# Kizuna42/office-person-detection-vit

Measured on AMD Instinct MI355X. Metric: frames/sec (Phase-2 DETR detect) at 800x1333 batch 8, higher is better.
Workload: dtype f16

## Files before the change

office_person_detection_vit_amd/_capi.py:

```python

from __future__ import annotations

import ctypes as C
import os
from typing import Optional

_HERE = os.path.dirname(os.path.abspath(__file__))
LIB_PATH = os.path.join(_HERE, "libopd_hip.so")
TEST_LIB_PATH = os.path.join(_HERE, "libopd_hip_test.so")

OPD_PIXELS_U8_BGR_HWC = 0
OPD_PIXELS_F32_NCHW = 1
OPD_MEM_HOST = 0
OPD_MEM_DEVICE = 1
OPD_MEM_HOST_PIXELS_DEVICE_OUT = 2
OPD_FLAG_NO_GRAPH = 1
OPD_FLAG_MULTI_STREAM = 2
OPD_REID_MODEL_CLIP = 0
OPD_REID_MODEL_OSNET = 1
OPD_FLAG_BF16 = 4
OPD_COMM_ID_BYTES = 128
OPD_OK, OPD_EINVAL, OPD_EIO, OPD_ESCHEMA, OPD_EHIP, OPD_ENOMEM, OPD_ESTATE = 0, -1, -2, -3, -4, -5, -6


class OpdConfig(C.Structure):
    _fields_ = [("struct_size", C.c_int32), ("max_batch", C.c_int32), ("max_height", C.c_int32),
                ("max_width", C.c_int32), ("flags", C.c_int32), ("reserved", C.c_int32 * 3)]


class OpdKernelStat(C.Structure):
    _fields_ = [("name", C.c_char * 96), ("launches", C.c_int32), ("ms", C.c_float), ("flops", C.c_double)]


class OpdDet(C.Structure):
    _fields_ = [("x1", C.c_float), ("y1", C.c_float), ("x2", C.c_float), ("y2", C.c_float), ("score", C.c_float),
                ("label", C.c_int32), ("query_index", C.c_int32), ("frame", C.c_int32)]


class OpdModelInfo(C.Structure):
    _fields_ = [("depths", C.c_int32 * 4), ("d_model", C.c_int32), ("heads", C.c_int32), ("ffn_dim", C.c_int32),
                ("encoder_layers", C.c_int32), ("decoder_layers", C.c_int32), ("num_queries", C.c_int32),
                ("num_classes_plus1", C.c_int32), ("max_batch", C.c_int32), ("max_height", C.c_int32),
                ("max_width", C.c_int32), ("device_ordinal", C.c_int32), ("weight_bytes_device", C.c_int64),
                ("workspace_bytes_device", C.c_int64)]


class OpdReidConfig(C.Structure):
    _fields_ = [("struct_size", C.c_int32), ("max_crops", C.c_int32), ("flags", C.c_int32), ("model", C.c_int32), ("reserved", C.c_int32 * 4)]


class OpdReidModelInfo(C.Structure):
    _fields_ = [("feature_dim", C.c_int32), ("tokens", C.c_int32), ("hidden", C.c_int32), ("layers", C.c_int32), ("heads", C.c_int32),
                ("mlp_dim", C.c_int32), ("patch", C.c_int32), ("max_crops", C.c_int32), ("device_ordinal", C.c_int32),
                ("model", C.c_int32), ("weight_bytes_device", C.c_int64), ("workspace_bytes_device", C.c_int64)]


API = {
    "opd_detr_create": (C.c_int, [C.POINTER(OpdConfig), C.c_char_p, C.c_int, C.POINTER(C.c_void_p)]),
    "opd_detr_destroy": (None, [C.c_void_p]),
    "opd_detr_clone": (C.c_int, [C.c_void_p, C.POINTER(C.c_void_p)]),
    "opd_detr_info": (C.c_int, [C.c_void_p, C.POINTER(OpdModelInfo)]),
    "opd_detr_forward": (C.c_int, [C.c_void_p, C.c_void_p, C.c_int, C.c_int, C.c_int, C.c_int, C.c_int, C.c_void_p,
                                   C.c_void_p, C.c_void_p]),
    "opd_detr_forward_ragged": (C.c_int, [C.c_void_p, C.c_void_p, C.c_int, C.c_int, C.c_int, C.c_int, C.c_int, C.c_void_p,
                                          C.c_void_p, C.c_void_p, C.c_void_p]),
    "opd_detr_forward_resized": (C.c_int, [C.c_void_p, C.c_void_p] + [C.c_int] * 6 + [C.c_void_p] * 3),
    "opd_detr_resize_u8": (C.c_int, [C.c_void_p, C.c_void_p] + [C.c_int] * 5 + [C.c_void_p]),
    "opd_detr_detect_resized": (C.c_int, [C.c_void_p, C.c_void_p] + [C.c_int] * 6 + [C.c_float, C.POINTER(OpdDet), C.POINTER(C.c_int32)]),
    "opd_detr_detect_frames": (C.c_int, [C.c_void_p, C.POINTER(C.c_void_p)] + [C.c_int] * 6 + [C.c_float, C.POINTER(OpdDet), C.POINTER(C.c_int32)]),
    "opd_detr_detect_frames_features": (C.c_int, [C.c_void_p, C.POINTER(C.c_void_p)] + [C.c_int] * 5 + [C.c_float, C.c_int, C.POINTER(OpdDet), C.POINTER(C.c_int32),
                                                   C.POINTER(C.c_float)]),
    "opd_detr_postprocess": (C.c_int, [C.c_void_p, C.c_float, C.c_void_p, C.POINTER(OpdDet), C.POINTER(C.c_int32)]),
    "opd_detr_detect": (C.c_int, [C.c_void_p, C.c_void_p, C.c_int, C.c_int, C.c_int, C.c_int, C.c_int, C.c_float,
                                  C.c_void_p, C.POINTER(OpdDet), C.POINTER(C.c_int32)]),
    "opd_detr_detect_ragged": (C.c_int, [C.c_void_p, C.c_void_p, C.c_int, C.c_int, C.c_int, C.c_int, C.c_int, C.c_void_p,
                                         C.c_float, C.c_void_p, C.POINTER(OpdDet), C.POINTER(C.c_int32)]),
    "opd_detr_detect_async": (C.c_int, [C.c_void_p, C.c_void_p, C.c_int, C.c_int, C.c_int, C.c_int, C.c_int, C.c_float, C.c_void_p,
                                        C.POINTER(OpdDet), C.POINTER(C.c_int32), C.POINTER(C.c_int)]),
    "opd_detr_wait": (C.c_int, [C.c_void_p, C.c_int]),
    "opd_person_nms": (C.c_int, [C.POINTER(OpdDet), C.c_int, C.c_int, C.c_float]),
    "opd_person_nms_batch": (C.c_int, [C.POINTER(OpdDet), C.POINTER(C.c_int32), C.c_int, C.c_int, C.c_int, C.c_float]),
    "opd_host_alloc": (C.c_int, [C.c_size_t, C.POINTER(C.c_void_p)]),
    "opd_host_free": (None, [C.c_void_p]),
    "opd_similarity_matrix": (C.c_int, [C.c_int, C.c_void_p, C.c_void_p, C.c_void_p, C.c_int, C.c_void_p, C.c_void_p, C.c_void_p, C.c_int,
                                        C.c_int, C.c_double, C.c_double, C.c_int, C.c_void_p]),
    "opd_detr_roi_features": (C.c_int, [C.c_void_p, C.c_int, C.c_void_p, C.c_int, C.c_int, C.c_int, C.c_void_p]),
    "opd_detr_attention_map": (C.c_int, [C.c_void_p, C.c_int, C.c_int, C.c_void_p, C.c_int, C.c_void_p, C.c_int]),
    "opd_detr_set_profiling": (C.c_int, [C.c_void_p, C.c_int]),
    "opd_detr_stage_times": (C.c_int, [C.c_void_p, C.POINTER(C.c_float)]),
    "opd_detr_kernel_times": (C.c_int, [C.c_void_p, C.POINTER(C.c_float), C.POINTER(C.c_int32), C.POINTER(C.c_double)]),
    "opd_detr_kernel_table": (C.c_int, [C.c_void_p, C.c_void_p, C.c_int, C.POINTER(C.c_int)]),
    "opd_comm_available": (C.c_int, []),
    "opd_comm_unique_id": (C.c_int, [C.c_void_p]),
    "opd_comm_create": (C.c_int, [C.c_void_p, C.c_int, C.c_int, C.c_void_p, C.POINTER(C.c_void_p)]),
    "opd_comm_attach": (C.c_int, [C.c_void_p, C.c_void_p, C.POINTER(C.c_void_p)]),
    "opd_comm_destroy": (None, [C.c_void_p]),
    "opd_comm_info": (C.c_int, [C.c_void_p, C.POINTER(C.c_int), C.POINTER(C.c_int)]),
    "opd_comm_begin": (C.c_int, [C.c_void_p, C.c_int]),
    "opd_comm_detect": (C.c_int, [C.c_void_p, C.c_int, C.c_void_p, C.c_int, C.c_int, C.c_int, C.c_int, C.c_int, C.c_float, C.c_void_p]),
    "opd_comm_buffers": (C.c_int, [C.c_void_p, C.c_int, C.POINTER(C.c_void_p), C.POINTER(C.c_void_p)]),
    "opd_comm_exchange": (C.c_int, [C.c_void_p]),
    "opd_comm_wait": (C.c_int, [C.c_void_p, C.POINTER(OpdDet), C.POINTER(C.c_int32)]),
    "opd_reid_create": (C.c_int, [C.POINTER(OpdReidConfig), C.c_char_p, C.c_int, C.POINTER(C.c_void_p)]),
    "opd_reid_destroy": (None, [C.c_void_p]),
    "opd_reid_info": (C.c_int, [C.c_void_p, C.POINTER(OpdReidModelInfo)]),
    "opd_reid_extract": (C.c_int, [C.c_void_p, C.POINTER(C.c_void_p), C.c_void_p, C.c_int, C.c_int, C.c_void_p, C.c_void_p, C.c_int,
                                   C.c_void_p]),
    "opd_last_error": (C.c_char_p, []),
    "opd_version": (C.c_char_p, []),
}

TEST_API = {
    "opd_test_conv_gemm": (C.c_int, [C.c_void_p] * 6 + [C.c_int] * 15),
    "opd_test_gemm_splitk_ln": (C.c_int, [C.c_void_p] * 8 + [C.c_int] * 3),
    "opd_test_gemm_k256": (C.c_int, [C.c_void_p] * 5 + [C.c_int] * 5),
    "opd_test_gemm_ln": (C.c_int, [C.c_void_p] * 8 + [C.c_int] * 2),
    "opd_test_bench_gemm_ln": (C.c_int, [C.c_int] * 4 + [C.POINTER(C.c_float)]),
    "opd_test_gemm_ln_deep": (C.c_int, [C.c_void_p] * 7 + [C.c_int] + [C.c_void_p] * 3 + [C.c_int] * 3),
    "opd_test_set_heads2": (C.c_int, [C.c_int]),
    "opd_test_enc_ffn": (C.c_int, [C.c_void_p] * 9 + [C.c_int] + [C.c_void_p] * 3 + [C.c_int] * 3 + [C.c_void_p] * 2 + [C.c_int] * 2 + [C.c_void_p] * 5 + [C.c_int]),
    "opd_test_bench_enc_ffn": (C.c_int, [C.c_int] * 6 + [C.POINTER(C.c_float)]),
    "opd_test_bench_conv": (C.c_int, [C.c_int] * 11 + [C.POINTER(C.c_float)]),
    "opd_test_trace_btail": (C.c_int, [C.c_int] * 6 + [C.POINTER(C.c_ulonglong), C.c_int, C.POINTER(C.c_int)]),
    "opd_test_trace_conv": (C.c_int, [C.c_int] * 10 + [C.POINTER(C.c_ulonglong), C.c_int, C.POINTER(C.c_int)]),
    "opd_test_btail": (C.c_int, [C.c_void_p] * 10 + [C.c_int] * 6),
    "opd_test_bench_btail": (C.c_int, [C.c_int] * 8 + [C.POINTER(C.c_float)]),
    "opd_test_btail_repeat": (C.c_int, [C.c_void_p] * 8 + [C.c_int] * 6 + [C.POINTER(C.c_int)]),
    "opd_test_attention": (C.c_int, [C.c_void_p] * 4 + [C.c_int] * 4 + [C.c_float]),
    "opd_test_layernorm": (C.c_int, [C.c_void_p] * 5 + [C.c_int]),
    "opd_test_maxpool": (C.c_int, [C.c_void_p] * 2 + [C.c_int] * 6),
    "opd_test_preprocess_u8": (C.c_int, [C.c_void_p] * 2 + [C.c_int] * 5 + [C.c_void_p]),
    "opd_test_attention_masked": (C.c_int, [C.c_void_p] * 4 + [C.c_int] * 4 + [C.c_float, C.c_void_p, C.c_int]),
    "opd_test_stem2": (C.c_int, [C.c_void_p] * 4 + [C.c_int] * 5),
    "opd_test_stem_pool": (C.c_int, [C.c_void_p] * 4 + [C.c_int] * 7),
    "opd_test_set_fuse_stem_pool": (C.c_int, [C.c_void_p, C.c_int]),
    "opd_test_set_pos_shadow": (C.c_int, [C.c_void_p, C.c_int]),
    "opd_test_stem_pool_u8": (C.c_int, [C.c_void_p] * 6 + [C.c_int] * 3),
    "opd_test_set_fuse_btail": (C.c_int, [C.c_void_p, C.c_int]),
    "opd_test_set_fuse_gemm_ln": (C.c_int, [C.c_void_p, C.c_int]),
    "opd_test_f32_to_f16": (C.c_uint16, [C.c_float]),
    "opd_test_f16_to_f32": (C.c_float, [C.c_uint16]),
    "opd_test_normalise_key": (C.c_int, [C.c_char_p, C.c_char_p, C.c_int]),
    "opd_test_inspect_checkpoint": (C.c_int, [C.c_char_p, C.POINTER(C.c_int32)]),
    "opd_test_resize_coeffs": (C.c_int, [C.c_int, C.c_int, C.c_void_p, C.c_void_p, C.c_int]),
    "opd_test_valid_prefix": (C.c_int, [C.c_int] * 3),
    "opd_test_trunk_plan": (C.c_int, [C.c_void_p] + [C.c_int] * 6 + [C.c_void_p, C.c_int, C.c_void_p]),
    "opd_test_sine_pos_embed": (C.c_int, [C.c_int] * 5 + [C.c_void_p]),
    "opd_test_conv_dual": (C.c_int, [C.c_void_p] * 6 + [C.c_int] * 13),
    "opd_test_btail_sc": (C.c_int, [C.c_void_p] * 11 + [C.c_int] * 3),
    "opd_test_btail_chain": (C.c_int, [C.c_void_p] * 13 + [C.c_int] * 4),
    "opd_test_bench_attention": (C.c_int, [C.c_void_p] * 3 + [C.c_int] * 6 + [C.c_float, C.c_int, C.POINTER(C.c_float)]),
    "opd_test_trace_attention": (C.c_int, [C.c_void_p] * 3 + [C.c_int] * 6 + [C.c_float, C.c_void_p, C.c_int, C.POINTER(C.c_int)]),
    "opd_test_heads": (C.c_int, [C.c_void_p] * 13 + [C.c_int] * 2),
    "opd_test_postprocess": (C.c_int, [C.c_void_p] * 3 + [C.c_int] * 3 + [C.c_float, C.c_void_p, C.c_void_p]),
    "opd_test_roi_features": (C.c_int, [C.c_void_p] * 2 + [C.c_int] * 3 + [C.c_void_p]),
    "opd_test_set_conv_flags": (C.c_int, [C.c_int]),
    "opd_test_set_gemm_ln_kloop": (C.c_int, [C.c_int]),
    "opd_test_set_graph_guard": (C.c_int, [C.c_int]),
    "opd_test_set_alloc_poison": (C.c_int, [C.c_int]),
    "opd_test_check_redzones": (C.c_int, [C.c_void_p]),
    "opd_test_set_taps": (C.c_int, [C.c_void_p, C.c_int]),
    "opd_test_read_taps": (C.c_int, [C.c_void_p, C.c_void_p, C.c_int, C.c_char_p, C.c_int]),
    "opd_test_round_f16_diffused": (C.c_int, [C.c_void_p, C.c_int, C.c_int, C.c_int]),
    "opd_test_dec_qkv": (C.c_int, [C.c_void_p, C.c_void_p, C.c_int] + [C.c_void_p] * 5 + [C.c_int] * 2 + [C.c_void_p] * 4),
    "opd_test_dec_self": (C.c_int, [C.c_void_p] * 10 + [C.c_int, C.c_int, C.c_float, C.c_void_p]),
    "opd_test_attention_split": (C.c_int, [C.c_void_p] * 3 + [C.c_int] * 4 + [C.c_float, C.c_int, C.c_void_p, C.c_int, C.c_void_p, C.c_void_p]),
    "opd_test_dec_cross_out": (C.c_int, [C.c_void_p, C.c_void_p, C.c_int, C.c_void_p, C.c_int] + [C.c_void_p] * 4 + [C.c_int, C.c_void_p]),
    "opd_test_dec_ffn": (C.c_int, [C.c_void_p] * 4 + [C.c_int, C.c_int, C.c_void_p]),
    "opd_test_bench_dec": (C.c_int, [C.c_int] * 6 + [C.POINTER(C.c_float)]),
    "opd_test_heads_fused": (C.c_int, [C.c_void_p, C.c_void_p, C.c_int] + [C.c_void_p] * 13 + [C.c_int, C.c_int, C.c_void_p, C.c_void_p]),
    "opd_test_set_fused_dec": (C.c_int, [C.c_void_p, C.c_int]),
    "opd_test_set_elem_bf16": (C.c_int, [C.c_int]),
    "opd_test_trace_dec_self": (C.c_int, [C.c_int, C.c_int, C.c_void_p]),
    "opd_test_reid_geometry": (C.c_int, [C.c_void_p, C.c_int, C.c_int, C.c_int, C.c_void_p]),
    "opd_test_reid_coeffs": (C.c_int, [C.c_int] * 4 + [C.c_void_p, C.c_void_p, C.c_int]),
    "opd_test_reid_lut": (C.c_int, [C.c_void_p]),
    "opd_test_reid_pixels_host": (C.c_int, [C.c_void_p, C.c_int, C.c_int, C.c_void_p] + [C.c_int] * 3 + [C.c_void_p]),
    "opd_test_reid_pixels": (C.c_int, [C.c_void_p, C.POINTER(C.c_void_p), C.c_void_p, C.c_int, C.c_int, C.c_void_p, C.c_void_p, C.c_int,
                                       C.c_void_p]),
    "opd_test_reid_attention": (C.c_int, [C.c_void_p, C.c_void_p] + [C.c_int] * 3),
    "opd_test_reid_layernorm": (C.c_int, [C.c_void_p] * 5 + [C.c_int] * 3),
    "opd_test_reid_gemm": (C.c_int, [C.c_int, C.c_void_p, C.c_void_p, C.c_void_p, C.c_int, C.c_void_p] + [C.c_int] * 3),
    "opd_test_reid_l2norm": (C.c_int, [C.c_void_p] + [C.c_int] * 2),
    "opd_test_osnet_lut": (C.c_int, [C.c_void_p]),
    "opd_test_osnet_geometry": (C.c_int, [C.c_void_p, C.c_int, C.c_int, C.c_int, C.c_void_p]),
    "opd_test_osnet_pixels_host": (C.c_int, [C.c_void_p, C.c_int, C.c_int, C.c_void_p, C.c_int, C.c_void_p]),
    "opd_test_osnet_stem": (C.c_int, [C.c_void_p] * 4 + [C.c_int] * 2),
    "opd_test_osnet_gemm": (C.c_int, [C.c_int, C.c_void_p, C.c_int, C.c_int, C.c_void_p, C.c_int, C.c_int, C.c_void_p, C.c_void_p, C.c_void_p,
                                      C.c_int, C.c_void_p] + [C.c_int] * 6),
    "opd_test_osnet_dwconv": (C.c_int, [C.c_void_p] * 4 + [C.c_int] * 7),
    "opd_test_osnet_gate": (C.c_int, [C.c_void_p] * 7 + [C.c_int] * 4),
    "opd_test_osnet_avgpool2": (C.c_int, [C.c_void_p] * 2 + [C.c_int] * 4),
    "opd_test_osnet_head": (C.c_int, [C.c_void_p] * 4 + [C.c_int] * 3),
    "opd_test_reid_kernel_table": (C.c_int, [C.c_void_p, C.POINTER(C.c_void_p), C.c_void_p, C.c_int, C.c_void_p, C.c_void_p, C.c_int, C.c_int,
                                             C.POINTER(OpdKernelStat), C.c_int, C.POINTER(C.c_int)]),
}

_lib: Optional[C.CDLL] = None
_lib_has_hooks = False


def load_library(test_hooks: bool = False) -> C.CDLL:
    global _lib, _lib_has_hooks
    test_hooks = test_hooks or os.environ.get("OPD_TEST_HOOKS") == "1"
    if _lib is not None:
        if test_hooks and not _lib_has_hooks:
            raise RuntimeError("the product library is already loaded in this process; load the test build first "
                               "(_capi.load_library(test_hooks=True) or OPD_TEST_HOOKS=1)")
        return _lib
    path = TEST_LIB_PATH if test_hooks else LIB_PATH
    if not os.path.exists(path):
        raise RuntimeError(
            f"HIP extension not built: {path} is missing (run `python -c 'import __graft_entry__ as g; g.build()'`). "
            "This package has no CPU fallback.")
    lib = C.CDLL(path)
    for table in (API, TEST_API) if test_hooks else (API,):
        for name, (res, args) in table.items():
            fn = getattr(lib, name)
            fn.restype = res
            fn.argtypes = args
    _lib, _lib_has_hooks = lib, test_hooks
    return lib


def last_error() -> str:
    return load_library().opd_last_error().decode("utf-8", "replace")


def check(rc: int, what: str) -> None:
    if rc != 0:
        raise RuntimeError(f"{what} failed (code {rc}): {last_error()}")
```

office_person_detection_vit_amd/csrc/kernels_btail.hip:

```cpp
#include <hip/hip_runtime.h>
#include "opd_kernels.h"
#include "opd_elem.h"

typedef elem_t half8 __attribute__((ext_vector_type(8)));
typedef float float4v __attribute__((ext_vector_type(4)));
typedef unsigned int uint2v __attribute__((ext_vector_type(2)));
typedef unsigned int uint4v __attribute__((ext_vector_type(4)));

namespace {

constexpr int ROW_BYTES = 128;
constexpr int NW = 4;

__device__ __forceinline__ int swz(int row, int chunk) { return row * ROW_BYTES + ((chunk ^ (row & 7)) << 4); }

__device__ __forceinline__ int xcd_logical_block(int bid, int nblocks) {
    const int q = nblocks >> 3, r = nblocks & 7;
    const int x = bid & 7, k = bid >> 3;
    return (x < r ? x * (q + 1) : r * (q + 1) + (x - r) * q) + k;
}

__device__ __forceinline__ int own_row(const int rho) { return (rho & ~31) | (((rho >> 2) & 3) << 3) | (((rho >> 4) & 1) << 2) | (rho & 3); }
__device__ __forceinline__ int own_ch(const int nt, const int g) { return (nt >> 1) * 32 + g * 8 + (nt & 1) * 4; }

__device__ __forceinline__ int fdiv(const int m, const FastDiv& f) {
    return f.one ? m : (int)(__umulhi((unsigned)m, f.mul) >> f.shift);
}

__device__ __forceinline__ int xcd_logical_block_rev(int bid, int nblocks) {
    const int q = nblocks >> 3, r = nblocks & 7;
    const int x = bid & 7, k = bid >> 3;
    return (x < r ? x * (q + 1) + q - k : r * (q + 1) + (x - r) * q + q - 1 - k);
}

__device__ __forceinline__ unsigned pack2h(float a, float b) {
    typedef elem_t half2v __attribute__((ext_vector_type(2)));
    half2v h;
    h[0] = (elem_t)a;
    h[1] = (elem_t)b;
    unsigned u;
    __builtin_memcpy(&u, &h, 4);
    return u;
}
__device__ __forceinline__ void unpack2h(unsigned u, float& a, float& b) {
    typedef elem_t half2v __attribute__((ext_vector_type(2)));
    half2v h;
    __builtin_memcpy(&h, &u, 4);
    a = (float)h[0];
    b = (float)h[1];
}
__device__ __forceinline__ half8 as_half8(unsigned a, unsigned b, unsigned c, unsigned d) {
    uint4v u = {a, b, c, d};
    half8 h;
    __builtin_memcpy(&h, &u, 16);
    return h;
}

template <int N_OUTSTANDING>
__device__ __forceinline__ void wait_vmcnt() {
    static_assert(N_OUTSTANDING >= 0 && N_OUTSTANDING <= 63, "vmcnt range");
    asm volatile("s_waitcnt vmcnt(%0)" ::"n"(N_OUTSTANDING) : "memory");
}
__device__ __forceinline__ void compiler_fence() { asm volatile("" ::: "memory"); }

template <int C1, int C3, bool RDMA, bool SC = false, bool TRACE = false, int RC = 0>
__global__ __launch_bounds__(64 * NW, 8 / NW) void btail_kernel(BtailParams p) {
#if defined(__HIP_DEVICE_COMPILE__)
    unsigned long long tstamp[16] = {};
    auto stamp = [&](const int i) {
        if constexpr (TRACE) asm volatile("s_memtime %0\n\ts_waitcnt lgkmcnt(0)" : "=s"(tstamp[i])::"memory");
    };
    if constexpr (TRACE) asm volatile("s_memrealtime %0\n\ts_waitcnt lgkmcnt(0)" : "=s"(tstamp[0])::"memory");
    stamp(1);
    static_assert(!RDMA || C1 == 64, "residual staging buffers are budgeted for C1 == 64 (80 KiB of LDS per workgroup)");
    static_assert(!RDMA || RC == 0, "a rebuilt residual is not staged");
    static_assert(!SC || (C1 == 64 && !RDMA), "fused shortcut: 64-channel tails only; it replaces the residual");
    extern __shared__ __attribute__((aligned(16))) unsigned char smem[];
    constexpr int C2 = 4 * C1;
    constexpr int NT1 = C1 / 16;
    constexpr int KK1 = C1 / 32;
    constexpr int BM = 32 * NW;
    constexpr int A_BYTES = BM * ROW_BYTES;
    constexpr int RC_BYTES = RC ? 2 * 64 * ROW_BYTES : 0;
    constexpr int W1_PIECES = C1 / (8 * NW);
    constexpr int NCH = C2 / 64;
    constexpr int W2C_BYTES = 64 * C1 * 2;
    constexpr int W2_PIECES = W2C_BYTES / (1024 * NW);
    constexpr int W3_PIECES = C3 / (8 * NW);
    constexpr int SC_PIECES = 8 / NW;
    static_assert(W1_PIECES >= 1 && W2_PIECES >= 1 && (C3 == 0 || W3_PIECES >= 1), "every wave stages at least one piece of every operand");
    constexpr int NT3 = C3 / 16;
    constexpr int WSC_BYTES = SC ? 64 * ROW_BYTES : 0;
    constexpr int CHUNK_BYTES = W2C_BYTES + C3 * ROW_BYTES + WSC_BYTES + RC_BYTES;
    constexpr int STAGE_BYTES = (A_BYTES + C1 * ROW_BYTES) > CHUNK_BYTES ? (A_BYTES + C1 * ROW_BYTES) : CHUNK_BYTES;
    static_assert(RC == 0 || (RC == 1 && C1 == 64 && !RDMA && !SC), "residual rebuild: second block of stage 1");

    const int tid = threadIdx.x;
    const int lane = tid & 63;
    const int wave = __builtin_amdgcn_readfirstlane(tid >> 6);
    const int g = lane >> 4, li = lane & 15;
    const int m_base = (p.rev ? xcd_logical_block_rev(blockIdx.x, gridDim.x) : xcd_logical_block(blockIdx.x, gridDim.x)) * BM;
    const int wm0 = m_base + wave * 32;

    const int lrow = lane >> 3;
    const int lchunk = (lane & 7) ^ lrow;
    const unsigned backoff = (unsigned)(p.W + 1) * (unsigned)C1 * 2u;
    const __amdgpu_buffer_rsrc_t rsrc_a = __builtin_amdgcn_make_buffer_rsrc(
        const_cast<char*>(reinterpret_cast<const char*>(p.x1)) - backoff, 0, (unsigned)((size_t)p.B * p.H * p.W * C1 * 2) + backoff, 0x00020000);
    const __amdgpu_buffer_rsrc_t rsrc_w1 = __builtin_amdgcn_make_buffer_rsrc(const_cast<f16_t*>(p.w1), 0, (unsigned)(C1 * 9 * C1 * 2), 0x00020000);
    const __amdgpu_buffer_rsrc_t rsrc_w2 = __builtin_amdgcn_make_buffer_rsrc(const_cast<f16_t*>(p.w2p), 0, (unsigned)(C2 * C1 * 2), 0x00020000);
    const __amdgpu_buffer_rsrc_t rsrc_w3 = __builtin_amdgcn_make_buffer_rsrc(const_cast<f16_t*>(C3 ? p.w3p : p.w2p), 0, (unsigned)((C3 ? C3 : 1) * C2 * 2), 0x00020000);
    const __amdgpu_buffer_rsrc_t rsrc_sc = __builtin_amdgcn_make_buffer_rsrc(const_cast<f16_t*>(SC ? p.wsc : RC ? p.rc_wsc : p.w2p), 0, (unsigned)(C2 * 64 * 2), 0x00020000);
    const __amdgpu_buffer_rsrc_t rsrc_rw = __builtin_amdgcn_make_buffer_rsrc(const_cast<f16_t*>(RC ? p.rc_w2 : p.w2p), 0, (unsigned)(C2 * 64 * 2), 0x00020000);
    unsigned rowoff[4], rowmask[4], woff1[W1_PIECES], woff2[W2_PIECES], woff3[W3_PIECES ? W3_PIECES : 1], woffsc[2];
#pragma unroll
    for (int i = 0; i < 2; ++i)
        woffsc[i] = (unsigned)(own_row(((wave * SC_PIECES + i) & 7) * 8 + lrow) * 64) * 2u + (unsigned)lchunk * 16u;
    {
        const int ohw = p.OH * p.OW;
#pragma unroll
        for (int i = 0; i < 4; ++i) {
            const int m = m_base + (wave * 4 + i) * 8 + lrow;
            const bool okm = m < p.M;
            const int mm = okm ? m : 0;
            const int b = fdiv(mm, p.fd_ohw);
            const int r = mm - b * ohw;
            const int oh = fdiv(r, p.fd_ow);
            const int ow = r - oh * p.OW;
            rowoff[i] = (unsigned)(((b * p.H + oh * p.stride) * p.W + ow * p.stride) * C1) * 2u + (unsigned)lchunk * 16u;
            unsigned kwmask = 0, mask = 0;
#pragma unroll
            for (int kw = 0; kw < 3; ++kw)
                if ((unsigned)(ow * p.stride - 1 + kw) < (unsigned)p.W) kwmask |= 1u << kw;
#pragma unroll
            for (int kh = 0; kh < 3; ++kh)
                if ((unsigned)(oh * p.stride - 1 + kh) < (unsigned)p.H) mask |= kwmask << (kh * 3);
            rowmask[i] = okm ? mask : 0u;
        }
#pragma unroll
        for (int i = 0; i < W1_PIECES; ++i)
            woff1[i] = (unsigned)(own_row((wave * W1_PIECES + i) * 8 + lrow) * (9 * C1)) * 2u + (unsigned)lchunk * 16u;
#pragma unroll
        for (int i = 0; i < W2_PIECES; ++i) {
            const int q = wave * W2_PIECES + i;
            woff2[i] = (unsigned)(own_row((q & 7) * 8 + lrow) * C1 + (q >> 3) * 64) * 2u + (unsigned)lchunk * 16u;
        }
#pragma unroll
        for (int i = 0; i < W3_PIECES; ++i)
            woff3[i] = (unsigned)(own_row((wave * W3_PIECES + i) * 8 + lrow) * C2) * 2u + (unsigned)lchunk * 16u;
    }

    constexpr int kpc = C1 / 64;
    constexpr int nk = 9 * kpc;
    int tap_kh = 0, tap_kw = 0, tap_c = 0;
    auto issue_main = [&](int ks, int buf) {
        unsigned char* As = smem + buf * STAGE_BYTES;
        unsigned char* Ws = As + A_BYTES;
        const int tap = tap_kh * 3 + tap_kw;
        const int soff_a = ((tap_kh * p.W + tap_kw) * C1 + tap_c * 64) * 2;
#pragma unroll
        for (int i = 0; i < 4; ++i) {
            const unsigned vo = ((rowmask[i] >> tap) & 1u) ? rowoff[i] : 0x80000000u;
            __builtin_amdgcn_raw_ptr_buffer_load_lds(rsrc_a, (__attribute__((address_space(3))) void*)(As + (wave * 4 + i) * 1024), 16, vo,
                                                     soff_a, 0, 0);
        }
#pragma unroll
        for (int i = 0; i < W1_PIECES; ++i)
            __builtin_amdgcn_raw_ptr_buffer_load_lds(rsrc_w1, (__attribute__((address_space(3))) void*)(Ws + (wave * W1_PIECES + i) * 1024),
                                                     16, woff1[i], ks * 128, 0, 0);
        if (++tap_c == kpc) {
            tap_c = 0;
            if (++tap_kw == 3) { tap_kw = 0; ++tap_kh; }
        }
    };
    auto issue_chunk = [&](int j, int buf) {
        unsigned char* W2s = smem + buf * STAGE_BYTES;
#pragma unroll
        for (int i = 0; i < W2_PIECES; ++i)
            __builtin_amdgcn_raw_ptr_buffer_load_lds(rsrc_w2, (__attribute__((address_space(3))) void*)(W2s + (wave * W2_PIECES + i) * 1024),
                                                     16, woff2[i], j * (64 * C1 * 2), 0, 0);
        if constexpr (C3 > 0) {
            unsigned char* W3s = W2s + W2C_BYTES;
#pragma unroll
            for (int i = 0; i < W3_PIECES; ++i)
                __builtin_amdgcn_raw_ptr_buffer_load_lds(rsrc_w3, (__attribute__((address_space(3))) void*)(W3s + (wave * W3_PIECES + i) * 1024),
                                                         16, woff3[i], j * 128, 0, 0);
        }
        if constexpr (SC) {
            unsigned char* Wscs = W2s + W2C_BYTES + C3 * ROW_BYTES;
#pragma unroll
            for (int i = 0; i < SC_PIECES; ++i)
                __builtin_amdgcn_raw_ptr_buffer_load_lds(rsrc_sc, (__attribute__((address_space(3))) void*)(Wscs + (wave * SC_PIECES + i) * 1024), 16,
                                                         woffsc[i], j * (64 * 64 * 2), 0, 0);
        }
        if constexpr (RC) {
            unsigned char* Wr = W2s + W2C_BYTES + C3 * ROW_BYTES;
#pragma unroll
            for (int i = 0; i < SC_PIECES; ++i) {
                __builtin_amdgcn_raw_ptr_buffer_load_lds(rsrc_rw, (__attribute__((address_space(3))) void*)(Wr + (wave * SC_PIECES + i) * 1024), 16,
                                                         woffsc[i], j * (64 * 64 * 2), 0, 0);
                __builtin_amdgcn_raw_ptr_buffer_load_lds(rsrc_sc, (__attribute__((address_space(3))) void*)(Wr + 8192 + (wave * SC_PIECES + i) * 1024), 16,
                                                         woffsc[i], j * (64 * 64 * 2), 0, 0);
            }
        }
    };
    const bool pr_ok[2] = {wm0 + li < p.M, wm0 + 16 + li < p.M};
    bool y_ok[2] = {pr_ok[0] && p.y != nullptr, pr_ok[1] && p.y != nullptr};
    if (p.y_stride2) {
#pragma unroll
        for (int mt = 0; mt < 2; ++mt) {
            const int m = wm0 + mt * 16 + li;
            const int r = m - fdiv(m, p.fd_ohw) * (p.OH * p.OW);
            const int oh = fdiv(r, p.fd_ow), ow = r - oh * p.OW;
            y_ok[mt] = y_ok[mt] && !((oh | ow) & 1);
        }
    }
    const size_t pr_row[2] = {(size_t)(wm0 + li) * C2 + g * 8, (size_t)(wm0 + 16 + li) * C2 + g * 8};
    constexpr int RES_BUF = NW * 4096;
    unsigned char* const res_lds = smem + 2 * STAGE_BYTES + wave * 4096;
    const __amdgpu_buffer_rsrc_t rsrc_r = __builtin_amdgcn_make_buffer_rsrc(
        const_cast<f16_t*>(p.res ? p.res : p.x1), 0, p.res ? (unsigned)((size_t)p.M * C2 * 2) : 0u, 0x00020000);
    const unsigned res_voff = (unsigned)((wm0 + lrow) * C2) * 2u + (unsigned)lchunk * 16u;
    auto issue_res = [&](int j) {
#pragma unroll
        for (int i = 0; i < 4; ++i)
            __builtin_amdgcn_raw_ptr_buffer_load_lds(rsrc_r, (__attribute__((address_space(3))) void*)(res_lds + (j & 1) * RES_BUF + i * 1024), 16,
                                                     res_voff + (unsigned)(i * 8 * C2 * 2), j * 128, 0, 0);
    };
    const bool has_res = RC ? true : (!SC && p.res != nullptr && !(p.dbg & 4));
    const bool res_dma = RDMA && has_res;
    auto load_res = [&](int j, uint4 (&r)[4]) {
        if constexpr (RDMA) {
            if (has_res) issue_res(j);
        } else {
#pragma unroll
            for (int i = 0; i < 4; ++i) {
                r[i] = make_uint4(0u, 0u, 0u, 0u);
                if (has_res && pr_ok[i & 1]) r[i] = *reinterpret_cast<const uint4*>(p.res + pr_row[i & 1] + j * 64 + (i >> 1) * 32);
            }
        }
    };

    const int ks_first = (p.dbg & 1) ? nk - 1 : 0;
    if (ks_first) { tap_kh = 2; tap_kw = 2; tap_c = kpc - 1; }
    half8 xs[2][2], a1p[2][2];
    if constexpr (SC || RC != 0) {
        const f16_t* xsrc = SC ? p.xs : p.rc_xs;
#pragma unroll
        for (int mt = 0; mt < 2; ++mt) {
            const int m = wm0 + mt * 16 + li;
#pragma unroll
            for (int kk = 0; kk < 2; ++kk) {
                half8 v = {}, u = {};
                if (m < p.M) v = *reinterpret_cast<const half8*>(xsrc + (size_t)m * 64 + kk * 32 + g * 8);
                if constexpr (RC != 0)
                    if (m < p.M) u = *reinterpret_cast<const half8*>(p.rc_a1 + (size_t)m * 64 + kk * 32 + g * 8);
                xs[mt][kk] = v;
                a1p[mt][kk] = u;
            }
        }
    }
    stamp(2);
    issue_main(ks_first, ks_first & 1);
    float4v acc1[NT1][2];
#pragma unroll
    for (int nt = 0; nt < NT1; ++nt) {
        const float4v b = *reinterpret_cast<const float4v*>(p.b1 + own_ch(nt, g));
        acc1[nt][0] = b;
        acc1[nt][1] = b;
    }
    OPD_DMA_BARRIER();
    uint4 res[3][4];
    auto compute_main = [&](int buf) {
        const unsigned char* As = smem + buf * STAGE_BYTES;
        const unsigned char* Ws = As + A_BYTES;
#pragma unroll
        for (int kk = 0; kk < 2; ++kk) {
            half8 xf[2], wf[NT1];
#pragma unroll
            for (int mt = 0; mt < 2; ++mt) xf[mt] = *reinterpret_cast<const half8*>(As + swz(wave * 32 + mt * 16 + li, kk * 4 + g));
#pragma unroll
            for (int nt = 0; nt < NT1; ++nt) wf[nt] = *reinterpret_cast<const half8*>(Ws + swz(nt * 16 + li, kk * 4 + g));
#pragma unroll
            for (int nt = 0; nt < NT1; ++nt)
#pragma unroll
                for (int mt = 0; mt < 2; ++mt) acc1[nt][mt] = OPD_MFMA_16x16x32(wf[nt], xf[mt], acc1[nt][mt]);
        }
    };
#pragma unroll 1
    for (int ks = ks_first; ks + 1 < nk; ++ks) {
        issue_main(ks + 1, (ks + 1) & 1);
        compute_main(ks & 1);
        __syncthreads();
    }
    issue_chunk(0, nk & 1);
    compiler_fence();
    if constexpr (RC == 0) {
        load_res(0, res[0]);
        load_res(1, res[1]);
    }
    compiler_fence();
    compute_main((nk - 1) & 1);
    if (res_dma) wait_vmcnt<4>();
    else wait_vmcnt<0>();
    __builtin_amdgcn_s_barrier();
    stamp(3);

    half8 a1[2][KK1];
#pragma unroll
    for (int mt = 0; mt < 2; ++mt)
#pragma unroll
        for (int kk = 0; kk < KK1; ++kk) {
            float4v u = acc1[2 * kk][mt], v = acc1[2 * kk + 1][mt];
#pragma unroll
            for (int r = 0; r < 4; ++r) {
                u[r] = u[r] > 0.f ? u[r] : 0.f;
                v[r] = v[r] > 0.f ? v[r] : 0.f;
            }
            a1[mt][kk] = as_half8(pack2h(u[0], u[1]), pack2h(u[2], u[3]), pack2h(v[0], v[1]), pack2h(v[2], v[3]));
        }

    if (p.a1_out) {
#pragma unroll
        for (int mt = 0; mt < 2; ++mt)
#pragma unroll
            for (int kk = 0; kk < KK1; ++kk)
                if (pr_ok[mt]) *reinterpret_cast<half8*>(p.a1_out + (size_t)(wm0 + mt * 16 + li) * C1 + kk * 32 + g * 8) = a1[mt][kk];
    }

    float4v accz[NT3 ? NT3 : 1][2];
    if constexpr (C3 > 0) {
#pragma unroll
        for (int nt = 0; nt < NT3; ++nt) {
            const float4v b = *reinterpret_cast<const float4v*>(p.b3 + own_ch(nt, g));
            accz[nt][0] = b;
            accz[nt][1] = b;
        }
    }

    if (p.dbg & 8) return;
#pragma unroll
    for (int j = 0; j < NCH; ++j) {
        const int buf = (nk + j) & 1;
        uint4 (&res_cur)[4] = res[j % 3];
        if (j + 1 < NCH) issue_chunk(j + 1, buf ^ 1);
        compiler_fence();
        if constexpr (RDMA) {
            if (has_res) {
#pragma unroll
                for (int i = 0; i < 4; ++i)
                    res_cur[i] = *reinterpret_cast<const uint4*>(res_lds + (j & 1) * RES_BUF + swz((i & 1) * 16 + li, (i >> 1) * 4 + g));
                asm volatile("s_waitcnt lgkmcnt(0)" ::: "memory");
                if (j + 2 < NCH) issue_res(j + 2);
            }
        } else if constexpr (RC == 0) {
            if (j + 2 < NCH) load_res(j + 2, res[(j + 2) % 3]);
        }
        compiler_fence();
        const unsigned char* W2s = smem + buf * STAGE_BYTES;
        if constexpr (RC != 0) {
            const unsigned char* Wr = W2s + W2C_BYTES + C3 * ROW_BYTES;
            float4v accr[4][2];
#pragma unroll
            for (int nt = 0; nt < 4; ++nt) {
                const float4v b = *reinterpret_cast<const float4v*>(p.rc_b + j * 64 + own_ch(nt, g));
                accr[nt][0] = b;
                accr[nt][1] = b;
            }
#pragma unroll
            for (int half = 0; half < 2; ++half)
#pragma unroll
                for (int kk = 0; kk < 2; ++kk) {
                    half8 wf[4];
#pragma unroll
                    for (int nt = 0; nt < 4; ++nt) wf[nt] = *reinterpret_cast<const half8*>(Wr + half * 8192 + swz(nt * 16 + li, kk * 4 + g));
#pragma unroll
                    for (int nt = 0; nt < 4; ++nt)
#pragma unroll
                        for (int mt = 0; mt < 2; ++mt) accr[nt][mt] = OPD_MFMA_16x16x32(wf[nt], half ? xs[mt][kk] : a1p[mt][kk], accr[nt][mt]);
                }
#pragma unroll
            for (int q = 0; q < 2; ++q)
#pragma unroll
                for (int mt = 0; mt < 2; ++mt) {
                    float4v v0 = accr[2 * q][mt], v1 = accr[2 * q + 1][mt];
#pragma unroll
                    for (int r = 0; r < 4; ++r) {
                        v0[r] = v0[r] > 0.f ? v0[r] : 0.f;
                        v1[r] = v1[r] > 0.f ? v1[r] : 0.f;
                    }
                    res_cur[2 * q + mt] = make_uint4(pack2h(v0[0], v0[1]), pack2h(v0[2], v0[3]), pack2h(v1[0], v1[1]), pack2h(v1[2], v1[3]));
                }
        }
        float4v acc2[4][2];
#pragma unroll
        for (int nt = 0; nt < 4; ++nt) {
            const float4v b = *reinterpret_cast<const float4v*>(p.b2 + j * 64 + own_ch(nt, g));
            acc2[nt][0] = b;
            acc2[nt][1] = b;
        }
#pragma unroll
        for (int kk = 0; kk < KK1; ++kk) {
            half8 wf[4];
#pragma unroll
            for (int nt = 0; nt < 4; ++nt)
                wf[nt] = *reinterpret_cast<const half8*>(W2s + (kk >> 1) * 8192 + swz(nt * 16 + li, (kk & 1) * 4 + g));
#pragma unroll
            for (int nt = 0; nt < 4; ++nt)
#pragma unroll
                for (int mt = 0; mt < 2; ++mt) acc2[nt][mt] = OPD_MFMA_16x16x32(wf[nt], a1[mt][kk], acc2[nt][mt]);
        }
        if constexpr (SC) {
            const unsigned char* Wscs = W2s + W2C_BYTES + C3 * ROW_BYTES;
#pragma unroll
            for (int kk = 0; kk < 2; ++kk) {
                half8 wf[4];
#pragma unroll
                for (int nt = 0; nt < 4; ++nt) wf[nt] = *reinterpret_cast<const half8*>(Wscs + swz(nt * 16 + li, kk * 4 + g));
#pragma unroll
                for (int nt = 0; nt < 4; ++nt)
#pragma unroll
                    for (int mt = 0; mt < 2; ++mt) acc2[nt][mt] = OPD_MFMA_16x16x32(wf[nt], xs[mt][kk], acc2[nt][mt]);
            }
        }
        half8 yf[2][2];
#pragma unroll
        for (int q = 0; q < 2; ++q)
#pragma unroll
            for (int mt = 0; mt < 2; ++mt) {
                float4v v0 = acc2[2 * q][mt], v1 = acc2[2 * q + 1][mt];
                if (has_res) {
                    const uint4 r = res_cur[2 * q + mt];
                    float a, b;
                    unpack2h(r.x, a, b); v0[0] += a; v0[1] += b;
                    unpack2h(r.y, a, b); v0[2] += a; v0[3] += b;
                    unpack2h(r.z, a, b); v1[0] += a; v1[1] += b;
                    unpack2h(r.w, a, b); v1[2] += a; v1[3] += b;
                }
#pragma unroll
                for (int r = 0; r < 4; ++r) {
                    v0[r] = v0[r] > 0.f ? v0[r] : 0.f;
                    v1[r] = v1[r] > 0.f ? v1[r] : 0.f;
                }
                yf[q][mt] = as_half8(pack2h(v0[0], v0[1]), pack2h(v0[2], v0[3]), pack2h(v1[0], v1[1]), pack2h(v1[2], v1[3]));
            }
        if constexpr (C3 > 0) {
            const unsigned char* W3s = W2s + W2C_BYTES;
#pragma unroll
            for (int kk = 0; kk < 2; ++kk) {
#pragma unroll
                for (int nt = 0; nt < NT3; ++nt) {
                    const half8 wf = *reinterpret_cast<const half8*>(W3s + swz(nt * 16 + li, kk * 4 + g));
#pragma unroll
                    for (int mt = 0; mt < 2; ++mt) accz[nt][mt] = OPD_MFMA_16x16x32(wf, yf[kk][mt], accz[nt][mt]);
                }
            }
        }
        if (j + 1 < NCH) {
            if (res_dma && j + 2 < NCH) wait_vmcnt<4>();
            else wait_vmcnt<0>();
            __builtin_amdgcn_s_barrier();
        }
#pragma unroll
        for (int q = 0; q < 2; ++q)
#pragma unroll
            for (int mt = 0; mt < 2; ++mt)
                if (y_ok[mt] && !(p.dbg & 2)) *reinterpret_cast<half8*>(p.y + pr_row[mt] + j * 64 + q * 32) = yf[q][mt];
        stamp(4 + j);
    }

    if constexpr (C3 > 0) {
#pragma unroll
        for (int q = 0; q < NT3 / 2; ++q)
#pragma unroll
            for (int mt = 0; mt < 2; ++mt) {
                float4v v0 = accz[2 * q][mt], v1 = accz[2 * q + 1][mt];
#pragma unroll
                for (int r = 0; r < 4; ++r) {
                    v0[r] = v0[r] > 0.f ? v0[r] : 0.f;
                    v1[r] = v1[r] > 0.f ? v1[r] : 0.f;
                }
                if (pr_ok[mt] && !(p.dbg & 2))
                    *reinterpret_cast<uint4*>(p.z + (size_t)(wm0 + mt * 16 + li) * C3 + q * 32 + g * 8) =
                        make_uint4(pack2h(v0[0], v0[1]), pack2h(v0[2], v0[3]), pack2h(v1[0], v1[1]), pack2h(v1[2], v1[3]));
            }
    }
    if constexpr (TRACE) {
        stamp(4 + NCH);
        asm volatile("s_waitcnt vmcnt(0)" ::: "memory");
        stamp(5 + NCH);
        asm volatile("s_memrealtime %0\n\ts_waitcnt lgkmcnt(0)" : "=s"(tstamp[15])::"memory");
        if (threadIdx.x == 0 && p.trace) {
#pragma unroll
            for (int i = 0; i < 16; ++i) p.trace[(size_t)blockIdx.x * 16 + i] = tstamp[i];
        }
    }
#endif
}

template <int C1, int C3, bool RDMA, bool SC = false, bool TRACE = false, int RC = 0>
hipError_t launch_btail_t(const BtailParams& p, hipStream_t stream) {
    constexpr int BM = 32 * NW;
    constexpr int MAIN = (BM + C1) * ROW_BYTES, CHUNK = 64 * C1 * 2 + C3 * ROW_BYTES + (SC ? 64 * ROW_BYTES : 0) + (RC ? 2 * 64 * ROW_BYTES : 0);
    constexpr int LDS = 2 * (MAIN > CHUNK ? MAIN : CHUNK) + (RDMA ? 2 * NW * 4096 : 0);
    static_assert(LDS <= 160 * 1024, "LDS per workgroup");
    OPD_SET_MAX_LDS_ONCE((btail_kernel<C1, C3, RDMA, SC, TRACE, RC>), LDS);
    OPD_LAUNCH((btail_kernel<C1, C3, RDMA, SC, TRACE, RC>), dim3((p.M + BM - 1) / BM), dim3(64 * NW), LDS, stream, p);
    static const char* const kname = opd_kernel_name("btail_kernel<%d, %d, %s, %s, %s, %d>", C1, C3, OPD_BOOLSTR(RDMA), OPD_BOOLSTR(SC), OPD_BOOLSTR(TRACE), RC);
    opd_last_kernel_name = kname;
    return hipGetLastError();
}

}

#ifndef OPD_ELEM_BF16
bool opd_btail_supported(int C1, int C3) {
    return (C1 == 64 && (C3 == 0 || C3 == 64 || C3 == 128)) || (C1 == 128 && (C3 == 0 || C3 == 128)) || opd_btail256_supported(C1, C3);
}
#endif

hipError_t OPD_SYM(opd_launch_btail)(const BtailParams& p_in, hipStream_t stream) {
    if (!opd_btail_supported(p_in.C1, p_in.C3) || p_in.OH <= 0 || p_in.OW <= 0) return hipErrorInvalidValue;
    BtailParams p = p_in;
    p.fd_ohw = opd_make_fastdiv((unsigned)p.OH * (unsigned)p.OW);
    p.fd_ow = opd_make_fastdiv((unsigned)p.OW);
    if ((size_t)p.B * p.H * p.W * p.C1 * 2 + (size_t)(p.W + 1) * p.C1 * 2 >= 0x7fffff00ull) return hipErrorInvalidValue;
    if ((size_t)p.M * p.C1 * 8 >= 0x7fffff00ull) return hipErrorInvalidValue;
    if (p.C1 == 256) return OPD_SYM(opd_launch_btail256)(p, stream);
    if (p.y_stride2 && (p.stride != 1 || p.C3 == 0)) return hipErrorInvalidValue;
    if (!p.y && !p.a1_out) return hipErrorInvalidValue;
    if (p.rc) {
        if (p.rc != 1 || p.C1 != 64 || p.C3 != 64 || p.stride != 1 || p.res || p.xs || !p.rc_a1 || !p.rc_xs || !p.rc_w2 || !p.rc_wsc || !p.rc_b ||
            p.trace || (size_t)p.M * 64 * 2 >= 0x7fffff00ull)
            return hipErrorInvalidValue;
        return launch_btail_t<64, 64, false, false, false, 1>(p, stream);
    }
    if (p.xs) {
        if (p.C1 != 64 || p.C3 != 64 || p.stride != 1 || !p.wsc || p.res || (size_t)p.M * 64 * 2 >= 0x7fffff00ull) return hipErrorInvalidValue;
        return launch_btail_t<64, 64, false, true>(p, stream);
    }
    if (p.trace) {
        if (p.C1 == 64 && p.C3 == 64 && (p.dbg & 16)) return launch_btail_t<64, 64, false, false, true>(p, stream);
        if (p.C1 == 64 && p.C3 == 64) return launch_btail_t<64, 64, true, false, true>(p, stream);
        if (p.C1 == 128 && p.C3 == 128) return launch_btail_t<128, 128, false, false, true>(p, stream);
        return hipErrorInvalidValue;
    }
    if (p.C1 == 64) {
        const bool rdma = !(p.dbg & 16);
        if (p.C3 == 0) return rdma ? launch_btail_t<64, 0, true>(p, stream) : launch_btail_t<64, 0, false>(p, stream);
        if (p.C3 == 64) return rdma ? launch_btail_t<64, 64, true>(p, stream) : launch_btail_t<64, 64, false>(p, stream);
        return rdma ? launch_btail_t<64, 128, true>(p, stream) : launch_btail_t<64, 128, false>(p, stream);
    }
    if (p.C3 == 0) return launch_btail_t<128, 0, false>(p, stream);
    return launch_btail_t<128, 128, false>(p, stream);
}

#ifndef OPD_ELEM_BF16
void opd_permute_k32(const f16_t* w, f16_t* out, int rows, int K) {
    for (int n = 0; n < rows; ++n)
        for (int b = 0; b < K; b += 32)
            for (int g = 0; g < 4; ++g)
                for (int e = 0; e < 4; ++e) {
                    out[(size_t)n * K + b + 8 * g + e] = w[(size_t)n * K + b + 4 * g + e];
                    out[(size_t)n * K + b + 8 * g + 4 + e] = w[(size_t)n * K + b + 16 + 4 * g + e];
                }
}
#endif
```

office_person_detection_vit_amd/csrc/opd_kernels.h:

```cpp
#pragma once
#include <hip/hip_runtime.h>
#include <stdint.h>
#include <vector>

typedef uint16_t f16_t;
enum { OPD_DT_F16 = 0, OPD_DT_BF16 = 1 };

#include <mutex>
#define OPD_SET_MAX_LDS_ONCE(kernel, bytes)                                                                                  \
    do {                                                                                                                     \
        static std::once_flag once_[16];                                                                                     \
        static hipError_t err_[16];                                                                                          \
        int dev_ = 0;                                                                                                        \
        if (hipGetDevice(&dev_) != hipSuccess || dev_ < 0 || dev_ >= 16) return hipErrorInvalidDevice;    \
        std::call_once(once_[dev_], [&] { err_[dev_] = hipFuncSetAttribute(reinterpret_cast<const void*>(kernel), hipFuncAttributeMaxDynamicSharedMemorySize, (bytes)); }); \
        if (err_[dev_] != hipSuccess) return err_[dev_];                                                                     \
    } while (0)

extern thread_local const char* opd_last_kernel_name;
extern thread_local int opd_dbg_skip_launch;
const char* opd_kernel_name(const char* fmt, ...);
#define OPD_LAUNCH(kernel, ...)                       \
    do {                                              \
        opd_last_kernel_name = #kernel;               \
        if (!opd_dbg_skip_launch) hipLaunchKernelGGL(kernel, __VA_ARGS__); \
    } while (0)
#define OPD_BOOLSTR(b) ((b) ? "true" : "false")

#if defined(__HIP_DEVICE_COMPILE__)
#define OPD_DMA_BARRIER()                                        \
    do {                                                         \
        asm volatile("s_waitcnt vmcnt(0)" ::: "memory");         \
        __syncthreads();                                         \
    } while (0)
#else
#define OPD_DMA_BARRIER() __syncthreads()
#endif

struct FastDiv { unsigned mul, shift, one; };
inline FastDiv opd_make_fastdiv(unsigned d) {
    FastDiv f{0u, 0u, 1u};
    if (d <= 1u) return f;
    int s = 0;
    while ((1ull << s) < d) ++s;
    f.mul = (unsigned)(((1ull << (31 + s)) + d - 1) / d);
    f.shift = (unsigned)(s - 1);
    f.one = 0u;
    return f;
}

struct ConvGemmParams {
    const f16_t* x;
    const f16_t* w;
    const float* bias;
    const float* const* bias_ptrs;
    const f16_t* res16;
    const float* res32;
    void* out;
    f16_t* out16_aux;
    const void* zero16;
    int B, H, W, Cin, OH, OW, N, KH, KW, stride, pad;
    int M, K;
    int relu, bias_period, out_f32;
    int bias_pmod, bias_pcols;
    int stem;
    int dbg;
    int split_k;
    const f16_t* x2;
    int H2, W2, Cin2, stride2, K1;
    FastDiv fd_ohw, fd_ow, fd_period;
    const f16_t* x_alt;
    int alt_mod, alt_cols;
    unsigned tap_rep;
    FastDiv fd_tilesn, fd_ntiles;
    unsigned long long* trace;
    int force_mt;
    int wprefetch;
    int flat_staging;
    int dtype;
};
hipError_t opd_launch_conv_gemm(const ConvGemmParams& p, hipStream_t stream);
bool opd_conv_w8_supported(const ConvGemmParams& p);
hipError_t opd_launch_conv_w8(const ConvGemmParams& p, hipStream_t stream);
hipError_t opd_launch_stem_pool_u8(const uint8_t* frames, const int32_t* valid_hw, const f16_t* w, const float* bias, f16_t* out, int B, int H,
                                   int W, int OH, int OW, int PH, int PW, hipStream_t stream, int dtype = 0);
hipError_t opd_launch_stem_pool(const f16_t* x4p, const f16_t* w, const float* bias, f16_t* out, int B, int Hp, int Wp, int OH,
                                int OW, int PH, int PW, hipStream_t stream, int dtype = 0);
struct BtailParams {
    const f16_t* x1;
    const f16_t* w1;
    const float* b1;
    const f16_t* w2p;
    const float* b2;
    const f16_t* res;
    const f16_t* xs;
    const f16_t* wsc;
    f16_t* y;
    const f16_t* w3p;
    const float* b3;
    f16_t* z;
    int B, H, W, OH, OW, stride, M, C1, C3;
    int dbg;
    FastDiv fd_ohw, fd_ow;
    unsigned long long* trace;
    int rev;
    int dtype;
    f16_t* a1_out;
    const f16_t* rc_a1;
    const f16_t* rc_xs;
    const f16_t* rc_w2;
    const f16_t* rc_wsc;
    const float* rc_b;
    int rc;
    int y_stride2;
};
bool opd_btail_supported(int C1, int C3);
hipError_t opd_launch_btail(const BtailParams& p, hipStream_t stream);
void opd_permute_k32(const f16_t* w, f16_t* out, int rows, int K);
bool opd_btail256_supported(int C1, int C3);
hipError_t opd_launch_btail256(const BtailParams& p, hipStream_t stream);

struct GemmLnParams {
    const f16_t* x;
    const f16_t* w;
    const float* bias;
    const float* res32;
    const float* gamma;
    const float* beta;
    float* y32;
    f16_t* y16;
    int M, K;
    int kloop;
    int deep_k;
    const float* pos;
    const float* const* pos_ptrs;
    int pos_period;
    f16_t* yp16;
    int dtype;
};
hipError_t opd_launch_gemm_ln(const GemmLnParams& p, hipStream_t stream);
struct EncFfnParams {
    const f16_t* x;
    const unsigned char* wpack;
    const float* b2;
    const float* res32;
    const float* gamma;
    const float* beta;
    float* y32;
    f16_t* y16;
    f16_t* yp16;
    const float* pos;
    const float* const* pos_ptrs;
    int pos_period;
    int M, F;
    int dtype;
    int dbg;
    int wprefetch;
    const f16_t* attn;
    const float* bo;
    const float* gamma1;
    const float* beta1;
    int pack_front;
    int pack_tail;
    int tail, tail_pos;
    f16_t* tail_out;
    int tail_ld;
    int tail_col[16];
};
hipError_t opd_launch_enc_ffn(const EncFfnParams& p, hipStream_t stream);
size_t opd_encffn_pack_bytes(int F, int tail, int front);
void opd_encffn_pack(const uint16_t* w1, const float* b1, const uint16_t* w2, int F, const uint16_t* wt, const float* bt, int tail, const uint16_t* wo,
                     unsigned char* out);
struct GemmK256Params {
    const f16_t* x;
    const f16_t* w;
    const float* bias;
    f16_t* out16;
    float* out32;
    int M, N, ldx, ldw, slices, bias_period, relu;
    int dtype;
};
hipError_t opd_launch_gemm_k256(const GemmK256Params& p, hipStream_t stream);

hipError_t opd_launch_preprocess_u8(const uint8_t* frames, f16_t* out, int B, int H, int W, int Hp, int Wp, const int32_t* valid_hw,
                                    hipStream_t stream, int dtype = 0);
hipError_t opd_launch_preprocess_f32(const float* pv, f16_t* out, int B, int H, int W, int Hp, int Wp, const int32_t* valid_hw,
                                     hipStream_t stream, int dtype = 0);
void opd_resize_coeffs(int in_size, int out_size, std::vector<int32_t>* bounds, std::vector<int32_t>* coeffs, int* ksize_out);
hipError_t opd_launch_resize_u8(const uint8_t* in, uint8_t* out, int B, int h, int w, int oh, int ow, const int32_t* bounds_h,
                                const int32_t* coeff_h, int ksize_h, const int32_t* bounds_v, const int32_t* coeff_v, int ksize_v,
                                hipStream_t stream);
hipError_t opd_launch_maxpool(const f16_t* x, f16_t* out, int B, int H, int W, int C, int OH, int OW, hipStream_t stream, int dtype = 0);
hipError_t opd_launch_layernorm(const float* x, const float* gamma, const float* beta, float* y, f16_t* y16,
                                int rows, hipStream_t stream, int dtype = 0);
hipError_t opd_launch_reduce_ln(const float* partials, int nsplit, size_t slab_stride, const float* residual,
                                const float* gamma, const float* beta, float* y, f16_t* y16, int rows, hipStream_t stream, int dtype = 0);
hipError_t opd_launch_reduce_ln_pos(const float* partials, int nsplit, size_t slab_stride, const float* residual, const float* gamma,
                                    const float* beta, float* y, f16_t* y16, int rows, const float* pos, const float* const* pos_ptrs,
                                    int period, f16_t* yp16, hipStream_t stream, int dtype = 0);
hipError_t opd_launch_broadcast_rows(const float* c, float* y, f16_t* y16, int rows, hipStream_t stream, int dtype = 0);
hipError_t opd_launch_cast_f16(const float* x, f16_t* y, size_t n, hipStream_t stream, int dtype = 0);
hipError_t opd_launch_reduce_act16(const float* partials, int nsplit, size_t slab_stride, f16_t* out, size_t n, int relu, hipStream_t stream, int dtype = 0);
#define OPD_TAP_BLOCKS 64
hipError_t opd_launch_checksum(const void* buf, size_t bytes, unsigned long long* slots, hipStream_t stream);
hipError_t opd_launch_gemm_f32(const float* A, const float* Wt, const float* bias, float* C, int M, int N, int K,
                               int ldc, hipStream_t stream);
struct HeadParams {
    const float* hs;
    const float* partials;
    int nsplit;
    const float *ffn_b2, *ln3_gamma, *ln3_beta;
    const float *ln_gamma, *ln_beta;
    const float *wc, *bc, *w1, *b1, *w2, *b2, *w3, *b3;
    const f16_t *wc_f, *w1_f, *w2_f;
    float* logits;
    float* boxes;
    int rows, ncls;
};
hipError_t opd_launch_heads(const HeadParams& p, hipStream_t stream);
hipError_t opd_launch_heads2(const HeadParams& p, hipStream_t stream);
struct PostParams {
    const float* logits;
    const float* boxes;
    const int32_t* orig_hw;
    void* records;
    int32_t* counts;
    int B, Q, ncls;
    float threshold;
};
hipError_t opd_launch_postprocess(const PostParams& p, hipStream_t stream);
hipError_t opd_launch_roi_features(const float* enc, const int32_t* rois , float* out,
                                   int n, int h, int w, hipStream_t stream);
hipError_t opd_launch_roi_features_records(const float* enc, const void* records, const int32_t* counts, const int32_t* orig_hw, int label,
                                           float* out, int B, int Q, int h, int w, hipStream_t stream);

hipError_t opd_launch_attention_map(const f16_t* q, int ldq, const f16_t* k, int ldk, const int32_t* sel, int nsel, int heads, int Lk, float scale,
                                    const int32_t* key_valid2, int key_row, void* stat, float* out, hipStream_t stream, int dtype = 0);

hipError_t opd_launch_similarity_matrix(const float* f1, const float* b1, const uint8_t* has1, int n1, const float* f2, const float* b2,
                                        const uint8_t* has2, int n2, int D, double aw, double mw, int as_distance, float* out,
                                        hipStream_t stream);

void opd_split_f16_frag(const float* w, int N, int K, f16_t* out);
struct DecQkvParams {
    const float* h_in;
    const float* partials;
    int nsplit;
    const float* b2;
    const float *ln_g, *ln_b;
    float* h_out;
    const f16_t* w;
    const float* bias;
    f16_t* q16;
    f16_t* k16;
    f16_t* vT;
    int M, Q;
};
hipError_t opd_launch_dec_qkv(const DecQkvParams& p, hipStream_t stream);
struct DecSelfParams {
    const f16_t *q16, *k16, *vT;
    float* h;
    const f16_t* wo;
    const float *bo, *ln_g, *ln_b;
    const f16_t* wq;
    const float* rbq;
    f16_t* qc16;
    int qc_bf16;
// ... 72 lines not shown
```

office_person_detection_vit_amd/csrc/opd_model.cpp:

```cpp
#include <new>
#include <stdexcept>

#include "opd_model.h"

using namespace opd;


namespace opd {

std::atomic<int> g_alloc_poison{-1};

static int upload_f32(opd_detr* m, float** dst, const std::vector<float>& v) {
    RCCHK(dalloc(m, dst, v.size(), true));
    HIPCHK(hipMemcpy(*dst, v.data(), v.size() * 4, hipMemcpyHostToDevice));
    return OPD_OK;
}
static int upload_f16(opd_detr* m, f16_t** dst, const std::vector<float>& v) {
    std::vector<f16_t> h(v.size());
    if (m->dtype == OPD_DT_BF16) for (size_t i = 0; i < v.size(); ++i) h[i] = f32_to_bf16(v[i]);
    else for (size_t i = 0; i < v.size(); ++i) h[i] = f32_to_f16(v[i]);
    RCCHK(dalloc(m, dst, h.size(), true));
    HIPCHK(hipMemcpy(*dst, h.data(), h.size() * 2, hipMemcpyHostToDevice));
    return OPD_OK;
}
// ... 492 lines not shown
    HIPCHK(opd_launch_checksum(p, bytes, m->d_taps + (size_t)m->tap_next * OPD_TAP_BLOCKS, m->stream));
    if ((int)m->tap_names.size() <= m->tap_next) m->tap_names.resize(m->tap_next + 1);
    m->tap_names[m->tap_next++] = name;
    return OPD_OK;
}

static int conv_splits(const opd_detr* m, const Conv& c, int stage) {
    if (!m->sw.small_splitk || stage < 0 || stage > 3 || c.stem || c.K % 64 != 0 || c.Cout % 64 != 0) return 1;
    const long long px = (long long)m->cfg.max_batch * (long long)m->stage_px[stage];
    const long long tiles = ((px + 127) / 128) * (c.Cout / 64);
    const int nk = c.K / 64;
    if (tiles > 160 || nk < 24) return 1;
    int best = 1;
    for (int s : {2, 3, 4, 6, 8})
        if (nk % s == 0 && nk / s >= 6 && tiles * s <= 640) best = s;
    return best;
}

static int run_conv(opd_detr* m, const Conv& c, const f16_t* x, int B, int H, int W, int OH, int OW, void* out, bool relu,
                    const f16_t* res16, int stage = -1) {
    ConvGemmParams p{}; p.dtype = m->dtype;
    p.x = x; p.w = c.w; p.bias = c.bias; p.res16 = res16; p.res32 = nullptr; p.out = out; p.out16_aux = nullptr; p.zero16 = m->zero_bias;
    p.B = B; p.H = H; p.W = W; p.Cin = c.Cin; p.OH = OH; p.OW = OW; p.N = c.Cout; p.KH = c.KH; p.KW = c.KW;
    p.stride = c.stride; p.pad = c.pad; p.M = B * OH * OW; p.K = c.K; p.relu = relu ? 1 : 0; p.bias_period = 0;
    p.out_f32 = 0; p.stem = c.stem ? 1 : 0; p.dbg = m->sw.dbg_gemm; p.wprefetch = m->sw.wprefetch & 1;
    if (const int splits = res16 ? 1 : conv_splits(m, c, stage); splits > 1 && (size_t)splits * p.M * c.Cout <= m->slab_floats) {
        p.out = m->d_slab; p.out_f32 = 1; p.relu = 0; p.split_k = splits;
        RCCHK(timed_begin(m, CLS_CONV, 2.0 * p.M * (double)c.Cout * c.KH * c.KW * c.Cin));
        HIPCHK(opd_launch_conv_gemm(p, m->stream));
        RCCHK(timed_end(m));
        RCCHK(timed_begin(m, CLS_OTHER, 0.0));
        HIPCHK(opd_launch_reduce_act16(m->d_slab, splits, (size_t)p.M * c.Cout, reinterpret_cast<f16_t*>(out), (size_t)p.M * c.Cout, relu ? 1 : 0, m->stream, m->dtype));
        RCCHK(timed_end(m));
        RCCHK(tap(m, c.KH == 3 ? "conv3x3" : "conv1x1", out, (size_t)p.M * c.Cout * 2));
        return OPD_OK;
    }
    RCCHK(timed_begin(m, CLS_CONV, 2.0 * p.M * (double)c.Cout * c.KH * c.KW * c.Cin));
    bool w8 = false;
    if (m->sw.w8 && c.Cout % 256 == 0 && c.Cout >= 512) {
        const long long tiles = (((long long)OH * OW * m->cfg.max_batch + 127) / 128) * (c.Cout / 256);
        const bool few = tiles <= 3LL * m->num_cus;
        const int kind = c.KH == 3 ? (m->sw.w8 & 1) : (c.K >= 1024 ? (m->sw.w8 & 2) : (c.K == 512 ? (m->sw.w8 & 4) : 0));
        w8 = few && kind && opd_conv_w8_supported(p);
    }
    HIPCHK(w8 ? opd_launch_conv_w8(p, m->stream) : opd_launch_conv_gemm(p, m->stream));
    RCCHK(timed_end(m));
    RCCHK(tap(m, c.KH == 3 ? "conv3x3" : "conv1x1", out, (size_t)p.M * c.Cout * 2));
    return OPD_OK;
}

static int run_gemm(opd_detr* m, const f16_t* x, const f16_t* w, const float* bias, int bias_period, int M, int N, int K,
                    void* out, bool out_f32, bool relu, const float* res32, const float* const* bias_ptrs = nullptr, int bias_pmod = 0,
                    int bias_pcols = 0, const f16_t* x_alt = nullptr, int alt_mod = 0, int alt_cols = 0) {
    ConvGemmParams p{}; p.dtype = m->dtype;
    p.bias_ptrs = bias_ptrs; p.bias_pmod = bias_pmod; p.bias_pcols = bias_pcols;
    p.x_alt = x_alt; p.alt_mod = alt_mod; p.alt_cols = alt_cols;
    p.x = x; p.w = w; p.bias = bias; p.res16 = nullptr; p.res32 = res32; p.out = out; p.out16_aux = nullptr; p.zero16 = m->zero_bias;
    p.B = M; p.H = 1; p.W = 1; p.Cin = K; p.OH = 1; p.OW = 1; p.N = N; p.KH = 1; p.KW = 1; p.stride = 1; p.pad = 0;
    p.M = M; p.K = K; p.relu = relu ? 1 : 0; p.bias_period = bias_period; p.out_f32 = out_f32 ? 1 : 0; p.stem = 0; p.dbg = m->sw.dbg_gemm; p.wprefetch = m->sw.wprefetch & 1;
    RCCHK(timed_begin(m, CLS_GEMM, 2.0 * M * (double)N * K));
    HIPCHK(opd_launch_conv_gemm(p, m->stream));
    RCCHK(timed_end(m));
    RCCHK(tap(m, "gemm", out, (size_t)M * N * (out_f32 ? 4 : 2)));
    return OPD_OK;
}

struct PosShadow { const float* pos; const float* const* pos_ptrs; int period; f16_t* yp16; };
static int run_gemm_splitk_ln(opd_detr* m, const f16_t* x, const f16_t* w, const float* bias, int M, int N, int K, int splits,
                              const float* res32, const LNp* ln, float* y32, f16_t* y16, int cls, const PosShadow* ps = nullptr) {
    ConvGemmParams p{}; p.dtype = m->dtype;
    p.x = x; p.w = w; p.bias = bias; p.out = m->d_slab; p.zero16 = m->zero_bias;
    p.B = M; p.H = 1; p.W = 1; p.Cin = K; p.OH = 1; p.OW = 1; p.N = N; p.KH = 1; p.KW = 1; p.stride = 1; p.pad = 0;
    p.M = M; p.K = K; p.out_f32 = 1; p.split_k = splits;
    RCCHK(timed_begin(m, cls, 2.0 * M * (double)N * K));
    HIPCHK(opd_launch_conv_gemm(p, m->stream));
    RCCHK(timed_end(m));
    RCCHK(tap(m, "splitk_slabs", m->d_slab, (size_t)splits * M * N * 4));
    RCCHK(timed_begin(m, CLS_OTHER, 0.0));
    HIPCHK(opd_launch_reduce_ln_pos(m->d_slab, splits, (size_t)M * N, res32, ln ? ln->g : nullptr, ln ? ln->b : nullptr, y32, y16, M,
                                    ps ? ps->pos : nullptr, ps ? ps->pos_ptrs : nullptr, ps ? ps->period : 0, ps ? ps->yp16 : nullptr, m->stream, m->dtype));
    RCCHK(timed_end(m));
    RCCHK(tap(m, "reduce_ln", y32, (size_t)M * N * 4));
    return OPD_OK;
}

static int run_gemm_ln(opd_detr* m, const f16_t* x, const f16_t* w, const float* bias, int M, int K, const float* res32,
                       const LNp& ln, float* y32, f16_t* y16) {
    GemmLnParams p{}; p.dtype = m->dtype;
    p.x = x; p.w = w; p.bias = bias; p.res32 = res32; p.gamma = ln.g; p.beta = ln.b; p.y32 = y32; p.y16 = y16; p.M = M; p.K = K;
    RCCHK(timed_begin(m, CLS_GEMM, 2.0 * M * 256.0 * K));
    HIPCHK(opd_launch_gemm_ln(p, m->stream));
    RCCHK(timed_end(m));
    RCCHK(tap(m, "gemm_ln", y32, (size_t)M * 256 * 4));
    return OPD_OK;
}

static int run_small_gemm(opd_detr* m, const f16_t* x, const f16_t* w, const float* bias, int bias_period, int M, int N, int K,
                          f16_t* out16, bool relu) {
    GemmK256Params p{}; p.dtype = m->dtype;
    p.x = x; p.w = w; p.bias = bias; p.out16 = out16; p.M = M; p.N = N; p.ldx = K; p.ldw = K; p.slices = 1;
    p.bias_period = bias_period; p.relu = relu ? 1 : 0;
    RCCHK(timed_begin(m, CLS_GEMM, 2.0 * M * (double)N * K));
    HIPCHK(opd_launch_gemm_k256(p, m->stream));
    RCCHK(timed_end(m));
    RCCHK(tap(m, "gemm_k256", out16, (size_t)M * N * 2));
    return OPD_OK;
}
static int run_small_gemm_ln(opd_detr* m, const f16_t* x, const f16_t* w, const float* bias, int M, int K, const float* res32,
                             const LNp& ln, float* y32, f16_t* y16) {
    GemmK256Params p{}; p.dtype = m->dtype;
    p.x = x; p.w = w; p.bias = bias; p.out32 = m->d_slab; p.M = M; p.N = 256; p.ldx = K; p.ldw = K; p.slices = K / 256;
    RCCHK(timed_begin(m, CLS_GEMM, 2.0 * M * 256.0 * K));
    HIPCHK(opd_launch_gemm_k256(p, m->stream));
    RCCHK(timed_end(m));
    RCCHK(timed_begin(m, CLS_OTHER, 0.0));
    HIPCHK(opd_launch_reduce_ln(m->d_slab, p.slices, (size_t)M * 256, res32, ln.g, ln.b, y32, y16, M, m->stream, m->dtype));
    RCCHK(timed_end(m));
    RCCHK(tap(m, "small_gemm_ln", y32, (size_t)M * 256 * 4));
    return OPD_OK;
}

static int run_attn(opd_detr* m, const f16_t* q, int ldq, const f16_t* k, int ldk, const f16_t* v, int ldv, f16_t* o, int ldo,
                    int B, int Lq, int Lk, const int32_t* key_valid = nullptr, int key_row = 0) {
    AttnParams p{}; p.dtype = m->dtype;
    p.key_valid = key_valid; p.key_row = key_row;
    p.q = q; p.k = k; p.v = v; p.o = o; p.B = B; p.heads = m->arch.heads; p.Lq = Lq; p.Lk = Lk;
    p.ldq = ldq; p.ldk = ldk; p.ldv = ldv; p.ldo = ldo;
    p.scale = 1.0f / sqrtf((float)(m->arch.d_model / m->arch.heads));
    RCCHK(timed_begin(m, CLS_ATTN, 4.0 * B * (double)m->arch.heads * Lq * Lk * 32));
    HIPCHK(opd_launch_attention(p, m->stream));
    RCCHK(timed_end(m));
    if (ldo == m->arch.d_model) RCCHK(tap(m, "attention", o, (size_t)B * Lq * ldo * 2));
    return OPD_OK;
}

TrunkPlan plan_trunk(const Arch& a, const std::vector<Block>& blocks, const opd_config& cfg, const Switches& sw, int B, int H2, int W2, int num_cus,
                     bool taps, int profiling, bool has_stream2) {
    TrunkPlan plan;
    plan.steps.resize(blocks.size());
    plan.split = B;
    const bool multi = (cfg.flags & OPD_FLAG_MULTI_STREAM) != 0;
    int ch = H2, cw = W2, oh3 = 0, ow3 = 0;
    for (int s = 0, bi = 0; s < 4; ++s) {
        for (int l = 0; l < a.depths[s]; ++l, ++bi) {
            const Block& b = blocks[bi];
            const Block* nbk = bi + 1 < (int)blocks.size() ? &blocks[bi + 1] : nullptr;
            const int oh = (b.c1.stride == 2) ? down2(ch) : ch, ow = (b.c1.stride == 2) ? down2(cw) : cw;
            const int C1 = b.c1.Cin;
            const bool sc_in_tail = b.has_sc && sw.fuse_shortcut && sw.fuse_btail && block_has_bias2sc(b) && b.sc.KH == 1 && b.sc.stride == 1 &&
                                    b.sc.Cin == 64 && b.c1.Cin == 64 && b.c1.stride == 1 && b.c2.Cout == 256 && nbk && conv_has_kperm(nbk->c0) &&
                                    nbk->c0.Cin == 256 && nbk->c0.Cout == 64;
            bool tail = sw.fuse_btail && b.c1.KH == 3 && b.c1.Cout == C1 && b.c2.Cin == C1 && b.c2.Cout == 4 * C1 && conv_has_kperm(b.c2) &&
                        opd_btail_supported(C1, 0);
            if (sw.dual_over_tail && tail && b.has_sc && !sc_in_tail && block_has_w2sc(b)) tail = false;
            if (C1 == 256 && tail) {
                const long long tiles = ((long long)cfg.max_batch * oh * ow + 127) / 128;
                const bool pays = tiles * 10 >= (long long)num_cus * 6;
                if (sw.tail3 == 0 || (sw.tail3 == 1 && !pays && !multi)) tail = false;
            }
            const bool sc_in_expand = b.has_sc && sw.fuse_shortcut && block_has_w2sc(b) && !sc_in_tail && !tail;
            tail = tail && (size_t)B * ch * cw * C1 * 2 < 0x7ff00000ull;
            TrunkStep& t = plan.steps[bi];
            t.path = tail ? PATH_TAIL : sc_in_expand ? PATH_DUAL : PATH_CONVS;
            t.sc = !b.has_sc ? SC_NONE : (sc_in_tail && tail) ? SC_TAIL : sc_in_expand ? SC_EXPAND : SC_LAUNCH;
            t.res = (t.sc == SC_TAIL || t.sc == SC_EXPAND) ? RES_NONE : t.sc == SC_LAUNCH ? RES_SHORTCUT : RES_TRUNK;
            t.store = STORE_Y;
            t.C3 = 0;
            if (tail && nbk && conv_has_kperm(nbk->c0) && nbk->c0.Cin == 4 * C1 && opd_btail_supported(C1, nbk->c0.Cout)) t.C3 = nbk->c0.Cout;
            if (tail && sw.y_stride2 && t.C3 && b.c1.stride == 1 && l + 1 == a.depths[s] && nbk && nbk->has_sc && nbk->sc.stride == 2 && nbk->sc.KH == 1 &&
                nbk->c1.stride == 2 && !taps)
                t.store = STORE_Y_STRIDE2;
            if (l > 0 && sw.tail_rc && !taps) {
                TrunkStep& prev = plan.steps[bi - 1];
                if (prev.path == PATH_TAIL && prev.sc == SC_TAIL && prev.C3 == 64 && prev.store == STORE_Y && tail && C1 == 64 && t.C3 == 64 &&
                    t.res == RES_TRUNK) {
                    prev.store = STORE_A1;
                    t.res = RES_REBUILD;
                }
            }
            if (s == 2 && l == 0) { oh3 = oh; ow3 = ow; }
            ch = oh; cw = ow;
        }
    }
    const int s3 = a.depths[0] + a.depths[1], s4 = s3 + a.depths[2];
    bool fused3 = a.depths[2] > 2 && profiling != 1 && !taps && has_stream2 && sw.tail3_split && !multi && B >= 2;
    for (int bi = s3 + 1; bi < s4 && fused3; ++bi) fused3 = plan.steps[bi].path == PATH_TAIL;
    if (fused3) {
        auto tiles_of = [&](int frames) { return ((long long)frames * oh3 * ow3 + 127) / 128; };
        const long long total = tiles_of(B), cus = num_cus, last = total % cus;
        if (total > cus && last > 0 && last < cus / 2) {
            const long long whole = (total / cus) * cus;
            int bA = B - 1;
            while (bA > 1 && tiles_of(bA) > whole) --bA;
            if (tiles_of(bA) <= whole) plan.split = bA;
        }
    }
    int n = 0;
    auto rev = [&](const TrunkStep& t) { return t.path == PATH_TAIL && sw.tail_rev ? (n++ & 1) : 0; };
    for (int bi = 0; bi < s4; ++bi) plan.steps[bi].rev = rev(plan.steps[bi]);
    for (int bi = s3 + 1; bi < s4 && plan.split < B; ++bi) plan.steps[bi].rev_b = rev(plan.steps[bi]);
    for (int bi = s4; bi < (int)blocks.size(); ++bi) plan.steps[bi].rev = rev(plan.steps[bi]);
    return plan;
}

#define MARK(i)                                                   \
    do {                                                          \
        if (m->profiling) HIPCHK(hipEventRecord(m->ev[i], m->stream)); \
        opd_dbg_skip_launch = (m->sw.dbg_skip >> (i)) & 1;           \
    } while (0)

static bool is_ragged(const int32_t* valid_hw, int B, int H, int W) {
    if (!valid_hw) return false;
    for (int b = 0; b < B; ++b)
        if (valid_hw[2 * b] != H || valid_hw[2 * b + 1] != W) return true;
    return false;
}

static int enqueue_forward(opd_detr* m, const void* d_pixels, int pixel_format, int B, int H, int W, const int32_t* valid_hw = nullptr) {
    const Arch& a = m->arch;
    Dims d;
    compute_dims(B, H, W, &d);
    const int fh = d.sh[3], fw = d.sw[3];
    const bool ragged = is_ragged(valid_hw, B, H, W);
    Plan* plan = nullptr;
    const float* const* enc_bias_ptrs[16] = {};
    const float* const* kv_bias_ptrs = nullptr;
    const float* const* pos_ptrs = nullptr;
    const int32_t *d_valid = nullptr, *d_keyv = nullptr;
    if (!ragged) {
        RCCHK(get_plan(m, fh, fw, fh, fw, &plan));
    } else {
        if (a.enc_layers > 16) return fail(OPD_EINVAL, "ragged batches: at most 16 encoder layers");
        m->h_valid_hw.assign(valid_hw, valid_hw + 2 * B);
        m->h_key_valid.resize((size_t)2 * B);
        m->h_bias_ptrs.assign((size_t)(a.enc_layers + 2) * B, nullptr);
        for (int b = 0; b < B; ++b) {
            const int vh = valid_hw[2 * b], vw = valid_hw[2 * b + 1];
            if (vh < 1 || vw < 1 || vh > H || vw > W) return fail(OPD_EINVAL, "valid_hw outside the frame canvas");
            const int vfh = valid_prefix(vh, H, fh), vfw = valid_prefix(vw, W, fw);
            if (vfh < 1 || vfw < 1) return fail(OPD_EINVAL, "frame too small: no valid feature-map position");
            m->h_key_valid[2 * b] = vfh; m->h_key_valid[2 * b + 1] = vfw;
            Plan* pb = nullptr;
            RCCHK(get_plan(m, fh, fw, vfh, vfw, &pb));
            if (b == 0) plan = pb;
            for (int i = 0; i < a.enc_layers; ++i) m->h_bias_ptrs[(size_t)i * B + b] = pb->rb_enc[i];
            m->h_bias_ptrs[(size_t)a.enc_layers * B + b] = pb->rb_kv;
            m->h_bias_ptrs[(size_t)(a.enc_layers + 1) * B + b] = pb->d_pos;
        }
        HIPCHK(hipMemcpyAsync(m->d_valid_hw, m->h_valid_hw.data(), (size_t)2 * B * 4, hipMemcpyHostToDevice, m->stream));
        HIPCHK(hipMemcpyAsync(m->d_key_valid, m->h_key_valid.data(), (size_t)2 * B * 4, hipMemcpyHostToDevice, m->stream));
        HIPCHK(hipMemcpyAsync(m->d_bias_ptrs, m->h_bias_ptrs.data(), m->h_bias_ptrs.size() * sizeof(float*), hipMemcpyHostToDevice, m->stream));
        for (int i = 0; i < a.enc_layers; ++i) enc_bias_ptrs[i] = m->d_bias_ptrs + (size_t)i * B;
        kv_bias_ptrs = m->d_bias_ptrs + (size_t)a.enc_layers * B;
        pos_ptrs = m->d_bias_ptrs + (size_t)(a.enc_layers + 1) * B;
        d_valid = m->d_valid_hw;
        d_keyv = m->d_key_valid;
    }
    timed_reset(m);
    m->tap_next = 0;
    if (pixel_format == OPD_PIXELS_U8_BGR_HWC) RCCHK(tap(m, "pixels_u8", d_pixels, (size_t)B * H * W * 3));
    MARK(0);
    const int Hp = 2 * d.H1 + 6, Wp = 2 * d.W1 + 6;
    const bool prep_in_stem = m->sw.fuse_prep && m->sw.fuse_stem_pool && pixel_format == OPD_PIXELS_U8_BGR_HWC;
    if (!prep_in_stem) {
        RCCHK(timed_begin(m, CLS_OTHER, 0.0));
        if (pixel_format == OPD_PIXELS_U8_BGR_HWC)
            HIPCHK(opd_launch_preprocess_u8(reinterpret_cast<const uint8_t*>(d_pixels), m->d_x4, B, H, W, Hp, Wp, d_valid, m->stream, m->dtype));
        else
            HIPCHK(opd_launch_preprocess_f32(reinterpret_cast<const float*>(d_pixels), m->d_x4, B, H, W, Hp, Wp, d_valid, m->stream, m->dtype));
        RCCHK(timed_end(m));
    }
    if (prep_in_stem) {
        RCCHK(timed_begin(m, CLS_CONV, 2.0 * B * d.H1 * d.W1 * 64.0 * 147.0));
        HIPCHK(opd_launch_stem_pool_u8(reinterpret_cast<const uint8_t*>(d_pixels), d_valid, m->stem.w, m->stem.bias, m->d_pool, B, H, W, d.H1, d.W1,
                                       d.H2, d.W2, m->stream, m->dtype));
        RCCHK(timed_end(m));
        RCCHK(tap(m, "stem_pool_u8", m->d_pool, (size_t)B * d.H2 * d.W2 * 64 * 2));
    } else if (m->sw.fuse_stem_pool) {
        RCCHK(timed_begin(m, CLS_CONV, 2.0 * B * d.H1 * d.W1 * 64.0 * 147.0));
        HIPCHK(opd_launch_stem_pool(m->d_x4, m->stem.w, m->stem.bias, m->d_pool, B, Hp, Wp, d.H1, d.W1, d.H2, d.W2, m->stream, m->dtype));
        RCCHK(timed_end(m));
    } else {
        ConvGemmParams p{}; p.dtype = m->dtype;
        p.x = m->d_x4; p.w = m->stem.w; p.bias = m->stem.bias; p.out = m->d_stem; p.zero16 = m->zero_bias;
        p.B = B; p.H = Hp; p.W = Wp; p.Cin = 256; p.OH = d.H1; p.OW = d.W1; p.N = 64; p.KH = 1; p.KW = 1; p.stride = 2; p.pad = 0;
        p.M = B * d.H1 * d.W1; p.K = 256; p.relu = 1; p.stem = 2;
        RCCHK(timed_begin(m, CLS_CONV, 2.0 * p.M * 64.0 * 147.0));
        HIPCHK(opd_launch_conv_gemm(p, m->stream));
        RCCHK(timed_end(m));
        RCCHK(timed_begin(m, CLS_OTHER, 0.0));
        HIPCHK(opd_launch_maxpool(m->d_stem, m->d_pool, B, d.H1, d.W1, 64, d.H2, d.W2, m->stream, m->dtype));
        RCCHK(timed_end(m));
    }
    MARK(1);
    const TrunkPlan tp = plan_trunk(a, m->blocks, m->cfg, m->sw, B, d.H2, d.W2, m->num_cus, m->taps != 0, m->profiling, m->stream2 != nullptr);
    struct TrunkState { int cur_id; int ch, cw; int z_id; int prev_id; };
    auto run_blocks = [&](int s_begin, int s_end, int b0, int nb, TrunkState& st, int l_begin = 0, int l_end = 1 << 30) -> int {
        auto trunk = [&](int id, size_t per_frame) { return (id == 0 ? m->d_pool : id == 1 ? m->d_t0 : m->d_t1) + (size_t)b0 * per_frame; };
        auto mid = [&](int id, size_t per_frame) { return (id ? m->d_m1 : m->d_m0) + (size_t)b0 * per_frame; };
        for (int s = s_begin; s < s_end; ++s) {
            for (int l = l_begin; l < a.depths[s] && l < l_end; ++l) {
                const int bi = m->stage_first[s] + l;
                const Block& b = m->blocks[bi];
                const TrunkStep& t = tp.steps[bi];
                const int ch = st.ch, cw = st.cw;
                const int oh = (b.c1.stride == 2) ? down2(ch) : ch, ow = (b.c1.stride == 2) ? down2(cw) : cw;
                const int C1 = b.c1.Cin, C2 = b.c2.Cout, C3 = t.C3;
                const f16_t* cur = trunk(st.cur_id, (size_t)ch * cw * b.c0.Cin);
                const int out_id = st.cur_id == 1 ? 2 : 1;
                f16_t* out = trunk(out_id, (size_t)oh * ow * C2);
                f16_t* const scb = m->d_sc + (size_t)b0 * oh * ow * C2;
                if (t.sc == SC_LAUNCH) RCCHK(run_conv(m, b.sc, cur, nb, ch, cw, oh, ow, scb, false, nullptr));
                const f16_t* res = t.res == RES_TRUNK ? cur : t.res == RES_SHORTCUT ? scb : nullptr;
                int x1_id = st.z_id;
                const f16_t* x1 = nullptr;
                if (x1_id >= 0) {
                    x1 = mid(x1_id, (size_t)ch * cw * C1);
                } else {
                    x1_id = 0;
                    f16_t* c0out = mid(0, (size_t)ch * cw * b.c0.Cout);
                    RCCHK(run_conv(m, b.c0, cur, nb, ch, cw, ch, cw, c0out, true, nullptr, (l == 0 && s > 0) ? s - 1 : s));
                    x1 = c0out;
                }
                st.z_id = -1;
                if (t.path == PATH_TAIL) {
                    const Block* nbk = C3 ? &m->blocks[bi + 1] : nullptr;
                    BtailParams p{}; p.dtype = m->dtype;
                    p.x1 = x1; p.w1 = b.c1.w; p.b1 = b.c1.bias; p.w2p = C1 == 256 ? b.c2.wp : b.c2.w; p.b2 = b.c2.bias; p.res = res;
                    p.y = t.store == STORE_A1 ? nullptr : out;
                    if (t.sc == SC_TAIL) { p.xs = cur; p.wsc = b.sc.w; p.b2 = b.bias2sc; }
                    f16_t* z = mid(1 - x1_id, (size_t)oh * ow * C3);
                    if (C3) { p.w3p = C1 == 256 ? nbk->c0.wp : nbk->c0.w; p.b3 = nbk->c0.bias; p.z = z; }
                    f16_t* const a1_keep = m->d_sc + (size_t)b0 * oh * ow * C1;
                    if (t.store == STORE_A1) p.a1_out = a1_keep;
                    if (t.res == RES_REBUILD) {
                        const Block& pb = m->blocks[bi - 1];
                        p.rc = 1; p.rc_a1 = a1_keep; p.rc_xs = trunk(st.prev_id, (size_t)ch * cw * pb.c0.Cin); p.rc_w2 = pb.c2.w; p.rc_wsc = pb.sc.w; p.rc_b = pb.bias2sc;
                    }
                    p.y_stride2 = t.store == STORE_Y_STRIDE2;
                    p.B = nb; p.H = ch; p.W = cw; p.OH = oh; p.OW = ow; p.stride = b.c1.stride; p.M = nb * oh * ow; p.C1 = C1; p.C3 = C3;
                    p.rev = b0 ? t.rev_b : t.rev;
                    p.dbg = m->sw.dbg_btail;
                    RCCHK(timed_begin(m, CLS_CONV, 2.0 * p.M * ((double)C1 * 9 * C1 + 4.0 * C1 * C1 + 4.0 * C1 * C3 + (t.sc == SC_TAIL ? 64.0 * 256 : 0.0))));
                    HIPCHK(opd_launch_btail(p, m->stream));
                    RCCHK(timed_end(m));
                    if (p.y) RCCHK(tap(m, "btail_y", out, (size_t)p.M * 4 * C1 * 2));
                    if (C3) RCCHK(tap(m, "btail_z", z, (size_t)p.M * C3 * 2));
                    if (C3) st.z_id = 1 - x1_id;
                } else {
                    f16_t* a1 = mid(1 - x1_id, (size_t)oh * ow * C1);
                    RCCHK(run_conv(m, b.c1, x1, nb, ch, cw, oh, ow, a1, true, nullptr, s));
                    if (t.path == PATH_DUAL) {
                        ConvGemmParams p{}; p.dtype = m->dtype;
                        p.x = a1; p.w = b.w2sc; p.bias = b.bias2sc; p.out = out; p.zero16 = m->zero_bias;
                        p.B = nb; p.H = oh; p.W = ow; p.Cin = C1; p.OH = oh; p.OW = ow; p.N = C2; p.KH = 1; p.KW = 1; p.stride = 1; p.pad = 0;
                        p.M = nb * oh * ow; p.K1 = C1; p.K = C1 + b.sc.Cin; p.relu = 1;
                        p.x2 = cur; p.H2 = ch; p.W2 = cw; p.Cin2 = b.sc.Cin; p.stride2 = b.sc.stride; p.dbg = m->sw.dbg_gemm; p.wprefetch = m->sw.wprefetch & 1;
                        RCCHK(timed_begin(m, CLS_CONV, 2.0 * p.M * (double)C2 * p.K));
                        HIPCHK(opd_launch_conv_gemm(p, m->stream));
                        RCCHK(timed_end(m));
                        RCCHK(tap(m, "dual_expand", out, (size_t)p.M * C2 * 2));
                    } else {
                        RCCHK(run_conv(m, b.c2, a1, nb, oh, ow, oh, ow, out, true, res));
                    }
                }
                st.prev_id = st.cur_id; st.cur_id = out_id; st.ch = oh; st.cw = ow;
            }
            if (b0 + nb == B && l_end >= a.depths[s]) MARK(2 + s);
        }
        return OPD_OK;
    };
    TrunkState st{0, d.H2, d.W2, -1, -1};
    RCCHK(run_blocks(0, 2, 0, B, st));
    const int nbA = tp.split;
    RCCHK(run_blocks(2, 3, 0, B, st, 0, 1));
    if (nbA < B) {
        TrunkState ta = st, tb = st;
        HIPCHK(hipEventRecord(m->ev_fork, m->stream));
        HIPCHK(hipStreamWaitEvent(m->stream2, m->ev_fork, 0));
        hipStream_t main_stream = m->stream;
        const int rc_a = run_blocks(2, 3, 0, nbA, ta, 1);
        m->stream = m->stream2;
        const int rc_b = rc_a == OPD_OK ? run_blocks(2, 3, nbA, B - nbA, tb, 1) : OPD_OK;
        m->stream = main_stream;
        const hipError_t ej = hipEventRecord(m->ev_join, m->stream2);
        const hipError_t ew = ej == hipSuccess ? hipStreamWaitEvent(m->stream, m->ev_join, 0) : ej;
        RCCHK(rc_a);
        RCCHK(rc_b);
        HIPCHK(ew);
        MARK(4);
        st = ta;
    } else {
        RCCHK(run_blocks(2, 3, 0, B, st, 1));
    }
    RCCHK(run_blocks(3, 4, 0, B, st));
    const f16_t* cur = st.cur_id == 1 ? m->d_t0 : m->d_t1;
    const int ch = st.ch, cw = st.cw;
    const int hw = ch * cw, M = B * hw, D = a.d_model, F = a.ffn;
    const bool shadow = m->sw.pos_shadow && D == 256 && m->enc[0].bqkv && m->bkv_all;
    const PosShadow psh{plan->d_pos, pos_ptrs, hw, m->d_xp16};
    const PosShadow* ps = shadow ? &psh : nullptr;
    auto run_deep = [&](const f16_t* x, const Lin* lin, const f16_t* w, const float* bias, int K, const float* res32, const LNp* ln, int cls) -> int {
        GemmLnParams gp{}; gp.dtype = m->dtype;
        gp.x = x; gp.w = w; gp.bias = bias; gp.res32 = res32; gp.gamma = ln ? ln->g : nullptr; gp.beta = ln ? ln->b : nullptr;
        gp.y32 = m->d_x32; gp.y16 = m->d_x16; gp.M = M; gp.K = K; gp.deep_k = 1;
        if (ps) { gp.pos = ps->pos; gp.pos_ptrs = ps->pos_ptrs; gp.pos_period = ps->period; gp.yp16 = ps->yp16; }
        RCCHK(timed_begin(m, cls, 2.0 * M * (double)D * K));
        HIPCHK(opd_launch_gemm_ln(gp, m->stream));
        RCCHK(timed_end(m));
        RCCHK(tap(m, ln ? "fc2_ln_ring" : "input_proj_ring", m->d_x32, (size_t)M * D * 4));
        (void)lin;
        return OPD_OK;
    };
    const bool small_enc = m->sw.small_enc && (size_t)m->cfg.max_batch * m->stage_px[3] <= 1400;
    const int enc_splits = small_enc ? 8 : 4;
    const bool deep_ok = m->sw.deep_fc2 && D == 256 && !small_enc;
    if (deep_ok && m->proj.K % 64 == 0 && (size_t)M * m->proj.K * 2 < 0x7fffff00ull)
        RCCHK(run_deep(cur, nullptr, m->proj.w, m->proj.bias, m->proj.K, nullptr, nullptr, CLS_CONV));
    else
        RCCHK(run_gemm_splitk_ln(m, cur, m->proj.w, m->proj.bias, M, D, m->proj.K, (m->proj.K / 64) % enc_splits == 0 ? enc_splits : 4, nullptr, nullptr, m->d_x32, m->d_x16, CLS_CONV, ps));
    bool qkv_done = false, kv_done = false;
    const int Q = a.queries, Md = B * Q, NKV = a.dec_layers * 2 * D;
    for (int i = 0; i < a.enc_layers; ++i) {
        const EncLayer& L = m->enc[i];
        if (qkv_done) {
        } else if (shadow)
            RCCHK(run_gemm(m, m->d_xp16, L.wqkv, L.bqkv, 0, M, 3 * D, D, m->d_qkv16, false, false, nullptr, nullptr, 0, 0, m->d_x16, 3 * D, 2 * D));
        else
            RCCHK(run_gemm(m, m->d_x16, L.wqkv, plan->rb_enc[i], hw, M, 3 * D, D, m->d_qkv16, false, false, nullptr, enc_bias_ptrs[i], 3 * D, 2 * D));
        RCCHK(run_attn(m, m->d_qkv16, 3 * D, m->d_qkv16 + D, 3 * D, m->d_qkv16 + 2 * D, 3 * D, m->d_attn16, D, B, hw, hw, d_keyv, cw));
        const bool ffn_fused = m->sw.fused_enc_ffn && m->sw.fuse_gemm_ln && L.ffn_pack && D == 256 && !small_enc;
        const bool front = ffn_fused && L.front && m->sw.enc_front;
        if (front) {
        } else if (m->sw.fuse_gemm_ln && D == 256) {
            RCCHK(run_gemm_ln(m, m->d_attn16, L.o.w, L.o.b, M, D, m->d_x32, L.ln1, m->d_x32, m->d_x16));
        } else {
            RCCHK(run_gemm(m, m->d_attn16, L.o.w, L.o.b, 0, M, D, D, m->d_y32, true, false, m->d_x32));
            RCCHK(timed_begin(m, CLS_OTHER, 0.0));
            HIPCHK(opd_launch_layernorm(m->d_y32, L.ln1.g, L.ln1.b, m->d_x32, m->d_x16, M, m->stream, m->dtype));
            RCCHK(timed_end(m));
        }
        if (ffn_fused) {
            EncFfnParams fp{}; fp.dtype = m->dtype; fp.wprefetch = (m->sw.wprefetch >> 1) & 1;
            fp.x = m->d_x16; fp.wpack = L.ffn_pack; fp.b2 = L.fc2.b; fp.res32 = m->d_x32; fp.gamma = L.ln2.g; fp.beta = L.ln2.b;
            fp.y32 = m->d_x32; fp.y16 = m->d_x16; fp.M = M; fp.F = F; fp.pack_tail = L.tail; fp.pack_front = L.front;
            if (front) { fp.attn = m->d_attn16; fp.bo = L.o.b; fp.gamma1 = L.ln1.g; fp.beta1 = L.ln1.b; }
            if (ps) { fp.pos = ps->pos; fp.pos_ptrs = ps->pos_ptrs; fp.pos_period = ps->period; fp.yp16 = ps->yp16; }
            const bool last = i + 1 == a.enc_layers;
            qkv_done = false;
            if (ps && m->sw.enc_tail && L.tail && L.tail_ld == (last ? NKV : 3 * D) && (last ? (size_t)M * NKV * 2 < (1ull << 32) : true)) {
                fp.tail = L.tail; fp.tail_pos = L.tail_pos; fp.tail_ld = L.tail_ld;
                fp.tail_out = last ? m->d_memkv16 : m->d_qkv16;
                for (int t = 0; t < L.tail; ++t) fp.tail_col[t] = L.tail_col[t];
                (last ? kv_done : qkv_done) = true;
            }
            RCCHK(timed_begin(m, CLS_GEMM, 4.0 * M * (double)D * F + 2.0 * M * (double)D * 256 * (fp.tail + (front ? 1 : 0))));
            HIPCHK(opd_launch_enc_ffn(fp, m->stream));
            RCCHK(timed_end(m));
            RCCHK(tap(m, "enc_ffn", m->d_x32, (size_t)M * D * 4));
        } else {
            qkv_done = false;
            RCCHK(run_gemm(m, m->d_x16, L.fc1.w, L.fc1.b, 0, M, F, D, m->d_ffn16, false, true, nullptr));
            if (deep_ok && F % 64 == 0 && (size_t)M * F * 2 < 0x7fffff00ull) {
                RCCHK(run_deep(m->d_ffn16, nullptr, L.fc2.w, L.fc2.b, F, m->d_x32, &L.ln2, CLS_GEMM));
            } else {
                RCCHK(run_gemm_splitk_ln(m, m->d_ffn16, L.fc2.w, L.fc2.b, M, D, F, (F / 64) % enc_splits == 0 ? enc_splits : 4, m->d_x32, &L.ln2, m->d_x32, m->d_x16, CLS_GEMM, ps));
            }
        }
    }
    MARK(6);
    if (kv_done) {
    } else if (shadow)
        RCCHK(run_gemm(m, m->d_xp16, m->wkv_all, m->bkv_all, 0, M, NKV, D, m->d_memkv16, false, false, nullptr, nullptr, 0, 0, m->d_x16, 2 * D, D));
    else
        RCCHK(run_gemm(m, m->d_x16, m->wkv_all, plan->rb_kv, hw, M, NKV, D, m->d_memkv16, false, false, nullptr, kv_bias_ptrs, 2 * D, D));
    const bool dec0 = m->sw.fuse_dec0 && m->dec0_h && D == 256;
    const bool fused_dec = m->sw.fused_dec && dec0 && m->qc0 && a.heads == 8 && Q <= 128 && (Q & 3) == 0 && F % OPD_DEC_FFN_CHUNK == 0 && F / OPD_DEC_FFN_CHUNK <= 16 && m->sw.dec_splits <= 6 && D == 256 && m->dec[0].wqkv_f &&
                           (size_t)M * NKV * 2 < (1ull << 32);
    const float* dec_final_h = m->d_h32;
    if (fused_dec) {
        const int S = m->sw.dec_splits, nchunk = F / OPD_DEC_FFN_CHUNK;
        float* hbuf[2] = {m->d_h32, m->d_yd32};
        int cur = 0;
        for (int i = 0; i < a.dec_layers && i < m->sw.dbg_dec_layers; ++i) {
            const DecLayer& L = m->dec[i];
            f16_t* qd = m->d_qd16 + (size_t)i * m->cfg.max_batch * Q * D;
            if (i > 0) {
                const DecLayer& P = m->dec[i - 1];
                DecQkvParams qp{};
                qp.h_in = hbuf[cur]; qp.partials = m->d_ffn_part; qp.nsplit = nchunk; qp.b2 = P.fc2.b; qp.ln_g = P.ln3.g; qp.ln_b = P.ln3.b;
                qp.h_out = hbuf[cur ^ 1]; qp.w = L.wqkv_f; qp.bias = L.rb_self;
                qp.q16 = m->d_dq16; qp.k16 = m->d_dk16; qp.vT = m->d_dvT; qp.M = Md; qp.Q = Q;
                RCCHK(timed_begin(m, CLS_GEMM, 2.0 * Md * 768.0 * D));
                HIPCHK(opd_launch_dec_qkv(qp, m->stream));
                RCCHK(timed_end(m));
                cur ^= 1;
// ... 189 lines not shown
    if (pixels_on_device(mem_kind) && !device_accessible(pixels))
        return fail(OPD_EINVAL, "OPD_MEM_DEVICE: the pixel pointer is not device-accessible memory");
    const int edge = std::max(m->cfg.max_height, m->cfg.max_width);
    if (B < 1 || B > m->cfg.max_batch || H < 32 || W < 32 || H > edge || W > edge ||
        (size_t)H * W > (size_t)m->cfg.max_height * m->cfg.max_width)
        return fail(OPD_EINVAL, "frame batch [" + std::to_string(B) + "," + std::to_string(H) + "," + std::to_string(W) +
                                    "] outside the configured maximum [" + std::to_string(m->cfg.max_batch) + "," +
                                    std::to_string(m->cfg.max_height) + "," + std::to_string(m->cfg.max_width) + "] (either orientation)");
    return OPD_OK;
}

int stage_pixels(opd_detr* m, const void* pixels, int pixel_format, int mem_kind, int B, int H, int W, const void** d_pixels) {
    if (pixels_on_device(mem_kind)) { *d_pixels = pixels; return OPD_OK; }
    const size_t n = (size_t)B * H * W * 3;
    if (pixel_format == OPD_PIXELS_U8_BGR_HWC) {
        HIPCHK(hipMemcpyAsync(m->d_u8, pixels, n, hipMemcpyHostToDevice, m->stream));
        *d_pixels = m->d_u8;
    } else {
        HIPCHK(hipMemcpyAsync(m->d_pv, pixels, n * 4, hipMemcpyHostToDevice, m->stream));
        *d_pixels = m->d_pv;
    }
    return OPD_OK;
}

static int enqueue_resize(opd_detr* m, const uint8_t* frames, int mem_kind, int B, int h, int w, int oh, int ow, const uint8_t* const* list = nullptr) {
    if (h < 1 || w < 1 || (size_t)h * w > (size_t)1 << 26) return fail(OPD_EINVAL, "source frame size out of range");
    const size_t need = (size_t)B * h * w * 3;
    const uint8_t* d_in = frames;
    if (!pixels_on_device(mem_kind)) {
        if (need > m->src_bytes) {
            HIPCHK(hipStreamSynchronize(m->stream));
            if (m->d_src) (void)hipFree(m->d_src);
            m->d_src = nullptr; m->src_bytes = 0;
            void* q = nullptr;
            if (hipMalloc(&q, need) != hipSuccess) return fail(OPD_ENOMEM, "source frame staging allocation failed");
            m->d_src = reinterpret_cast<uint8_t*>(q);
            m->src_bytes = need;
        }
        if (list) {
            for (int b = 0; b < B; ++b) HIPCHK(hipMemcpyAsync(m->d_src + (size_t)b * h * w * 3, list[b], (size_t)h * w * 3, hipMemcpyHostToDevice, m->stream));
        } else {
            HIPCHK(hipMemcpyAsync(m->d_src, frames, need, hipMemcpyHostToDevice, m->stream));
        }
        d_in = m->d_src;
    }
    const opd_detr::ResizeTab* tab = nullptr;
    for (const auto& t : m->resize_tabs)
        if (t.h == h && t.w == w && t.oh == oh && t.ow == ow) tab = &t;
    if (!tab) {
        std::vector<int32_t> bh, kh, bv, kv;
        opd_detr::ResizeTab t{h, w, oh, ow, 0, 0, nullptr, nullptr, nullptr, nullptr};
        opd_resize_coeffs(w, ow, &bh, &kh, &t.ksh);
        opd_resize_coeffs(h, oh, &bv, &kv, &t.ksv);
        auto up = [&](const std::vector<int32_t>& v, int32_t** d) -> int {
            RCCHK(dalloc(m, d, v.size(), false));
            HIPCHK(hipMemcpy(*d, v.data(), v.size() * 4, hipMemcpyHostToDevice));
            return OPD_OK;
        };
        RCCHK(up(bh, &t.bh)); RCCHK(up(kh, &t.kh)); RCCHK(up(bv, &t.bv)); RCCHK(up(kv, &t.kv));
        m->resize_tabs.push_back(t);
        tab = &m->resize_tabs.back();
    }
    HIPCHK(opd_launch_resize_u8(d_in, m->d_u8, B, h, w, oh, ow, tab->bh, tab->kh, tab->ksh, tab->bv, tab->kv, tab->ksv, m->stream));
    return OPD_OK;
}

int enqueue_postprocess(opd_detr* m, float threshold, const int32_t* orig_hw, opd_det* dev_out, int32_t* dev_counts) {
    const int B = m->last_B;
    std::vector<int32_t> hw((size_t)B * 2);
    for (int b = 0; b < B; ++b) {
        hw[2 * b] = orig_hw ? orig_hw[2 * b] : m->last_H;
        hw[2 * b + 1] = orig_hw ? orig_hw[2 * b + 1] : m->last_W;
    }
    if (hw != m->h_orig_hw) {
        HIPCHK(hipStreamSynchronize(m->stream));
        m->h_orig_hw = hw;
        HIPCHK(hipMemcpyAsync(m->d_orig_hw, m->h_orig_hw.data(), m->h_orig_hw.size() * 4, hipMemcpyHostToDevice, m->stream));
    }
    PostParams pp{};
    pp.logits = m->d_logits; pp.boxes = m->d_boxes; pp.orig_hw = m->d_orig_hw;
    pp.records = dev_out ? dev_out : m->d_records;
    pp.counts = dev_counts ? dev_counts : m->d_counts;
    pp.B = B; pp.Q = m->arch.queries; pp.ncls = m->arch.ncls; pp.threshold = threshold;
    RCCHK(timed_begin(m, CLS_OTHER, 0.0));
    HIPCHK(opd_launch_postprocess(pp, m->stream));
    RCCHK(timed_end(m));
    MARK(8);
    return OPD_OK;
}

static int fetch_records(opd_detr* m, opd_det* out, int32_t* counts, int mem_kind, float* features = nullptr) {
    const int B = m->last_B, Q = m->arch.queries;
    if (!outputs_on_device(mem_kind)) {
        const size_t rec_bytes = (size_t)m->cfg.max_batch * Q * sizeof(opd_det);
        const size_t feat_off = reinterpret_cast<const char*>(m->d_feat_all) - reinterpret_cast<const char*>(m->d_records);
        const size_t feat_row = (size_t)Q * m->arch.d_model * 4;
        if (!m->sync_pinned) HIPCHK(hipHostMalloc(&m->sync_pinned, feat_off + (size_t)m->cfg.max_batch * feat_row, hipHostMallocDefault));
        HIPCHK(hipMemcpyAsync(m->sync_pinned, m->d_records, features ? feat_off + (size_t)B * feat_row : rec_bytes + (size_t)B * 4, hipMemcpyDeviceToHost, m->stream));
        HIPCHK(hipStreamSynchronize(m->stream));
        memcpy(out, m->sync_pinned, (size_t)B * Q * sizeof(opd_det));
        memcpy(counts, static_cast<char*>(m->sync_pinned) + rec_bytes, (size_t)B * 4);
        if (features) memcpy(features, static_cast<char*>(m->sync_pinned) + feat_off, (size_t)B * feat_row);
    }
    HIPCHK(hipStreamSynchronize(m->stream));
    if (m->profiling) {
        for (int i = 0; i < 8; ++i) {
            float ms = 0.f;
            hipEvent_t from = (i == 7 && m->profiling == 2 && m->graph_marks) ? m->ev[9] : m->ev[i];
            if (hipEventElapsedTime(&ms, from, m->ev[i + 1]) == hipSuccess) m->stage_ms[i] = ms;
            else (void)hipGetLastError();
        }
        if (m->profiling == 1) timed_collect(m);
    }
    return OPD_OK;
}

}

static hipError_t make_branch_stream(opd_detr* m) {
    hipError_t e = hipStreamCreateWithFlags(&m->stream2, hipStreamNonBlocking);
    if (e == hipSuccess) e = hipEventCreateWithFlags(&m->ev_fork, hipEventDisableTiming);
    if (e == hipSuccess) e = hipEventCreateWithFlags(&m->ev_join, hipEventDisableTiming);
    return e;
}
static void drop_streams(opd_detr* m) {
    if (m->ev_fork) (void)hipEventDestroy(m->ev_fork);
    if (m->ev_join) (void)hipEventDestroy(m->ev_join);
    if (m->stream2) (void)hipStreamDestroy(m->stream2);
    if (m->stream) (void)hipStreamDestroy(m->stream);
    m->ev_fork = m->ev_join = nullptr; m->stream2 = m->stream = nullptr;
}

static int create_impl(const opd_config* cfg, const char* weights_path, int device_ordinal, opd_detr** out);
static int clone_impl(const opd_detr* src, opd_detr** out);
template <typename F>
static int guarded(const char* what, F&& body) {
    try {
        return body();
    } catch (const std::bad_alloc&) {
        return fail(OPD_ENOMEM, std::string(what) + ": out of host memory");
    } catch (const std::out_of_range& e) {
        return fail(OPD_ESCHEMA, std::string(what) + ": weight file lacks a tensor the model needs (" + e.what() + ")");
    } catch (const std::exception& e) {
        return fail(OPD_EINVAL, std::string(what) + ": " + e.what());
    } catch (...) {
        return fail(OPD_EINVAL, std::string(what) + ": unknown C++ exception");
    }
}
static Switches read_switches(int flags) {
    Switches sw;
    auto env = [](const char* name, int* v) { if (const char* e = getenv(name)) *v = atoi(e); };
    env("OPD_DUAL_OVER_TAIL", &sw.dual_over_tail);
    env("OPD_TAIL_REV", &sw.tail_rev);
    env("OPD_TAIL3", &sw.tail3);
    env("OPD_TAIL_RC", &sw.tail_rc);
    sw.tail_rc = sw.tail_rc != 0;
    env("OPD_WPREFETCH", &sw.wprefetch);
    env("OPD_W8", &sw.w8);
    if (sw.w8 < 0) sw.w8 = (flags & OPD_FLAG_MULTI_STREAM) ? 1 : 0;
    env("OPD_SMALL_SPLITK", &sw.small_splitk);
    env("OPD_SMALL_ENC", &sw.small_enc);
    env("OPD_Y_STRIDE2", &sw.y_stride2);
    env("OPD_TAIL3_SPLIT", &sw.tail3_split);
    env("OPD_FUSE_PREP", &sw.fuse_prep);
    env("OPD_POS_SHADOW", &sw.pos_shadow);
    env("OPD_DEEP_FC2", &sw.deep_fc2);
    env("OPD_WROUND", &sw.wround);
    env("OPD_FUSED_DEC", &sw.fused_dec);
    env("OPD_FUSED_ENC_FFN", &sw.fused_enc_ffn);
    env("OPD_ENC_TAIL", &sw.enc_tail);
    env("OPD_ENC_FRONT", &sw.enc_front);
    env("OPD_HEADS2", &sw.heads2);
    env("OPD_DBG_DEC_LAYERS", &sw.dbg_dec_layers);
    env("OPD_DBG_BTAIL", &sw.dbg_btail);
    env("OPD_DBG_SKIP", &sw.dbg_skip);
    env("OPD_DBG_GEMM", &sw.dbg_gemm);
    return sw;
}

extern "C" {

const char* opd_version(void) { return "opd_hip 0.2 gfx950 (fp16 MFMA operands, fp32 accumulate; OPD_FLAG_BF16: bf16 operands)"; }

int opd_detr_create(const opd_config* cfg, const char* weights_path, int device_ordinal, opd_detr** out) {
    ApiScope api_scope;
    if (out) *out = nullptr;
    return guarded("opd_detr_create", [&] { return create_impl(cfg, weights_path, device_ordinal, out); });
}
int opd_detr_clone(const opd_detr* src, opd_detr** out) {
    ApiScope api_scope;
    if (out) *out = nullptr;
    return guarded("opd_detr_clone", [&] { return clone_impl(src, out); });
}
static int create_impl(const opd_config* cfg, const char* weights_path, int device_ordinal, opd_detr** out) {
    if (!cfg || !weights_path || !out) return fail(OPD_EINVAL, "opd_detr_create: null argument");
    if (cfg->struct_size != (int32_t)sizeof(opd_config)) return fail(OPD_EINVAL, "opd_config.struct_size mismatch");
    if (cfg->max_batch < 1 || cfg->max_height < 32 || cfg->max_width < 32) return fail(OPD_EINVAL, "opd_config maxima must be >= 1 x 32 x 32");
    *out = nullptr;
    StateDict sd;
    std::string err;
    int rc = load_safetensors(weights_path, &sd, &err);
    if (rc) return fail(rc, err);
    std::unique_ptr<opd_detr> m(new opd_detr());
    rc = infer_arch(sd, &m->arch, &err);
    if (rc) return fail(rc, err);
    m->cfg = *cfg;
    m->dtype = (cfg->flags & OPD_FLAG_BF16) ? OPD_DT_BF16 : OPD_DT_F16;
    m->sw = read_switches(cfg->flags);
    m->device = device_ordinal;
    int ndev = 0;
    if (hipGetDeviceCount(&ndev) != hipSuccess || ndev == 0)
        return fail(OPD_EHIP, "no HIP device visible (this library has no CPU fallback)");
    if (device_ordinal < 0 || device_ordinal >= ndev) return fail(OPD_EINVAL, "device_ordinal out of range");
    auto cleanup = [&](int code) {
        for (void* p : m->allocs) (void)hipFree(p);
        drop_streams(m.get());
        return code;
    };
    {
        hipError_t e = hipSetDevice(device_ordinal);
        if (e == hipSuccess) e = hipStreamCreateWithFlags(&m->stream, hipStreamNonBlocking);
        if (e == hipSuccess) e = make_branch_stream(m.get());
        if (e != hipSuccess) { drop_streams(m.get()); return fail(OPD_EHIP, std::string("device/stream setup failed: ") + hipGetErrorString(e)); }
        int cus = 0;
        if (hipDeviceGetAttribute(&cus, hipDeviceAttributeMultiprocessorCount, device_ordinal) == hipSuccess && cus > 0) m->num_cus = cus;
    }
    m->weights = std::make_shared<WeightSet>();
    m->weights->device = device_ordinal;
    if ((rc = build_weights(m.get(), sd))) return cleanup(rc);
    m->weights_sealed = true;
    if ((rc = build_workspace(m.get()))) return cleanup(rc);
    for (auto& e : m->ev)
        if (hipEventCreate(&e) != hipSuccess) return cleanup(fail(OPD_EHIP, "hipEventCreate failed"));
    *out = m.release();
    ++g_handle_epoch;
    return OPD_OK;
}

static int clone_impl(const opd_detr* src, opd_detr** out) {
    if (!src || !out) return fail(OPD_EINVAL, "opd_detr_clone: null argument");
    *out = nullptr;
    std::unique_ptr<opd_detr> m(new opd_detr());
    m->arch = src->arch; m->cfg = src->cfg; m->device = src->device; m->dtype = src->dtype;
    m->weights = src->weights; m->weights_sealed = true; m->weight_bytes = src->weight_bytes;
    m->stem = src->stem; m->blocks = src->blocks; m->stage_first = src->stage_first; m->proj = src->proj;
    m->enc = src->enc; m->dec = src->dec; m->wkv_all = src->wkv_all; m->bkv_all = src->bkv_all; m->dec_ln = src->dec_ln;
    m->wc = src->wc; m->bc = src->bc; m->w1 = src->w1; m->b1 = src->b1; m->w2 = src->w2; m->b2 = src->b2; m->w3 = src->w3; m->b3 = src->b3; m->wc_f = src->wc_f; m->w1_f = src->w1_f; m->w2_f = src->w2_f;
    m->zero_bias = src->zero_bias;
    m->h_enc_cat_w = src->h_enc_cat_w; m->h_enc_cat_b = src->h_enc_cat_b; m->h_kv_cat_w = src->h_kv_cat_w; m->h_kv_cat_b = src->h_kv_cat_b;
    m->dec0_h = src->dec0_h; m->qc0 = src->qc0;
    m->sw = src->sw; m->num_cus = src->num_cus;
    auto cleanup = [&](int code) {
        for (void* p : m->allocs) (void)hipFree(p);
        drop_streams(m.get());
        return code;
    };
    {
        hipError_t e = hipSetDevice(m->device);
        if (e == hipSuccess) e = hipStreamCreateWithFlags(&m->stream, hipStreamNonBlocking);
        if (e == hipSuccess) e = make_branch_stream(m.get());
        if (e != hipSuccess) { drop_streams(m.get()); return fail(OPD_EHIP, std::string("device/stream setup failed: ") + hipGetErrorString(e)); }
    }
    int rc;
    if ((rc = build_workspace(m.get()))) return cleanup(rc);
    for (auto& e : m->ev)
        if (hipEventCreate(&e) != hipSuccess) return cleanup(fail(OPD_EHIP, "hipEventCreate failed"));
    *out = m.release();
    ++g_handle_epoch;
    return OPD_OK;
}

void opd_detr_destroy(opd_detr* m) {
    ApiScope api_scope;
    if (!m) return;
    (void)hipSetDevice(m->device);
    if (m->stream) (void)hipStreamSynchronize(m->stream);
    comm_detach_all(m);
    for (void* p : m->allocs) (void)hipFree(p);
    if (m->d_src) (void)hipFree(m->d_src);
    for (auto& e : m->ev_async)
        if (e) (void)hipEventDestroy(e);
    for (auto& a : m->async_host)
        if (a.pinned) (void)hipHostFree(a.pinned);
    if (m->sync_pinned) { (void)hipHostFree(m->sync_pinned); m->sync_pinned = nullptr; }
    for (auto& e : m->ev)
        if (e) (void)hipEventDestroy(e);
    for (auto& e : m->event_pool) (void)hipEventDestroy(e);
    for (auto& g : m->graphs)
        if (g.exec) (void)hipGraphExecDestroy(g.exec);
    drop_streams(m);
    delete m;
    ++g_handle_epoch;
}

int opd_detr_info(const opd_detr* m, opd_model_info* info) {
    if (!m || !info) return fail(OPD_EINVAL, "opd_detr_info: null argument");
    for (int i = 0; i < 4; ++i) info->depths[i] = m->arch.depths[i];
    info->d_model = m->arch.d_model; info->heads = m->arch.heads; info->ffn_dim = m->arch.ffn;
    info->encoder_layers = m->arch.enc_layers; info->decoder_layers = m->arch.dec_layers;
    info->num_queries = m->arch.queries; info->num_classes_plus1 = m->arch.ncls;
    info->max_batch = m->cfg.max_batch; info->max_height = m->cfg.max_height; info->max_width = m->cfg.max_width;
    info->device_ordinal = m->device;
    info->weight_bytes_device = m->weight_bytes; info->workspace_bytes_device = m->workspace_bytes;
    return OPD_OK;
}

// ... 341 lines not shown
```

office_person_detection_vit_amd/csrc/opd_model.h:

```cpp
#pragma once
#include <math.h>
#include <stdlib.h>
#include <string.h>

#include <atomic>
#include <memory>
#include <mutex>
#include <shared_mutex>
#include <string>
#include <vector>

#include "../../include/opd_detr.h"
#include "opd_kernels.h"
#include "opd_loader.h"
#include "opd_host.h"

#define HIPCHK(expr)                                                                                           \
    do {                                                                                                       \
        hipError_t _e = (expr);                                                                                \
        if (_e != hipSuccess)                                                                                  \
            return opd::fail(OPD_EHIP, std::string(#expr) + " failed: " + hipGetErrorString(_e) + " (" + __FILE__ + \
                                           ":" + std::to_string(__LINE__) + ")");                              \
    } while (0)

#define RCCHK(expr)            \
    do {                       \
        int _rc = (expr);      \
        if (_rc != 0) return _rc; \
    } while (0)

namespace opd {



struct Conv {
    f16_t* w = nullptr;
    f16_t* wp = nullptr;
    float* bias = nullptr;
    int Cin = 0, Cout = 0, KH = 1, KW = 1, stride = 1, pad = 0, K = 0;
    bool stem = false;
};
struct Lin {
    f16_t* w = nullptr;
    float* b = nullptr;
    int N = 0, K = 0;
};
struct LNp {
    float* g = nullptr;
    float* b = nullptr;
};
struct Block {
    Conv c0, c1, c2, sc;
    bool has_sc = false;
    float* bias2sc = nullptr;
    f16_t* w2sc = nullptr;
};
inline bool conv_has_kperm(const Conv& c) { return c.KH == 1 && c.KW == 1 && c.Cin % 32 == 0 && c.Cin <= 1024; }
inline bool block_has_bias2sc(const Block& b) { return b.has_sc && b.sc.Cout == b.c2.Cout; }
inline bool block_has_w2sc(const Block& b) {
    return block_has_bias2sc(b) && b.sc.KH == 1 && b.c2.KH == 1 && b.c2.Cout % 128 == 0 && b.c2.Cin >= 128;
}
struct EncLayer {
    f16_t* wqkv = nullptr;
    float* bqkv = nullptr;
    Lin o, fc1, fc2;
    LNp ln1, ln2;
    unsigned char* ffn_pack = nullptr;
    int tail = 0, tail_pos = 0, tail_ld = 0;
    int front = 0;
    int tail_col[16] = {};
};
struct DecLayer {
    f16_t* wqkv = nullptr;
    f16_t* wq_c = nullptr;
    Lin so, co, fc1, fc2;
    LNp ln1, ln2, ln3;
    float* rb_self = nullptr;
    float* rb_q = nullptr;
    f16_t *wqkv_f = nullptr, *so_f = nullptr, *wqc_f = nullptr, *co_f = nullptr, *fc1_f = nullptr, *fc2_f = nullptr;
};

struct Plan {
    int fh = 0, fw = 0;
    int vh = 0, vw = 0;
    std::vector<float*> rb_enc;
    float* rb_kv = nullptr;
    float* d_pos = nullptr;
};

struct Dims {
    int B, H, W, H1, W1, H2, W2;
    int sh[4], sw[4];
};

inline int down2(int n) { return (n - 1) / 2 + 1; }

struct Switches {
    int small_m_gemm = 1;
    int fuse_gemm_ln = 1;
    int deep_fc2 = 1;
    int fuse_dec0 = 1;
    int enc_front = 1;
    int enc_tail = 0;
    int fused_enc_ffn = 1;
    int fused_dec = 1;
    int dec_splits = 3;
    int heads2 = 1;
    int fuse_btail = 1;
    int fuse_shortcut = 1;
    int dual_over_tail = 1;
    int tail_rev = 1;
    int tail3 = 1;
    int tail3_split = 1;
    int tail_rc = 1;
    int y_stride2 = 1;
    int wprefetch = 3;
    int w8 = -1;
    int small_splitk = 1;
    int small_enc = 1;
    int fuse_stem_pool = 1;
    int fuse_prep = 1;
    int pos_shadow = 1;
    int wround = 1;
    int dbg_btail = 0, dbg_gemm = 0;
    int dbg_dec_layers = 1 << 20;
    int dbg_skip = 0;
};

enum TrunkPath { PATH_TAIL, PATH_CONVS, PATH_DUAL };
enum TrunkShortcut { SC_NONE, SC_TAIL, SC_EXPAND, SC_LAUNCH };
enum TrunkResidual { RES_NONE, RES_TRUNK, RES_SHORTCUT, RES_REBUILD };
enum TrunkStore { STORE_Y, STORE_A1, STORE_Y_STRIDE2 };
struct TrunkStep {
    int path, sc, res, store;
    int C3;
    int rev, rev_b;
};
struct TrunkPlan {
    std::vector<TrunkStep> steps;
    int split = 0;
};
TrunkPlan plan_trunk(const Arch& a, const std::vector<Block>& blocks, const opd_config& cfg, const Switches& sw, int B, int H2, int W2, int num_cus,
                     bool taps, int profiling, bool has_stream2);

}

using namespace opd;

struct RedZoned { void* base; size_t bytes; int poison; };
struct WeightSet {
    std::vector<void*> allocs;
    std::vector<RedZoned> zoned;
    int device = 0;
    std::mutex plan_mu;
    std::vector<std::unique_ptr<Plan>> plans;
    ~WeightSet() {
        (void)hipSetDevice(device);
        for (void* p : allocs) (void)hipFree(p);
    }
};

struct opd_detr {
    Arch arch;
    opd_config cfg{};
    Switches sw;
    int dtype = 0;
    int device = 0;
    hipStream_t stream = nullptr;
    hipStream_t stream2 = nullptr;
    hipEvent_t ev_fork = nullptr, ev_join = nullptr;
    std::vector<void*> allocs;
    std::vector<RedZoned> zoned;
    std::shared_ptr<WeightSet> weights;
    bool weights_sealed = false;
    int64_t weight_bytes = 0, workspace_bytes = 0;

    Conv stem;
    std::vector<Block> blocks;
    std::vector<int> stage_first;
    Conv proj;
    std::vector<EncLayer> enc;
    std::vector<DecLayer> dec;
    f16_t* wkv_all = nullptr;
    float* bkv_all = nullptr;
    float* dec0_h = nullptr;
    f16_t* qc0 = nullptr;
    LNp dec_ln;
    float *wc = nullptr, *bc = nullptr, *w1 = nullptr, *b1 = nullptr, *w2 = nullptr, *b2 = nullptr, *w3 = nullptr, *b3 = nullptr;
    f16_t *wc_f = nullptr, *w1_f = nullptr, *w2_f = nullptr;
    float* zero_bias = nullptr;

    std::vector<std::vector<float>> h_enc_cat_w, h_enc_cat_b;
    std::vector<float> h_kv_cat_w, h_kv_cat_b;

    uint8_t* d_u8 = nullptr;
    float* d_pv = nullptr;
    f16_t *d_x4 = nullptr, *d_stem = nullptr, *d_pool = nullptr, *d_t0 = nullptr, *d_t1 = nullptr, *d_m0 = nullptr,
          *d_m1 = nullptr, *d_sc = nullptr;
    float *d_x32 = nullptr, *d_y32 = nullptr, *d_slab = nullptr;
    f16_t* d_xp16 = nullptr;
    f16_t *d_x16 = nullptr, *d_qkv16 = nullptr, *d_attn16 = nullptr, *d_ffn16 = nullptr, *d_memkv16 = nullptr;
    float *d_h32 = nullptr, *d_yd32 = nullptr, *d_hs32 = nullptr;
    f16_t *d_h16 = nullptr, *d_qkvd16 = nullptr, *d_qd16 = nullptr, *d_attnd16 = nullptr, *d_ffnd16 = nullptr;
    f16_t *d_dq16 = nullptr, *d_dk16 = nullptr, *d_dvT = nullptr;
    float *d_part_o = nullptr, *d_part_ml = nullptr, *d_ffn_part = nullptr;
    float *d_logits = nullptr, *d_boxes = nullptr;
    opd_det* d_records = nullptr;
    int32_t *d_counts = nullptr, *d_orig_hw = nullptr;
    int32_t *d_valid_hw = nullptr, *d_key_valid = nullptr;
    const float** d_bias_ptrs = nullptr;
    std::vector<int32_t> h_valid_hw, h_key_valid;
    std::vector<const float*> h_bias_ptrs;
    hipEvent_t ev_async[4] = {};
    unsigned async_next = 0;
    bool async_pending[4] = {};
    struct AsyncHost { void* pinned = nullptr; opd_det* out = nullptr; int32_t* counts = nullptr; int B = 0; };
    AsyncHost async_host[4];
    void* sync_pinned = nullptr;
    float* d_feat_all = nullptr;
    uint8_t* d_src = nullptr;
    size_t src_bytes = 0;
    struct ResizeTab { int h, w, oh, ow, ksh, ksv; int32_t *bh, *kh, *bv, *kv; };
    std::vector<ResizeTab> resize_tabs;
    float *d_amap = nullptr, *d_amap_stat = nullptr;
    int32_t* d_amap_sel = nullptr;
    bool last_ragged = false;
    int32_t* d_rois = nullptr;
    float* d_roi_out = nullptr;
    std::vector<int32_t> h_orig_hw;

    int last_B = 0, last_H = 0, last_W = 0, last_fh = 0, last_fw = 0;
    int profiling = 0;
    hipEvent_t ev[10] = {};
    bool graph_marks = false;
    float stage_ms[8] = {};
    size_t slab_floats = 0;
    size_t stage_px[4] = {};
    int num_cus = 256;

    struct GraphEntry { int B, H, W, fmt, fh, fw; const void* pixels; int uses; hipGraphExec_t exec; unsigned epoch; };
    std::vector<GraphEntry> graphs;

    struct Timed { int cls; hipEvent_t a, b; double flops; const char* name; };
    struct KernelRow { std::string name; int launches; float ms; double flops; };
    std::vector<KernelRow> ktable;
    std::vector<Timed> timed;
    std::vector<hipEvent_t> event_pool;
    size_t pool_next = 0;
    float class_ms[4] = {};
    int class_launches[4] = {};
    double class_flops[4] = {};

    std::vector<struct opd_comm*> comms;

    int taps = 0;
    unsigned long long* d_taps = nullptr;
    int tap_next = 0;
    std::vector<std::string> tap_names;
};
enum { OPD_MAX_TAPS = 512 };

namespace opd {

// ... 54 lines not shown
```

office_person_detection_vit_amd/csrc/opd_test_api.cpp:

```cpp
#include <string.h>

#include <string>
#include <cstring>
#include <vector>

#include "opd_model.h"

namespace {
int tfail(int code, const std::string& msg) {
    opd::g_err = msg;
    return code;
}
struct DevMem {
    std::vector<void*> ptrs;
    ~DevMem() {
        for (void* p : ptrs) (void)hipFree(p);
    }
    template <typename T>
    T* up(const T* host, size_t count) {
        void* d = nullptr;
        if (hipMalloc(&d, count * sizeof(T) + 16) != hipSuccess) return nullptr;
        ptrs.push_back(d);
        if (host && hipMemcpy(d, host, count * sizeof(T), hipMemcpyHostToDevice) != hipSuccess) return nullptr;
        return reinterpret_cast<T*>(d);
// ... 382 lines not shown
        if (C3) w3p.assign(w3, w3 + (size_t)C3 * C2);
    }
    BtailParams p{}; p.dtype = g_test_dtype;
    p.x1 = dm.up(x1, (size_t)B * H * W * C1);
    p.w1 = dm.up(w1, (size_t)C1 * 9 * C1);
    p.b1 = dm.up(b1, C1);
    p.w2p = dm.up(w2p.data(), w2p.size());
    p.b2 = dm.up(b2, C2);
    p.res = res ? dm.up(res, M * C2) : nullptr;
    p.y = dm.up<uint16_t>(nullptr, M * C2);
    p.w3p = C3 ? dm.up(w3p.data(), w3p.size()) : nullptr;
    p.b3 = C3 ? dm.up(b3, C3) : nullptr;
    p.z = C3 ? dm.up<uint16_t>(nullptr, M * C3) : nullptr;
    if (!p.x1 || !p.w1 || !p.b1 || !p.w2p || !p.b2 || !p.y || (res && !p.res) || (C3 && (!p.w3p || !p.b3 || !p.z)))
        return tfail(OPD_ENOMEM, "test alloc failed");
    p.B = B; p.H = H; p.W = W; p.OH = OH; p.OW = OW; p.stride = stride; p.M = (int)M; p.C1 = C1; p.C3 = C3;
    TCHK(opd_launch_btail(p, nullptr));
    TCHK(hipDeviceSynchronize());
    TCHK(hipMemcpy(y, p.y, M * C2 * 2, hipMemcpyDeviceToHost));
    if (C3) TCHK(hipMemcpy(z, p.z, M * C3 * 2, hipMemcpyDeviceToHost));
    return OPD_OK;
}

int opd_test_btail_repeat(const uint16_t* x1, const uint16_t* w1, const float* b1, const uint16_t* w2, const float* b2, const uint16_t* res,
                          const uint16_t* w3, const float* b3, int B, int H, int W, int C1, int C3, int reps, int* n_diff) {
    if (!opd_btail_supported(C1, C3) || !C3 || reps < 2 || !n_diff) return tfail(OPD_EINVAL, "btail_repeat: bad arguments");
    DevMem dm;
    const int C2 = 4 * C1;
    const size_t M = (size_t)B * H * W;
    std::vector<uint16_t> w2p((size_t)C2 * C1), w3p((size_t)C3 * C2);
    if (C1 == 256) {
        opd_permute_k32(w2, w2p.data(), C2, C1);
        opd_permute_k32(w3, w3p.data(), C3, C2);
    } else {
        w2p.assign(w2, w2 + (size_t)C2 * C1);
        w3p.assign(w3, w3 + (size_t)C3 * C2);
    }
    BtailParams p{}; p.dtype = g_test_dtype;
    p.x1 = dm.up(x1, M * C1); p.w1 = dm.up(w1, (size_t)C1 * 9 * C1); p.b1 = dm.up(b1, C1); p.w2p = dm.up(w2p.data(), w2p.size());
    p.b2 = dm.up(b2, C2); p.res = dm.up(res, M * C2); p.y = dm.up<uint16_t>(nullptr, M * C2); p.w3p = dm.up(w3p.data(), w3p.size());
    p.b3 = dm.up(b3, C3); p.z = dm.up<uint16_t>(nullptr, M * C3);
    const size_t noise_bytes = (size_t)256 << 20;
    unsigned char* noise = dm.up<unsigned char>(nullptr, 2 * noise_bytes);
    unsigned long long* sums = dm.up<unsigned long long>(nullptr, (size_t)reps * 2 * OPD_TAP_BLOCKS);
    if (!p.x1 || !p.w1 || !p.b1 || !p.w2p || !p.b2 || !p.res || !p.y || !p.w3p || !p.b3 || !p.z || !noise || !sums) return tfail(OPD_ENOMEM, "test alloc failed");
    p.B = B; p.H = H; p.W = W; p.OH = H; p.OW = W; p.stride = 1; p.M = (int)M; p.C1 = C1; p.C3 = C3;
    hipStream_t side = nullptr;
    TCHK(hipStreamCreateWithFlags(&side, hipStreamNonBlocking));
    for (int r = 0; r < reps; ++r) {
        p.rev = r & 1;
        (void)hipMemcpyAsync(noise + ((r & 1) ? noise_bytes : 0), noise + ((r & 1) ? 0 : noise_bytes), noise_bytes, hipMemcpyDeviceToDevice, side);
        TCHK(hipMemsetAsync(p.y, 0xff, M * C2 * 2, nullptr));
        TCHK(hipMemsetAsync(p.z, 0xff, M * C3 * 2, nullptr));
        TCHK(opd_launch_btail(p, nullptr));
        TCHK(opd_launch_checksum(p.y, M * C2 * 2, sums + (size_t)(2 * r) * OPD_TAP_BLOCKS, nullptr));
        TCHK(opd_launch_checksum(p.z, M * C3 * 2, sums + (size_t)(2 * r + 1) * OPD_TAP_BLOCKS, nullptr));
    }
    TCHK(hipDeviceSynchronize());
    (void)hipStreamDestroy(side);
    std::vector<unsigned long long> h((size_t)reps * 2 * OPD_TAP_BLOCKS);
    TCHK(hipMemcpy(h.data(), sums, h.size() * 8, hipMemcpyDeviceToHost));
    int diff = 0;
    for (int r = 1; r < reps; ++r)
        if (memcmp(h.data() + (size_t)(2 * r) * OPD_TAP_BLOCKS, h.data(), 2 * OPD_TAP_BLOCKS * 8) != 0) ++diff;
    *n_diff = diff;
    return OPD_OK;
}

int opd_test_btail_sc(const uint16_t* x1, const uint16_t* w1, const float* b1, const uint16_t* w2, const float* b2sc, const uint16_t* xs,
                      const uint16_t* wsc, const uint16_t* w3, const float* b3, uint16_t* y, uint16_t* z, int B, int H, int W) {
    DevMem dm;
    const int C1 = 64, C2 = 256, C3 = 64;
    const size_t M = (size_t)B * H * W;
    std::vector<uint16_t> w2p((size_t)C2 * C1), w3p((size_t)C3 * C2);
    if (C1 == 256) {
        opd_permute_k32(w2, w2p.data(), C2, C1);
        opd_permute_k32(w3, w3p.data(), C3, C2);
    } else {
        w2p.assign(w2, w2 + (size_t)C2 * C1);
        w3p.assign(w3, w3 + (size_t)C3 * C2);
    }
    BtailParams p{}; p.dtype = g_test_dtype;
    p.x1 = dm.up(x1, M * C1);
    p.w1 = dm.up(w1, (size_t)C1 * 9 * C1);
    p.b1 = dm.up(b1, C1);
    p.w2p = dm.up(w2p.data(), w2p.size());
    p.b2 = dm.up(b2sc, C2);
    p.xs = dm.up(xs, M * 64);
    p.wsc = dm.up(wsc, (size_t)C2 * 64);
    p.y = dm.up<uint16_t>(nullptr, M * C2);
    p.w3p = dm.up(w3p.data(), w3p.size());
    p.b3 = dm.up(b3, C3);
    p.z = dm.up<uint16_t>(nullptr, M * C3);
    if (!p.x1 || !p.w1 || !p.b1 || !p.w2p || !p.b2 || !p.xs || !p.wsc || !p.y || !p.w3p || !p.b3 || !p.z) return tfail(OPD_ENOMEM, "test alloc failed");
    p.B = B; p.H = H; p.W = W; p.OH = H; p.OW = W; p.stride = 1; p.M = (int)M; p.C1 = C1; p.C3 = C3;
    TCHK(opd_launch_btail(p, nullptr));
    TCHK(hipDeviceSynchronize());
    TCHK(hipMemcpy(y, p.y, M * C2 * 2, hipMemcpyDeviceToHost));
    TCHK(hipMemcpy(z, p.z, M * C3 * 2, hipMemcpyDeviceToHost));
    return OPD_OK;
}

int opd_test_btail_chain(const uint16_t* x1, const uint16_t* xs, const uint16_t* const* w1, const float* const* b1, const uint16_t* const* w2,
                         const float* const* b2, const uint16_t* wsc, const uint16_t* const* w3, const float* const* b3, uint16_t* const* yb,
                         uint16_t* const* zb, uint16_t* const* yc, uint16_t* const* zc, int B, int H, int W, int fill) {
    DevMem dm;
    const size_t M = (size_t)B * H * W;
    const uint16_t* d_x1 = dm.up(x1, M * 64);
    const uint16_t* d_xs = dm.up(xs, M * 64);
    const uint16_t* d_wsc = dm.up(wsc, (size_t)256 * 64);
    const uint16_t *d_w1[3], *d_w2[3], *d_w3[3];
    const float *d_b1[3], *d_b2[3], *d_b3[3];
    for (int i = 0; i < 3; ++i) {
        const int c3 = i == 2 ? 128 : 64;
        d_w1[i] = dm.up(w1[i], (size_t)64 * 9 * 64); d_b1[i] = dm.up(b1[i], 64);
        d_w2[i] = dm.up(w2[i], (size_t)256 * 64); d_b2[i] = dm.up(b2[i], 256);
        d_w3[i] = dm.up(w3[i], (size_t)c3 * 256); d_b3[i] = dm.up(b3[i], c3);
        if (!d_w1[i] || !d_b1[i] || !d_w2[i] || !d_b2[i] || !d_w3[i] || !d_b3[i]) return tfail(OPD_ENOMEM, "test alloc failed");
    }
    uint16_t* ya = dm.up<uint16_t>(nullptr, M * 256);
    uint16_t* za = dm.up<uint16_t>(nullptr, M * 64);
    uint16_t* a1a = dm.up<uint16_t>(nullptr, M * 64);
    uint16_t* d_yb = dm.up<uint16_t>(nullptr, M * 256);
    uint16_t* d_zb = dm.up<uint16_t>(nullptr, M * 64);
    uint16_t* d_yc = dm.up<uint16_t>(nullptr, M * 256);
    uint16_t* d_zc = dm.up<uint16_t>(nullptr, M * 128);
    if (!d_x1 || !d_xs || !d_wsc || !ya || !za || !a1a || !d_yb || !d_zb || !d_yc || !d_zc) return tfail(OPD_ENOMEM, "test alloc failed");
    for (int route = 0; route < 2; ++route) {
        TCHK(hipMemset(ya, 0xEE, M * 256 * 2));
        TCHK(hipMemset(d_yc, fill, M * 256 * 2));
        auto base = [&](int i, const uint16_t* in, uint16_t* y, uint16_t* z, int c3) {
            BtailParams p{}; p.dtype = g_test_dtype;
            p.x1 = in; p.w1 = d_w1[i]; p.b1 = d_b1[i]; p.w2p = d_w2[i]; p.b2 = d_b2[i]; p.y = y; p.w3p = d_w3[i]; p.b3 = d_b3[i]; p.z = z;
            p.B = B; p.H = H; p.W = W; p.OH = H; p.OW = W; p.stride = 1; p.M = (int)M; p.C1 = 64; p.C3 = c3;
            return p;
        };
        BtailParams pa = base(0, d_x1, ya, za, 64);
        pa.xs = d_xs; pa.wsc = d_wsc;
        if (route) { pa.y = nullptr; pa.a1_out = a1a; }
        TCHK(opd_launch_btail(pa, nullptr));
        BtailParams pb = base(1, za, d_yb, d_zb, 64);
        if (route) { pb.rc = 1; pb.rc_a1 = a1a; pb.rc_xs = d_xs; pb.rc_w2 = d_w2[0]; pb.rc_wsc = d_wsc; pb.rc_b = d_b2[0]; }
        else pb.res = ya;
        TCHK(opd_launch_btail(pb, nullptr));
        BtailParams pc = base(2, d_zb, d_yc, d_zc, 128);
        pc.y_stride2 = route;
        pc.res = d_yb;
        TCHK(opd_launch_btail(pc, nullptr));
        TCHK(hipDeviceSynchronize());
        TCHK(hipMemcpy(yb[route], d_yb, M * 256 * 2, hipMemcpyDeviceToHost));
        TCHK(hipMemcpy(zb[route], d_zb, M * 64 * 2, hipMemcpyDeviceToHost));
        TCHK(hipMemcpy(yc[route], d_yc, M * 256 * 2, hipMemcpyDeviceToHost));
        TCHK(hipMemcpy(zc[route], d_zc, M * 128 * 2, hipMemcpyDeviceToHost));
    }
    return OPD_OK;
}

int opd_test_trace_btail(int B, int H, int W, int C1, int C3, int dbg, unsigned long long* trace_out, int max_wgs, int* wgs_out) {
    if (!opd_btail_supported(C1, C3)) return tfail(OPD_EINVAL, "btail: unsupported (C1, C3)");
    DevMem dm;
    const int C2 = 4 * C1;
    const size_t M = (size_t)B * H * W;
    const int wgs = (int)((M + 127) / 128);
    if (wgs > max_wgs) return tfail(OPD_EINVAL, "trace buffer too small");
    uint16_t* x1 = dm.up<uint16_t>(nullptr, M * C1);
    uint16_t* w1 = dm.up<uint16_t>(nullptr, (size_t)C1 * 9 * C1);
    uint16_t* w2 = dm.up<uint16_t>(nullptr, (size_t)C2 * C1);
    uint16_t* w3 = dm.up<uint16_t>(nullptr, (size_t)C3 * C2);
    float* bias = dm.up<float>(nullptr, C2);
    uint16_t* res = dm.up<uint16_t>(nullptr, M * C2);
    uint16_t* y = dm.up<uint16_t>(nullptr, M * C2);
    uint16_t* z = dm.up<uint16_t>(nullptr, M * C3);
    unsigned long long* tr = dm.up<unsigned long long>(nullptr, (size_t)wgs * 16);
    if (!x1 || !w1 || !w2 || !w3 || !bias || !res || !y || !z || !tr) return tfail(OPD_ENOMEM, "trace alloc failed");
    TCHK(hipMemset(x1, 0x2c, M * C1 * 2));
    TCHK(hipMemset(w1, 0x1c, (size_t)C1 * 9 * C1 * 2));
    TCHK(hipMemset(w2, 0x1c, (size_t)C2 * C1 * 2));
    TCHK(hipMemset(w3, 0x1c, (size_t)C3 * C2 * 2));
    TCHK(hipMemset(bias, 0, (size_t)C2 * 4));
    TCHK(hipMemset(res, 0x2c, M * C2 * 2));
    TCHK(hipMemset(tr, 0, (size_t)wgs * 128));
    BtailParams p{}; p.dtype = g_test_dtype;
    p.x1 = x1; p.w1 = w1; p.b1 = bias; p.w2p = w2; p.b2 = bias; p.res = res; p.y = y; p.w3p = w3; p.b3 = bias; p.z = z;
    p.B = B; p.H = H; p.W = W; p.OH = H; p.OW = W; p.stride = 1; p.M = (int)M; p.C1 = C1; p.C3 = C3; p.dbg = dbg;
    for (int i = 0; i < 2; ++i) TCHK(opd_launch_btail(p, nullptr));
    p.trace = tr;
    TCHK(opd_launch_btail(p, nullptr));
    TCHK(hipDeviceSynchronize());
    TCHK(hipMemcpy(trace_out, tr, (size_t)wgs * 128, hipMemcpyDeviceToHost));
    *wgs_out = wgs;
    return OPD_OK;
}

int opd_test_bench_btail(int B, int H, int W, int C1, int C3, int stride, int dbg, int iters, float* us_out) {
    if (!opd_btail_supported(C1, C3)) return tfail(OPD_EINVAL, "btail: unsupported (C1, C3)");
    DevMem dm;
    const int C2 = 4 * C1, OH = (H - 1) / stride + 1, OW = (W - 1) / stride + 1;
    const size_t M = (size_t)B * OH * OW;
    uint16_t* x1 = dm.up<uint16_t>(nullptr, (size_t)B * H * W * C1);
    uint16_t* w1 = dm.up<uint16_t>(nullptr, (size_t)C1 * 9 * C1);
    uint16_t* w2 = dm.up<uint16_t>(nullptr, (size_t)C2 * C1);
    uint16_t* w3 = dm.up<uint16_t>(nullptr, (size_t)(C3 ? C3 : 64) * C2);
    float* bias = dm.up<float>(nullptr, C2);
    uint16_t* res = dm.up<uint16_t>(nullptr, M * C2);
    uint16_t* a1 = dm.up<uint16_t>(nullptr, M * C1);
    uint16_t* y = dm.up<uint16_t>(nullptr, M * C2);
    uint16_t* z = dm.up<uint16_t>(nullptr, M * (C3 ? C3 : 64));
    float* zero = dm.up<float>(nullptr, 4096);
    if (!x1 || !w1 || !w2 || !w3 || !bias || !res || !a1 || !y || !z || !zero) return tfail(OPD_ENOMEM, "bench alloc failed");
    TCHK(hipMemset(x1, 0x2c, (size_t)B * H * W * C1 * 2));
    TCHK(hipMemset(w1, 0x1c, (size_t)C1 * 9 * C1 * 2));
    TCHK(hipMemset(w2, 0x1c, (size_t)C2 * C1 * 2));
    TCHK(hipMemset(w3, 0x1c, (size_t)(C3 ? C3 : 64) * C2 * 2));
    TCHK(hipMemset(bias, 0, (size_t)C2 * 4));
    TCHK(hipMemset(res, 0x2c, M * C2 * 2));
    TCHK(hipMemset(zero, 0, 4096 * 4));
    BtailParams p{}; p.dtype = g_test_dtype;
    p.x1 = x1; p.w1 = w1; p.b1 = bias; p.w2p = w2; p.b2 = bias; p.res = res; p.y = y; p.w3p = w3; p.b3 = bias; p.z = z;
    p.B = B; p.H = H; p.W = W; p.OH = OH; p.OW = OW; p.stride = stride; p.M = (int)M; p.C1 = C1; p.C3 = C3; p.dbg = dbg;
    ConvGemmParams c[3] = {};
    c[0].x = x1; c[0].w = w1; c[0].out = a1; c[0].B = B; c[0].H = H; c[0].W = W; c[0].Cin = C1; c[0].OH = OH; c[0].OW = OW; c[0].N = C1;
    c[0].KH = c[0].KW = 3; c[0].stride = stride; c[0].pad = 1; c[0].K = 9 * C1;
    c[1].x = a1; c[1].w = w2; c[1].res16 = res; c[1].out = y; c[1].B = B; c[1].H = OH; c[1].W = OW; c[1].Cin = C1; c[1].OH = OH; c[1].OW = OW;
    c[1].N = C2; c[1].KH = c[1].KW = 1; c[1].stride = 1; c[1].K = C1;
    c[2].x = y; c[2].w = w3; c[2].out = z; c[2].B = B; c[2].H = OH; c[2].W = OW; c[2].Cin = C2; c[2].OH = OH; c[2].OW = OW; c[2].N = C3 ? C3 : 64;
    c[2].KH = c[2].KW = 1; c[2].stride = 1; c[2].K = C2;
    for (auto& q : c) { q.bias = bias; q.zero16 = zero; q.M = (int)M; q.relu = 1; }
    hipEvent_t ev[2];
    TCHK(hipEventCreate(&ev[0])); TCHK(hipEventCreate(&ev[1]));
    for (int k = 0; k < 4; ++k) {
        if (k == 3 && !C3) { us_out[3] = 0.f; break; }
        if (k > 0 && dbg) { us_out[k] = 0.f; continue; }
        for (int i = -2; i < iters; ++i) {
            if (i == 0) TCHK(hipEventRecord(ev[0], nullptr));
            if (k == 0) TCHK(opd_launch_btail(p, nullptr));
            else TCHK(opd_launch_conv_gemm(c[k - 1], nullptr));
        }
        TCHK(hipEventRecord(ev[1], nullptr));
        TCHK(hipEventSynchronize(ev[1]));
        float ms = 0.f;
        TCHK(hipEventElapsedTime(&ms, ev[0], ev[1]));
        us_out[k] = ms * 1000.f / iters;
    }
    (void)hipEventDestroy(ev[0]); (void)hipEventDestroy(ev[1]);
    return OPD_OK;
}

int opd_test_bench_attention(const uint16_t* q, const uint16_t* k, const uint16_t* v, int B, int heads, int Lq, int Lk, int ldq, int ldkv,
                             float scale, int iters, float* us_out) {
    DevMem dm;
    AttnParams p{}; p.dtype = g_test_dtype;
    p.q = dm.up(q, (size_t)B * Lq * ldq);
    p.k = dm.up(k, (size_t)B * Lk * ldkv);
    p.v = dm.up(v, (size_t)B * Lk * ldkv);
    p.o = dm.up<uint16_t>(nullptr, (size_t)B * Lq * heads * 32);
    if (!p.q || !p.k || !p.v || !p.o) return tfail(OPD_ENOMEM, "bench alloc failed");
    p.B = B; p.heads = heads; p.Lq = Lq; p.Lk = Lk; p.ldq = ldq; p.ldk = p.ldv = ldkv; p.ldo = heads * 32; p.scale = scale;
    hipEvent_t a, b;
    TCHK(hipEventCreate(&a)); TCHK(hipEventCreate(&b));
    for (int i = 0; i < 3; ++i) TCHK(opd_launch_attention(p, nullptr));
    TCHK(hipEventRecord(a, nullptr));
    for (int i = 0; i < iters; ++i) TCHK(opd_launch_attention(p, nullptr));
    TCHK(hipEventRecord(b, nullptr));
    TCHK(hipEventSynchronize(b));
    float ms = 0.f;
    TCHK(hipEventElapsedTime(&ms, a, b));
    (void)hipEventDestroy(a); (void)hipEventDestroy(b);
    *us_out = ms * 1000.f / iters;
    return OPD_OK;
}

int opd_test_trace_attention(const uint16_t* q, const uint16_t* k, const uint16_t* v, int B, int heads, int Lq, int Lk, int ldq, int ldkv,
                             float scale, unsigned long long* trace_out, int max_wgs, int* wgs_out) {
    DevMem dm;
    AttnParams p{}; p.dtype = g_test_dtype;
    p.q = dm.up(q, (size_t)B * Lq * ldq);
    p.k = dm.up(k, (size_t)B * Lk * ldkv);
    p.v = dm.up(v, (size_t)B * Lk * ldkv);
    p.o = dm.up<uint16_t>(nullptr, (size_t)B * Lq * heads * 32);
    const int total = ((Lq + 63) / 64) * heads * B, grid = 8 * ((total + 7) / 8);
    unsigned long long* tr = dm.up<unsigned long long>(nullptr, (size_t)grid * 12);
    if (!p.q || !p.k || !p.v || !p.o || !tr) return tfail(OPD_ENOMEM, "trace alloc failed");
    TCHK(hipMemset(tr, 0, (size_t)grid * 96));
    p.B = B; p.heads = heads; p.Lq = Lq; p.Lk = Lk; p.ldq = ldq; p.ldk = p.ldv = ldkv; p.ldo = heads * 32; p.scale = scale;
    for (int i = 0; i < 2; ++i) TCHK(opd_launch_attention(p, nullptr));
    p.trace = tr;
    TCHK(opd_launch_attention(p, nullptr));
    TCHK(hipDeviceSynchronize());
    const int n = grid < max_wgs ? grid : max_wgs;
    TCHK(hipMemcpy(trace_out, tr, (size_t)n * 96, hipMemcpyDeviceToHost));
    *wgs_out = n;
    return OPD_OK;
}

int opd_test_attention(const uint16_t* q, const uint16_t* k, const uint16_t* v, uint16_t* o, int B, int heads, int Lq, int Lk,
                       float scale) {
    DevMem dm;
    const int D = heads * 32;
    AttnParams p{}; p.dtype = g_test_dtype;
    p.q = dm.up(q, (size_t)B * Lq * D);
    p.k = dm.up(k, (size_t)B * Lk * D);
    p.v = dm.up(v, (size_t)B * Lk * D);
    p.o = dm.up<uint16_t>(nullptr, (size_t)B * Lq * D);
    if (!p.q || !p.k || !p.v || !p.o) return tfail(OPD_ENOMEM, "test alloc failed");
    p.B = B; p.heads = heads; p.Lq = Lq; p.Lk = Lk; p.ldq = p.ldk = p.ldv = p.ldo = D; p.scale = scale;
    TCHK(opd_launch_attention(p, nullptr));
// ... 71 lines not shown
    p.out = dm.up<uint16_t>(nullptr, M * 64);
    if (!p.x || !p.w || !p.bias || !p.zero16 || !p.out) return tfail(OPD_ENOMEM, "test alloc failed");
    p.B = B; p.H = Hp; p.W = Wp; p.Cin = 256; p.OH = OH; p.OW = OW; p.N = 64; p.KH = 1; p.KW = 1; p.stride = 2; p.pad = 0;
    p.M = (int)M; p.K = 256; p.relu = 1; p.stem = 2;
    TCHK(opd_launch_conv_gemm(p, nullptr));
    TCHK(hipDeviceSynchronize());
    TCHK(hipMemcpy(out, p.out, M * 64 * 2, hipMemcpyDeviceToHost));
    return OPD_OK;
}

int opd_test_stem_pool(const uint16_t* x4p, const uint16_t* w, const float* bias, uint16_t* out, int B, int Hp, int Wp, int OH, int OW,
                       int PH, int PW) {
    DevMem dm;
    const uint16_t* dx = dm.up(x4p, (size_t)B * Hp * Wp * 4);
    const uint16_t* dw = dm.up(w, (size_t)64 * 256);
    const float* db = dm.up(bias, 64);
    uint16_t* dout = dm.up<uint16_t>(nullptr, (size_t)B * PH * PW * 64);
    if (!dx || !dw || !db || !dout) return tfail(OPD_ENOMEM, "test alloc failed");
    TCHK(opd_launch_stem_pool(dx, dw, db, dout, B, Hp, Wp, OH, OW, PH, PW, nullptr));
    TCHK(hipDeviceSynchronize());
    TCHK(hipMemcpy(out, dout, (size_t)B * PH * PW * 64 * 2, hipMemcpyDeviceToHost));
    return OPD_OK;
}

int opd_test_stem_pool_u8(const uint8_t* frames, const int32_t* valid_hw, const uint16_t* w, const float* bias, uint16_t* out_fused,
                          uint16_t* out_split, int B, int H, int W) {
    DevMem dm;
    const int OH = (H - 1) / 2 + 1, OW = (W - 1) / 2 + 1, PH = (OH - 1) / 2 + 1, PW = (OW - 1) / 2 + 1, Hp = 2 * OH + 6, Wp = 2 * OW + 6;
    const uint8_t* df = dm.up(frames, (size_t)B * H * W * 3);
    const int32_t* dv = valid_hw ? dm.up(valid_hw, (size_t)2 * B) : nullptr;
    const uint16_t* dw = dm.up(w, (size_t)64 * 256);
    const float* db = dm.up(bias, 64);
    uint16_t* dx = dm.up<uint16_t>(nullptr, (size_t)B * Hp * Wp * 4);
    uint16_t* d1 = dm.up<uint16_t>(nullptr, (size_t)B * PH * PW * 64);
    uint16_t* d2 = dm.up<uint16_t>(nullptr, (size_t)B * PH * PW * 64);
    if (!df || !dw || !db || !dx || !d1 || !d2 || (valid_hw && !dv)) return tfail(OPD_ENOMEM, "test alloc failed");
    TCHK(opd_launch_stem_pool_u8(df, dv, dw, db, d1, B, H, W, OH, OW, PH, PW, nullptr));
    TCHK(opd_launch_preprocess_u8(df, dx, B, H, W, Hp, Wp, dv, nullptr));
    TCHK(opd_launch_stem_pool(dx, dw, db, d2, B, Hp, Wp, OH, OW, PH, PW, nullptr));
    TCHK(hipDeviceSynchronize());
    TCHK(hipMemcpy(out_fused, d1, (size_t)B * PH * PW * 64 * 2, hipMemcpyDeviceToHost));
    TCHK(hipMemcpy(out_split, d2, (size_t)B * PH * PW * 64 * 2, hipMemcpyDeviceToHost));
    return OPD_OK;
}

static int g_test_heads2 = 1;
int opd_test_set_heads2(int on) { g_test_heads2 = on; return OPD_OK; }
static bool heads_frags(DevMem& dm, HeadParams& p, const float* wc, const float* w1, const float* w2, int ncls) {
    if (!g_test_heads2 || ncls > 128) return true;
    std::vector<float> wcp((size_t)128 * 256, 0.f);
    std::copy(wc, wc + (size_t)ncls * 256, wcp.begin());
    std::vector<uint16_t> f((size_t)2 * 128 * 256);
    opd_split_f16_frag(wcp.data(), 128, 256, f.data());
    p.wc_f = dm.up(f.data(), f.size());
    std::vector<uint16_t> f2((size_t)2 * 256 * 256);
    opd_split_f16_frag(w1, 256, 256, f2.data());
    p.w1_f = dm.up(f2.data(), f2.size());
    opd_split_f16_frag(w2, 256, 256, f2.data());
    p.w2_f = dm.up(f2.data(), f2.size());
    return p.wc_f && p.w1_f && p.w2_f;
}
int opd_test_heads(const float* hs, const float* ln_g, const float* ln_b, const float* wc, const float* bc, const float* w1, const float* b1,
                   const float* w2, const float* b2, const float* w3, const float* b3, float* logits, float* boxes, int rows, int ncls) {
    DevMem dm;
    auto tr = [&](const float* w, int O, int I) -> const float* {
        std::vector<float> t((size_t)O * I);
        for (int o = 0; o < O; ++o)
            for (int i = 0; i < I; ++i) t[(size_t)i * O + o] = w[(size_t)o * I + i];
        return dm.up(t.data(), t.size());
    };
    HeadParams p{};
    p.hs = dm.up(hs, (size_t)rows * 256);
    p.ln_gamma = ln_g ? dm.up(ln_g, 256) : nullptr;
    p.ln_beta = ln_b ? dm.up(ln_b, 256) : nullptr;
    p.wc = tr(wc, ncls, 256); p.bc = dm.up(bc, ncls);
    p.w1 = tr(w1, 256, 256); p.b1 = dm.up(b1, 256);
    p.w2 = tr(w2, 256, 256); p.b2 = dm.up(b2, 256);
    p.w3 = tr(w3, 4, 256); p.b3 = dm.up(b3, 4);
    p.logits = dm.up<float>(nullptr, (size_t)rows * ncls);
    p.boxes = dm.up<float>(nullptr, (size_t)rows * 4);
    if (!p.hs || !p.wc || !p.bc || !p.w1 || !p.b1 || !p.w2 || !p.b2 || !p.w3 || !p.b3 || !p.logits || !p.boxes) return tfail(OPD_ENOMEM, "test alloc failed");
    p.rows = rows; p.ncls = ncls;
    if (!heads_frags(dm, p, wc, w1, w2, ncls)) return tfail(OPD_ENOMEM, "test alloc failed");
    TCHK(opd_launch_heads(p, nullptr));
    TCHK(hipDeviceSynchronize());
    TCHK(hipMemcpy(logits, p.logits, (size_t)rows * ncls * 4, hipMemcpyDeviceToHost));
    TCHK(hipMemcpy(boxes, p.boxes, (size_t)rows * 4 * 4, hipMemcpyDeviceToHost));
    return OPD_OK;
}

int opd_test_postprocess(const float* logits, const float* boxes, const int32_t* orig_hw, int B, int Q, int ncls, float threshold,
                         opd_det* records, int32_t* counts) {
    DevMem dm;
    PostParams p{};
    p.logits = dm.up(logits, (size_t)B * Q * ncls);
    p.boxes = dm.up(boxes, (size_t)B * Q * 4);
    p.orig_hw = dm.up(orig_hw, (size_t)B * 2);
    opd_det* rec = dm.up<opd_det>(nullptr, (size_t)B * Q);
    p.counts = dm.up<int32_t>(nullptr, B);
    if (!p.logits || !p.boxes || !p.orig_hw || !rec || !p.counts) return tfail(OPD_ENOMEM, "test alloc failed");
    TCHK(hipMemset(rec, 0, (size_t)B * Q * sizeof(opd_det)));
    p.records = rec; p.B = B; p.Q = Q; p.ncls = ncls; p.threshold = threshold;
    TCHK(opd_launch_postprocess(p, nullptr));
    TCHK(hipDeviceSynchronize());
    TCHK(hipMemcpy(records, rec, (size_t)B * Q * sizeof(opd_det), hipMemcpyDeviceToHost));
    TCHK(hipMemcpy(counts, p.counts, (size_t)B * 4, hipMemcpyDeviceToHost));
    return OPD_OK;
}

int opd_test_roi_features(const float* enc, const int32_t* rois, int n, int h, int w, float* out) {
    DevMem dm;
    const float* d_enc = dm.up(enc, (size_t)h * w * 256);
    const int32_t* d_rois = dm.up(rois, (size_t)n * 4);
    float* d_out = dm.up<float>(nullptr, (size_t)n * 256);
    if (!d_enc || !d_rois || !d_out) return tfail(OPD_ENOMEM, "test alloc failed");
    TCHK(opd_launch_roi_features(d_enc, d_rois, d_out, n, h, w, nullptr));
    TCHK(hipDeviceSynchronize());
    TCHK(hipMemcpy(out, d_out, (size_t)n * 256 * 4, hipMemcpyDeviceToHost));
    return OPD_OK;
}

uint16_t opd_test_f32_to_f16(float f) { return opd::f32_to_f16(f); }
float opd_test_f16_to_f32(uint16_t h) { return opd::f16_to_f32(h); }
int opd_test_normalise_key(const char* in, char* out, int cap) {
    const std::string k = opd::normalise_key(in);
    if ((int)k.size() + 1 > cap) return OPD_EINVAL;
    memcpy(out, k.c_str(), k.size() + 1);
    return OPD_OK;
}
int opd_test_inspect_checkpoint(const char* path, int32_t* info8) {
    opd::StateDict sd;
    std::string err;
    int rc = opd::load_safetensors(path, &sd, &err);
    if (rc) return tfail(rc, err);
    opd::Arch a;
    rc = opd::infer_arch(sd, &a, &err);
    if (rc) return tfail(rc, err);
    for (int i = 0; i < 4; ++i) info8[i] = a.depths[i];
    info8[4] = a.enc_layers; info8[5] = a.dec_layers; info8[6] = a.queries; info8[7] = a.ncls;
    return OPD_OK;
}


int opd_test_resize_coeffs(int in_size, int out_size, int32_t* bounds, int32_t* coeffs, int coeffs_capacity) {
    std::vector<int32_t> b, k;
    int ksize = 0;
    opd_resize_coeffs(in_size, out_size, &b, &k, &ksize);
    if ((int)k.size() > coeffs_capacity) return fail(OPD_EINVAL, "coefficient buffer too small");
    memcpy(bounds, b.data(), b.size() * 4);
    memcpy(coeffs, k.data(), k.size() * 4);
    return ksize;
}
int opd_test_valid_prefix(int valid, int in, int out) { return valid_prefix(valid, in, out); }
int opd_test_trunk_plan(const int* depths, int max_batch, int flags, int B, int H, int W, int num_cus, int* steps_out, int max_steps, int* split_out) {
    if (!depths || !steps_out || !split_out || B < 1 || H < 1 || W < 1 || num_cus < 1) return tfail(OPD_EINVAL, "bad trunk_plan arguments");
    Arch a;
    std::vector<Block> blocks;
    auto conv = [](int cin, int cout, int k, int stride) {
        Conv c;
        c.Cin = cin; c.Cout = cout; c.KH = c.KW = k; c.stride = stride; c.pad = k / 2; c.K = k * k * cin;
        return c;
    };
    for (int s = 0, cin = 64; s < 4; ++s) {
        a.depths[s] = depths[s];
        if (depths[s] < 1) return tfail(OPD_EINVAL, "every stage needs a block");
        const int cout = a.hidden[s], mid = cout / 4;
        for (int l = 0; l < depths[s]; ++l) {
            const int stride = (l == 0 && s > 0) ? 2 : 1;
            Block b;
            b.has_sc = l == 0;
            if (b.has_sc) b.sc = conv(cin, cout, 1, stride);
            b.c0 = conv(cin, mid, 1, 1); b.c1 = conv(mid, mid, 3, stride); b.c2 = conv(mid, cout, 1, 1);
            blocks.push_back(b);
            cin = cout;
        }
    }
    if ((int)blocks.size() > max_steps) return tfail(OPD_EINVAL, "steps_out too small");
    opd_config cfg{};
    cfg.struct_size = sizeof(opd_config); cfg.max_batch = max_batch; cfg.max_height = H; cfg.max_width = W; cfg.flags = flags;
    const TrunkPlan plan = plan_trunk(a, blocks, cfg, Switches{}, B, down2(down2(H)), down2(down2(W)), num_cus, false, 0, true);
    for (size_t i = 0; i < plan.steps.size(); ++i) {
        const TrunkStep& t = plan.steps[i];
        const int row[7] = {t.path, t.sc, t.res, t.store, t.C3, t.rev, t.rev_b};
        memcpy(steps_out + 7 * i, row, sizeof(row));
    }
    *split_out = plan.split;
    return (int)blocks.size();
}
int opd_test_sine_pos_embed(int h, int w, int vh, int vw, int D, float* out) {
    if (!out || h < 1 || w < 1 || vh < 1 || vw < 1 || vh > h || vw > w || D < 2 || (D & 1)) return fail(OPD_EINVAL, "bad sine_pos_embed arguments");
    std::vector<float> pos;
    sine_pos_embed(h, w, vh, vw, D, &pos);
    memcpy(out, pos.data(), pos.size() * sizeof(float));
    return OPD_OK;
}
int opd_test_set_fuse_gemm_ln(opd_detr* m, int on) {
    if (!m) return fail(OPD_EINVAL, "null model handle");
    m->sw.fuse_gemm_ln = on ? 1 : 0;
    m->sw.small_m_gemm = on ? 1 : 0;
    m->sw.deep_fc2 = on ? 1 : 0;
    m->sw.fuse_dec0 = on ? 1 : 0;
    m->sw.fused_dec = on ? 1 : 0;
    if (fill_qc0(m) != OPD_OK) return OPD_EHIP;
    for (auto& g : m->graphs)
        if (g.exec) (void)hipGraphExecDestroy(g.exec);
    m->graphs.clear();
    return OPD_OK;
}
int opd_test_set_fuse_btail(opd_detr* m, int on) {
    if (!m) return fail(OPD_EINVAL, "null model handle");
    m->sw.fuse_btail = (on & 1) ? 1 : 0;
    m->sw.fuse_shortcut = (on & 2) ? 1 : 0;
    for (auto& g : m->graphs)
        if (g.exec) (void)hipGraphExecDestroy(g.exec);
    m->graphs.clear();
    return OPD_OK;
}
int opd_test_set_pos_shadow(opd_detr* m, int on) {
    if (!m) return fail(OPD_EINVAL, "null model handle");
    m->sw.pos_shadow = on ? 1 : 0;
    for (auto& g : m->graphs)
        if (g.exec) (void)hipGraphExecDestroy(g.exec);
    m->graphs.clear();
    return OPD_OK;
}
int opd_test_set_fuse_stem_pool(opd_detr* m, int on) {
    if (!m) return fail(OPD_EINVAL, "null model handle");
    m->sw.fuse_stem_pool = (on & 1) ? 1 : 0;
    m->sw.fuse_prep = (on & 2) ? 1 : 0;
    for (auto& g : m->graphs)
        if (g.exec) (void)hipGraphExecDestroy(g.exec);
    m->graphs.clear();
    return OPD_OK;
}

int opd_test_set_alloc_poison(int byte) {
    g_alloc_poison = byte < 0 ? -1 : (byte & 255);
    return OPD_OK;
}
int opd_test_check_redzones(opd_detr* m) {
    ApiScope api_scope;
    if (!m) return fail(OPD_EINVAL, "null model handle");
    HIPCHK(hipSetDevice(m->device));
    HIPCHK(hipDeviceSynchronize());
    std::vector<unsigned char> h(OPD_REDZONE);
    int bad = 0;
    std::string first;
    auto scan = [&](const std::vector<RedZoned>& v, const char* what) -> int {
        for (size_t i = 0; i < v.size(); ++i)
            for (int side = 0; side < 2; ++side) {
                const char* z = static_cast<const char*>(v[i].base) + (side ? OPD_REDZONE + v[i].bytes : 0);
                HIPCHK(hipMemcpy(h.data(), z, OPD_REDZONE, hipMemcpyDeviceToHost));
                size_t lo = OPD_REDZONE, hi = 0;
                for (size_t k = 0; k < OPD_REDZONE; ++k)
                    if (h[k] != (unsigned char)v[i].poison) { lo = std::min(lo, k); hi = k; }
                if (lo <= hi) {
                    if (!bad++) first = std::string(what) + " buffer #" + std::to_string(i) + " (" + std::to_string(v[i].bytes) + " bytes): " +
                                        (side ? "zone BEHIND it" : "zone IN FRONT of it") + " overwritten at zone offsets " + std::to_string(lo) + " .. " + std::to_string(hi);
                }
            }
        return OPD_OK;
    };
    RCCHK(scan(m->zoned, "handle"));
    if (m->weights) RCCHK(scan(m->weights->zoned, "weight-set"));
    if (bad) g_err = first;
    return bad;
}
int opd_test_set_graph_guard(int on) {
    g_graph_guard = on ? 1 : 0;
    return OPD_OK;
}
int opd_test_set_taps(opd_detr* m, int on) {
    ApiScope api_scope;
    if (!m) return fail(OPD_EINVAL, "null model handle");
    HIPCHK(hipSetDevice(m->device));
    if (on && !m->d_taps) RCCHK(dalloc(m, &m->d_taps, (size_t)OPD_MAX_TAPS * OPD_TAP_BLOCKS, false));
    m->taps = on ? 1 : 0;
    for (auto& g : m->graphs)
        if (g.exec) (void)hipGraphExecDestroy(g.exec);
    m->graphs.clear();
    return OPD_OK;
}
int opd_test_read_taps(opd_detr* m, unsigned long long* sums, int cap, char* names, int names_cap) {
    ApiScope api_scope;
    if (!m || !sums || !m->d_taps) return fail(OPD_EINVAL, "opd_test_read_taps: taps are not enabled");
    HIPCHK(hipSetDevice(m->device));
    HIPCHK(hipStreamSynchronize(m->stream));
    const int n = std::min(cap, (int)m->tap_names.size());
    std::vector<unsigned long long> h((size_t)n * OPD_TAP_BLOCKS);
    if (n) HIPCHK(hipMemcpy(h.data(), m->d_taps, h.size() * 8, hipMemcpyDeviceToHost));
    std::string all;
    for (int i = 0; i < n; ++i) {
        unsigned long long s = 0;
        for (int j = 0; j < OPD_TAP_BLOCKS; ++j) s += h[(size_t)i * OPD_TAP_BLOCKS + j];
        sums[i] = s;
        all += m->tap_names[i];
        all += '\n';
    }
    if (names && names_cap > 0) { strncpy(names, all.c_str(), (size_t)names_cap - 1); names[names_cap - 1] = 0; }
    return n;
}




static const f16_t* up_frag(DevMem& dm, const float* w, int N, int K) {
    std::vector<f16_t> f((size_t)N * K * 2);
    opd_split_f16_frag(w, N, K, f.data());
    return dm.up(f.data(), f.size());
}
int opd_test_dec_qkv(const float* h_in, const float* partials, int nsplit, const float* b2, const float* ln_g, const float* ln_b, const float* w,
                     const float* bias, int M, int Q, float* h_out, uint16_t* q16, uint16_t* k16, uint16_t* vT) {
    DevMem dm;
    DecQkvParams p{};
    const size_t n = (size_t)M * 256, nv = (size_t)(M / Q) * 8 * 8 * 512;
    if (partials) {
        p.h_in = dm.up(h_in, n); p.partials = dm.up(partials, n * nsplit); p.nsplit = nsplit; p.b2 = dm.up(b2, 256); p.ln_g = dm.up(ln_g, 256); p.ln_b = dm.up(ln_b, 256);
        p.h_out = dm.up<float>(nullptr, n);
        if (!p.h_in || !p.partials || !p.b2 || !p.ln_g || !p.ln_b) return tfail(OPD_ENOMEM, "test alloc failed");
    } else {
        p.h_out = dm.up(const_cast<const float*>(h_in), n);
    }
    p.w = up_frag(dm, w, 768, 256);
    if (!p.w) return tfail(OPD_ENOMEM, "test alloc failed");
    p.bias = dm.up(bias, (size_t)Q * 768);
    p.q16 = dm.up<uint16_t>(nullptr, n); p.k16 = dm.up<uint16_t>(nullptr, nv); p.vT = dm.up<uint16_t>(nullptr, nv);
    if (!p.h_out || !p.bias || !p.q16 || !p.k16 || !p.vT) return tfail(OPD_ENOMEM, "test alloc failed");
    TCHK(hipMemset(p.vT, 0, nv * 2));
    TCHK(hipMemset(p.k16, 0, nv * 2));
    p.M = M; p.Q = Q;
    TCHK(opd_launch_dec_qkv(p, nullptr));
    TCHK(hipDeviceSynchronize());
    TCHK(hipMemcpy(h_out, p.h_out, n * 4, hipMemcpyDeviceToHost));
// ... 185 lines not shown
```

Before: 2968.

## Fuse stride-2 shortcut conv into bottleneck tail for stage-2 transition block

Adds a transition variant of the bottleneck-tail kernel for the first block of the 128-channel stage. It folds the stride-2 1x1 shortcut projection from the 256-channel input into the expand GEMM's K loop, loading the strided input rows directly into registers. It also chains the next block's reduce conv as before. This removes a separate shortcut launch plus the write and re-read of its residual tensor. In exchange it uses a tighter two-phase LDS staging scheme and more registers. The planner enables it by default unless multi-stream mode is set.

```diff
diff --git a/office_person_detection_vit_amd/_capi.py b/office_person_detection_vit_amd/_capi.py
--- a/office_person_detection_vit_amd/_capi.py
+++ b/office_person_detection_vit_amd/_capi.py
@@ -149,6 +149,8 @@
     "opd_test_conv_dual": (C.c_int, [C.c_void_p] * 6 + [C.c_int] * 13),
     "opd_test_btail_sc": (C.c_int, [C.c_void_p] * 11 + [C.c_int] * 3),
     "opd_test_btail_chain": (C.c_int, [C.c_void_p] * 13 + [C.c_int] * 4),
+    "opd_test_btail_trans": (C.c_int, [C.c_void_p] * 11 + [C.c_int] * 4 + [C.POINTER(C.c_float)]),
+    "opd_test_trunk_plan_trans": (C.c_int, [C.c_int, C.c_void_p] + [C.c_int] * 6 + [C.c_void_p, C.c_int, C.c_void_p]),
     "opd_test_bench_attention": (C.c_int, [C.c_void_p] * 3 + [C.c_int] * 6 + [C.c_float, C.c_int, C.POINTER(C.c_float)]),
     "opd_test_trace_attention": (C.c_int, [C.c_void_p] * 3 + [C.c_int] * 6 + [C.c_float, C.c_void_p, C.c_int, C.POINTER(C.c_int)]),
     "opd_test_heads": (C.c_int, [C.c_void_p] * 13 + [C.c_int] * 2),
diff --git a/office_person_detection_vit_amd/csrc/kernels_btail.hip b/office_person_detection_vit_amd/csrc/kernels_btail.hip
--- a/office_person_detection_vit_amd/csrc/kernels_btail.hip
+++ b/office_person_detection_vit_amd/csrc/kernels_btail.hip
@@ -63,7 +63,7 @@
 }
 __device__ __forceinline__ void compiler_fence() { asm volatile("" ::: "memory"); }
 
-template <int C1, int C3, bool RDMA, bool SC = false, bool TRACE = false, int RC = 0>
+template <int C1, int C3, bool RDMA, bool SC = false, bool TRACE = false, int RC = 0, bool TR = false>
 __global__ __launch_bounds__(64 * NW, 8 / NW) void btail_kernel(BtailParams p) {
 #if defined(__HIP_DEVICE_COMPILE__)
     unsigned long long tstamp[16] = {};
@@ -75,6 +75,7 @@
     static_assert(!RDMA || C1 == 64, "residual staging buffers are budgeted for C1 == 64 (80 KiB of LDS per workgroup)");
     static_assert(!RDMA || RC == 0, "a rebuilt residual is not staged");
     static_assert(!SC || (C1 == 64 && !RDMA), "fused shortcut: 64-channel tails only; it replaces the residual");
+    static_assert(!TR || (C1 == 128 && C3 == 128 && !RDMA && !SC && !TRACE && RC == 0), "transition tail: first block of stage 2");
     extern __shared__ __attribute__((aligned(16))) unsigned char smem[];
     constexpr int C2 = 4 * C1;
     constexpr int NT1 = C1 / 16;
@@ -91,7 +92,10 @@
     static_assert(W1_PIECES >= 1 && W2_PIECES >= 1 && (C3 == 0 || W3_PIECES >= 1), "every wave stages at least one piece of every operand");
     constexpr int NT3 = C3 / 16;
     constexpr int WSC_BYTES = SC ? 64 * ROW_BYTES : 0;
-    constexpr int CHUNK_BYTES = W2C_BYTES + C3 * ROW_BYTES + WSC_BYTES + RC_BYTES;
+    constexpr int CS = 2 * C1;
+    constexpr int TRH_BYTES = 64 * 128 * 2;
+    static_assert(!TR || (W2C_BYTES == TRH_BYTES && C3 * ROW_BYTES == TRH_BYTES), "transition tail: both phases stage two 16-KiB operands");
+    constexpr int CHUNK_BYTES = TR ? 2 * TRH_BYTES : W2C_BYTES + C3 * ROW_BYTES + WSC_BYTES + RC_BYTES;
     constexpr int STAGE_BYTES = (A_BYTES + C1 * ROW_BYTES) > CHUNK_BYTES ? (A_BYTES + C1 * ROW_BYTES) : CHUNK_BYTES;
     static_assert(RC == 0 || (RC == 1 && C1 == 64 && !RDMA && !SC), "residual rebuild: second block of stage 1");
 
@@ -110,9 +114,14 @@
     const __amdgpu_buffer_rsrc_t rsrc_w1 = __builtin_amdgcn_make_buffer_rsrc(const_cast<f16_t*>(p.w1), 0, (unsigned)(C1 * 9 * C1 * 2), 0x00020000);
     const __amdgpu_buffer_rsrc_t rsrc_w2 = __builtin_amdgcn_make_buffer_rsrc(const_cast<f16_t*>(p.w2p), 0, (unsigned)(C2 * C1 * 2), 0x00020000);
     const __amdgpu_buffer_rsrc_t rsrc_w3 = __builtin_amdgcn_make_buffer_rsrc(const_cast<f16_t*>(C3 ? p.w3p : p.w2p), 0, (unsigned)((C3 ? C3 : 1) * C2 * 2), 0x00020000);
-    const __amdgpu_buffer_rsrc_t rsrc_sc = __builtin_amdgcn_make_buffer_rsrc(const_cast<f16_t*>(SC ? p.wsc : RC ? p.rc_wsc : p.w2p), 0, (unsigned)(C2 * 64 * 2), 0x00020000);
+    const __amdgpu_buffer_rsrc_t rsrc_sc = __builtin_amdgcn_make_buffer_rsrc(const_cast<f16_t*>((SC || TR) ? p.wsc : RC ? p.rc_wsc : p.w2p), 0, (unsigned)(C2 * (TR ? CS : 64) * 2), 0x00020000);
     const __amdgpu_buffer_rsrc_t rsrc_rw = __builtin_amdgcn_make_buffer_rsrc(const_cast<f16_t*>(RC ? p.rc_w2 : p.w2p), 0, (unsigned)(C2 * 64 * 2), 0x00020000);
-    unsigned rowoff[4], rowmask[4], woff1[W1_PIECES], woff2[W2_PIECES], woff3[W3_PIECES ? W3_PIECES : 1], woffsc[2];
+    unsigned rowoff[4], rowmask[4], woff1[W1_PIECES], woff2[W2_PIECES], woff3[W3_PIECES ? W3_PIECES : 1], woffsc[2], wofftr[4];
+#pragma unroll
+    for (int i = 0; i < 4; ++i) {
+        const int q = wave * 4 + i;
+        wofftr[i] = (unsigned)(own_row((q & 7) * 8 + lrow) * CS + (q >> 3) * 64) * 2u + (unsigned)lchunk * 16u;
+    }
 #pragma unroll
     for (int i = 0; i < 2; ++i)
         woffsc[i] = (unsigned)(own_row(((wave * SC_PIECES + i) & 7) * 8 + lrow) * 64) * 2u + (unsigned)lchunk * 16u;
@@ -204,6 +213,20 @@
             }
         }
     };
+    auto issue_tr = [&](int j, int ph, int buf) {
+        unsigned char* S = smem + buf * STAGE_BYTES;
+#pragma unroll
+        for (int i = 0; i < 4; ++i) {
+            if (ph == 0)
+                __builtin_amdgcn_raw_ptr_buffer_load_lds(rsrc_w2, (__attribute__((address_space(3))) void*)(S + (wave * 4 + i) * 1024), 16, woff2[i],
+                                                         j * (64 * C1 * 2), 0, 0);
+            __builtin_amdgcn_raw_ptr_buffer_load_lds(rsrc_sc, (__attribute__((address_space(3))) void*)(S + (ph ? 0 : TRH_BYTES) + (wave * 4 + i) * 1024),
+                                                     16, wofftr[i], j * (64 * CS * 2) + ph * 256, 0, 0);
+            if (ph == 1)
+                __builtin_amdgcn_raw_ptr_buffer_load_lds(rsrc_w3, (__attribute__((address_space(3))) void*)(S + TRH_BYTES + (wave * 4 + i) * 1024), 16,
+                                                         woff3[i], j * 128, 0, 0);
+        }
+    };
     const bool pr_ok[2] = {wm0 + li < p.M, wm0 + 16 + li < p.M};
     bool y_ok[2] = {pr_ok[0] && p.y != nullptr, pr_ok[1] && p.y != nullptr};
     if (p.y_stride2) {
@@ -227,7 +250,7 @@
             __builtin_amdgcn_raw_ptr_buffer_load_lds(rsrc_r, (__attribute__((address_space(3))) void*)(res_lds + (j & 1) * RES_BUF + i * 1024), 16,
                                                      res_voff + (unsigned)(i * 8 * C2 * 2), j * 128, 0, 0);
     };
-    const bool has_res = RC ? true : (!SC && p.res != nullptr && !(p.dbg & 4));
+    const bool has_res = RC ? true : (!SC && !TR && p.res != nullptr && !(p.dbg & 4));
     const bool res_dma = RDMA && has_res;
     auto load_res = [&](int j, uint4 (&r)[4]) {
         if constexpr (RDMA) {
@@ -260,6 +283,24 @@
             }
         }
     }
+    half8 xst[2][TR ? CS / 32 : 1];
+    if constexpr (TR) {
+#pragma unroll
+        for (int mt = 0; mt < 2; ++mt) {
+            const int m = wm0 + mt * 16 + li;
+            const int mm = m < p.M ? m : 0;
+            const int b = fdiv(mm, p.fd_ohw);
+            const int r = mm - b * (p.OH * p.OW);
+            const int oh = fdiv(r, p.fd_ow), ow = r - oh * p.OW;
+            const f16_t* src = p.xs + ((size_t)(b * p.xs_H + oh * p.xs_stride) * p.xs_W + ow * p.xs_stride) * CS + g * 8;
+#pragma unroll
+            for (int kk = 0; kk < CS / 32; ++kk) {
+                half8 v = {};
+                if (m < p.M) v = *reinterpret_cast<const half8*>(src + kk * 32);
+                xst[mt][kk] = v;
+            }
+        }
+    }
     stamp(2);
     issue_main(ks_first, ks_first & 1);
     float4v acc1[NT1][2];
@@ -293,9 +334,10 @@
         compute_main(ks & 1);
         __syncthreads();
     }
-    issue_chunk(0, nk & 1);
+    if constexpr (TR) issue_tr(0, 0, nk & 1);
+    else issue_chunk(0, nk & 1);
     compiler_fence();
-    if constexpr (RC == 0) {
+    if constexpr (RC == 0 && !TR) {
         load_res(0, res[0]);
         load_res(1, res[1]);
     }
@@ -339,6 +381,78 @@
     }
 
     if (p.dbg & 8) return;
+    if constexpr (TR) {
+        static_assert(!TR || (nk & 1) == 0, "phase buffers: chunk j's phase 0 follows an even number of steps");
+#pragma unroll
+        for (int j = 0; j < NCH; ++j) {
+            const unsigned char* Sa = smem + (nk & 1) * STAGE_BYTES;
+            const unsigned char* Sb = smem + ((nk & 1) ^ 1) * STAGE_BYTES;
+            issue_tr(j, 1, (nk & 1) ^ 1);
+            compiler_fence();
+            float4v acc2[4][2];
+#pragma unroll
+            for (int nt = 0; nt < 4; ++nt) {
+                const float4v b = *reinterpret_cast<const float4v*>(p.b2 + j * 64 + own_ch(nt, g));
+                acc2[nt][0] = b;
+                acc2[nt][1] = b;
+            }
+#pragma unroll
+            for (int kk = 0; kk < KK1 + 4; ++kk) {
+                half8 wf[4];
+#pragma unroll
+                for (int nt = 0; nt < 4; ++nt) wf[nt] = *reinterpret_cast<const half8*>(Sa + (kk >> 1) * 8192 + swz(nt * 16 + li, (kk & 1) * 4 + g));
+#pragma unroll
+                for (int nt = 0; nt < 4; ++nt)
+#pragma unroll
+                    for (int mt = 0; mt < 2; ++mt) acc2[nt][mt] = OPD_MFMA_16x16x32(wf[nt], kk < KK1 ? a1[mt][kk < KK1 ? kk : 0] : xst[mt][kk < KK1 ? 0 : kk - KK1], acc2[nt][mt]);
+            }
+            wait_vmcnt<0>();
+            __builtin_amdgcn_s_barrier();
+            if (j + 1 < NCH) issue_tr(j + 1, 0, nk & 1);
+            compiler_fence();
+#pragma unroll
+            for (int kk = 0; kk < 4; ++kk) {
+                half8 wf[4];
+#pragma unroll
+                for (int nt = 0; nt < 4; ++nt) wf[nt] = *reinterpret_cast<const half8*>(Sb + (kk >> 1) * 8192 + swz(nt * 16 + li, (kk & 1) * 4 + g));
+#pragma unroll
+                for (int nt = 0; nt < 4; ++nt)
+#pragma unroll
+                    for (int mt = 0; mt < 2; ++mt) acc2[nt][mt] = OPD_MFMA_16x16x32(wf[nt], xst[mt][4 + kk], acc2[nt][mt]);
+            }
+            half8 yf[2][2];
+#pragma unroll
+            for (int q = 0; q < 2; ++q)
+#pragma unroll
+                for (int mt = 0; mt < 2; ++mt) {
+                    float4v v0 = acc2[2 * q][mt], v1 = acc2[2 * q + 1][mt];
+#pragma unroll
+                    for (int r = 0; r < 4; ++r) {
+                        v0[r] = v0[r] > 0.f ? v0[r] : 0.f;
+                        v1[r] = v1[r] > 0.f ? v1[r] : 0.f;
+                    }
+                    yf[q][mt] = as_half8(pack2h(v0[0], v0[1]), pack2h(v0[2], v0[3]), pack2h(v1[0], v1[1]), pack2h(v1[2], v1[3]));
+                }
+#pragma unroll
+            for (int kk = 0; kk < 2; ++kk) {
+#pragma unroll
+                for (int nt = 0; nt < NT3; ++nt) {
+                    const half8 wf = *reinterpret_cast<const half8*>(Sb + TRH_BYTES + swz(nt * 16 + li, kk * 4 + g));
+#pragma unroll
+                    for (int mt = 0; mt < 2; ++mt) accz[nt][mt] = OPD_MFMA_16x16x32(wf, yf[kk][mt], accz[nt][mt]);
+                }
+            }
+            if (j + 1 < NCH) {
+                wait_vmcnt<0>();
+                __builtin_amdgcn_s_barrier();
+            }
+#pragma unroll
+            for (int q = 0; q < 2; ++q)
+#pragma unroll
+                for (int mt = 0; mt < 2; ++mt)
+                    if (y_ok[mt] && !(p.dbg & 2)) *reinterpret_cast<half8*>(p.y + pr_row[mt] + j * 64 + q * 32) = yf[q][mt];
+        }
+    } else
 #pragma unroll
     for (int j = 0; j < NCH; ++j) {
         const int buf = (nk + j) & 1;
@@ -498,15 +612,18 @@
 #endif
 }
 
-template <int C1, int C3, bool RDMA, bool SC = false, bool TRACE = false, int RC = 0>
+template <int C1, int C3, bool RDMA, bool SC = false, bool TRACE = false, int RC = 0, bool TR = false>
 hipError_t launch_btail_t(const BtailParams& p, hipStream_t stream) {
     constexpr int BM = 32 * NW;
-    constexpr int MAIN = (BM + C1) * ROW_BYTES, CHUNK = 64 * C1 * 2 + C3 * ROW_BYTES + (SC ? 64 * ROW_BYTES : 0) + (RC ? 2 * 64 * ROW_BYTES : 0);
+    constexpr int MAIN = (BM + C1) * ROW_BYTES;
+    constexpr int CHUNK = TR ? 4 * 64 * ROW_BYTES : 64 * C1 * 2 + C3 * ROW_BYTES + (SC ? 64 * ROW_BYTES : 0) + (RC ? 2 * 64 * ROW_BYTES : 0);
+    static_assert(!TR || 2 * (MAIN > CHUNK ? MAIN : CHUNK) <= 80 * 1024, "transition tail: two workgroups per CU");
     constexpr int LDS = 2 * (MAIN > CHUNK ? MAIN : CHUNK) + (RDMA ? 2 * NW * 4096 : 0);
     static_assert(LDS <= 160 * 1024, "LDS per workgroup");
-    OPD_SET_MAX_LDS_ONCE((btail_kernel<C1, C3, RDMA, SC, TRACE, RC>), LDS);
-    OPD_LAUNCH((btail_kernel<C1, C3, RDMA, SC, TRACE, RC>), dim3((p.M + BM - 1) / BM), dim3(64 * NW), LDS, stream, p);
-    static const char* const kname = opd_kernel_name("btail_kernel<%d, %d, %s, %s, %s, %d>", C1, C3, OPD_BOOLSTR(RDMA), OPD_BOOLSTR(SC), OPD_BOOLSTR(TRACE), RC);
+    OPD_SET_MAX_LDS_ONCE((btail_kernel<C1, C3, RDMA, SC, TRACE, RC, TR>), LDS);
+    OPD_LAUNCH((btail_kernel<C1, C3, RDMA, SC, TRACE, RC, TR>), dim3((p.M + BM - 1) / BM), dim3(64 * NW), LDS, stream, p);
+    static const char* const kname = opd_kernel_name("btail_kernel<%d, %d, %s, %s, %s, %d, %s>", C1, C3, OPD_BOOLSTR(RDMA), OPD_BOOLSTR(SC), OPD_BOOLSTR(TRACE), RC,
+                                                     OPD_BOOLSTR(TR));
     opd_last_kernel_name = kname;
     return hipGetLastError();
 }
@@ -535,6 +652,12 @@
             return hipErrorInvalidValue;
         return launch_btail_t<64, 64, false, false, false, 1>(p, stream);
     }
+    if (p.xs && p.C1 == 128) {
+        if (p.C3 != 128 || !p.wsc || p.res || !p.y || p.a1_out || p.y_stride2 || p.trace || p.xs_stride < 1 || p.xs_H < (p.OH - 1) * p.xs_stride + 1 ||
+            p.xs_W < (p.OW - 1) * p.xs_stride + 1)
+            return hipErrorInvalidValue;
+        return launch_btail_t<128, 128, false, false, false, 0, true>(p, stream);
+    }
     if (p.xs) {
         if (p.C1 != 64 || p.C3 != 64 || p.stride != 1 || !p.wsc || p.res || (size_t)p.M * 64 * 2 >= 0x7fffff00ull) return hipErrorInvalidValue;
         return launch_btail_t<64, 64, false, true>(p, stream);
diff --git a/office_person_detection_vit_amd/csrc/opd_kernels.h b/office_person_detection_vit_amd/csrc/opd_kernels.h
--- a/office_person_detection_vit_amd/csrc/opd_kernels.h
+++ b/office_person_detection_vit_amd/csrc/opd_kernels.h
@@ -113,6 +113,7 @@
     const float* rc_b;
     int rc;
     int y_stride2;
+    int xs_H, xs_W, xs_stride;
 };
 bool opd_btail_supported(int C1, int C3);
 hipError_t opd_launch_btail(const BtailParams& p, hipStream_t stream);
diff --git a/office_person_detection_vit_amd/csrc/opd_model.cpp b/office_person_detection_vit_amd/csrc/opd_model.cpp
--- a/office_person_detection_vit_amd/csrc/opd_model.cpp
+++ b/office_person_detection_vit_amd/csrc/opd_model.cpp
@@ -668,7 +668,10 @@
                                     nbk->c0.Cin == 256 && nbk->c0.Cout == 64;
             bool tail = sw.fuse_btail && b.c1.KH == 3 && b.c1.Cout == C1 && b.c2.Cin == C1 && b.c2.Cout == 4 * C1 && conv_has_kperm(b.c2) &&
                         opd_btail_supported(C1, 0);
-            if (sw.dual_over_tail && tail && b.has_sc && !sc_in_tail && block_has_w2sc(b)) tail = false;
+            const bool trans = sw.tail_trans > 0 && tail && sw.fuse_shortcut && !sc_in_tail && block_has_bias2sc(b) && C1 == 128 && b.c1.stride == 2 &&
+                               b.sc.KH == 1 && b.sc.stride == 2 && b.sc.Cin == 256 && b.c2.Cout == 512 && nbk && conv_has_kperm(nbk->c0) &&
+                               nbk->c0.Cin == 512 && nbk->c0.Cout == 128;
+            if (sw.dual_over_tail && tail && b.has_sc && !sc_in_tail && !trans && block_has_w2sc(b)) tail = false;
             if (C1 == 256 && tail) {
                 const long long tiles = ((long long)cfg.max_batch * oh * ow + 127) / 128;
                 const bool pays = tiles * 10 >= (long long)num_cus * 6;
@@ -678,7 +681,7 @@
             tail = tail && (size_t)B * ch * cw * C1 * 2 < 0x7ff00000ull;
             TrunkStep& t = plan.steps[bi];
             t.path = tail ? PATH_TAIL : sc_in_expand ? PATH_DUAL : PATH_CONVS;
-            t.sc = !b.has_sc ? SC_NONE : (sc_in_tail && tail) ? SC_TAIL : sc_in_expand ? SC_EXPAND : SC_LAUNCH;
+            t.sc = !b.has_sc ? SC_NONE : ((sc_in_tail || trans) && tail) ? SC_TAIL : sc_in_expand ? SC_EXPAND : SC_LAUNCH;
             t.res = (t.sc == SC_TAIL || t.sc == SC_EXPAND) ? RES_NONE : t.sc == SC_LAUNCH ? RES_SHORTCUT : RES_TRUNK;
             t.store = STORE_Y;
             t.C3 = 0;
@@ -844,7 +847,7 @@
                     BtailParams p{}; p.dtype = m->dtype;
                     p.x1 = x1; p.w1 = b.c1.w; p.b1 = b.c1.bias; p.w2p = C1 == 256 ? b.c2.wp : b.c2.w; p.b2 = b.c2.bias; p.res = res;
                     p.y = t.store == STORE_A1 ? nullptr : out;
-                    if (t.sc == SC_TAIL) { p.xs = cur; p.wsc = b.sc.w; p.b2 = b.bias2sc; }
+                    if (t.sc == SC_TAIL) { p.xs = cur; p.wsc = b.sc.w; p.b2 = b.bias2sc; p.xs_H = ch; p.xs_W = cw; p.xs_stride = b.sc.stride; }
                     f16_t* z = mid(1 - x1_id, (size_t)oh * ow * C3);
                     if (C3) { p.w3p = C1 == 256 ? nbk->c0.wp : nbk->c0.w; p.b3 = nbk->c0.bias; p.z = z; }
                     f16_t* const a1_keep = m->d_sc + (size_t)b0 * oh * ow * C1;
@@ -857,7 +860,7 @@
                     p.B = nb; p.H = ch; p.W = cw; p.OH = oh; p.OW = ow; p.stride = b.c1.stride; p.M = nb * oh * ow; p.C1 = C1; p.C3 = C3;
                     p.rev = b0 ? t.rev_b : t.rev;
                     p.dbg = m->sw.dbg_btail;
-                    RCCHK(timed_begin(m, CLS_CONV, 2.0 * p.M * ((double)C1 * 9 * C1 + 4.0 * C1 * C1 + 4.0 * C1 * C3 + (t.sc == SC_TAIL ? 64.0 * 256 : 0.0))));
+                    RCCHK(timed_begin(m, CLS_CONV, 2.0 * p.M * ((double)C1 * 9 * C1 + 4.0 * C1 * C1 + 4.0 * C1 * C3 + (t.sc == SC_TAIL ? (double)b.sc.Cin * C2 : 0.0))));
                     HIPCHK(opd_launch_btail(p, m->stream));
                     RCCHK(timed_end(m));
                     if (p.y) RCCHK(tap(m, "btail_y", out, (size_t)p.M * 4 * C1 * 2));
@@ -1353,6 +1356,8 @@
     auto env = [](const char* name, int* v) { if (const char* e = getenv(name)) *v = atoi(e); };
     env("OPD_DUAL_OVER_TAIL", &sw.dual_over_tail);
     env("OPD_TAIL_REV", &sw.tail_rev);
+    env("OPD_TAIL_TRANS", &sw.tail_trans);
+    if (sw.tail_trans < 0) sw.tail_trans = (flags & OPD_FLAG_MULTI_STREAM) ? 0 : 1;
     env("OPD_TAIL3", &sw.tail3);
     env("OPD_TAIL_RC", &sw.tail_rc);
     sw.tail_rc = sw.tail_rc != 0;
diff --git a/office_person_detection_vit_amd/csrc/opd_model.h b/office_person_detection_vit_amd/csrc/opd_model.h
--- a/office_person_detection_vit_amd/csrc/opd_model.h
+++ b/office_person_detection_vit_amd/csrc/opd_model.h
@@ -109,6 +109,7 @@
     int fuse_btail = 1;
     int fuse_shortcut = 1;
     int dual_over_tail = 1;
+    int tail_trans = -1;
     int tail_rev = 1;
     int tail3 = 1;
     int tail3_split = 1;
diff --git a/office_person_detection_vit_amd/csrc/opd_test_api.cpp b/office_person_detection_vit_amd/csrc/opd_test_api.cpp
--- a/office_person_detection_vit_amd/csrc/opd_test_api.cpp
+++ b/office_person_detection_vit_amd/csrc/opd_test_api.cpp
@@ -558,6 +558,81 @@
         TCHK(hipMemcpy(zb[route], d_zb, M * 64 * 2, hipMemcpyDeviceToHost));
         TCHK(hipMemcpy(yc[route], d_yc, M * 256 * 2, hipMemcpyDeviceToHost));
         TCHK(hipMemcpy(zc[route], d_zc, M * 128 * 2, hipMemcpyDeviceToHost));
+    }
+    return OPD_OK;
+}
+
+int opd_test_btail_trans(const uint16_t* x1, const uint16_t* xs, const uint16_t* w1, const float* b1, const uint16_t* w2, const uint16_t* wsc,
+                         const float* b2sc, const uint16_t* w3, const float* b3, uint16_t* const* y, uint16_t* const* z, int B, int H, int W, int iters,
+                         float* us_out) {
+    DevMem dm;
+    const int C1 = 128, C2 = 512, CS = 256, C3 = 128, OH = (H - 1) / 2 + 1, OW = (W - 1) / 2 + 1;
+    const size_t M = (size_t)B * OH * OW;
+    std::vector<uint16_t> cat((size_t)C2 * (C1 + CS));
+    for (int n = 0; n < C2; ++n) {
+        memcpy(&cat[(size_t)n * (C1 + CS)], w2 + (size_t)n * C1, (size_t)C1 * 2);
+        memcpy(&cat[(size_t)n * (C1 + CS) + C1], wsc + (size_t)n * CS, (size_t)CS * 2);
+    }
+    const uint16_t* d_x1 = dm.up(x1, (size_t)B * H * W * C1);
+    const uint16_t* d_xs = dm.up(xs, (size_t)B * H * W * CS);
+    const uint16_t* d_w1 = dm.up(w1, (size_t)C1 * 9 * C1);
+    const uint16_t* d_w2 = dm.up(w2, (size_t)C2 * C1);
+    const uint16_t* d_wsc = dm.up(wsc, (size_t)C2 * CS);
+    const uint16_t* d_cat = dm.up(cat.data(), cat.size());
+    const uint16_t* d_w3 = dm.up(w3, (size_t)C3 * C2);
+    const float* d_b1 = dm.up(b1, C1);
+    const float* d_b2 = dm.up(b2sc, C2);
+    const float* d_b3 = dm.up(b3, C3);
+    uint16_t* d_a2 = dm.up<uint16_t>(nullptr, M * C1);
+    uint16_t* d_y = dm.up<uint16_t>(nullptr, M * C2);
+    uint16_t* d_z = dm.up<uint16_t>(nullptr, M * C3);
+    const uint32_t zeros[8] = {0, 0, 0, 0, 0, 0, 0, 0};
+    const uint32_t* d_zero = dm.up(zeros, 8);
+    if (!d_x1 || !d_xs || !d_w1 || !d_w2 || !d_wsc || !d_cat || !d_w3 || !d_b1 || !d_b2 || !d_b3 || !d_a2 || !d_y || !d_z || !d_zero)
+        return tfail(OPD_ENOMEM, "test alloc failed");
+    ConvGemmParams c[3] = {};
+    for (auto& q : c) { q.dtype = g_test_dtype; q.zero16 = d_zero; q.B = B; q.OH = OH; q.OW = OW; q.M = (int)M; q.relu = 1; q.wprefetch = 1; }
+    c[0].x = d_x1; c[0].w = d_w1; c[0].bias = d_b1; c[0].out = d_a2; c[0].H = H; c[0].W = W; c[0].Cin = C1; c[0].N = C1; c[0].KH = c[0].KW = 3;
+    c[0].stride = 2; c[0].pad = 1; c[0].K = 9 * C1;
+    c[1].x = d_a2; c[1].w = d_cat; c[1].bias = d_b2; c[1].out = d_y; c[1].H = OH; c[1].W = OW; c[1].Cin = C1; c[1].N = C2; c[1].KH = c[1].KW = 1;
+    c[1].stride = 1; c[1].K1 = C1; c[1].K = C1 + CS; c[1].x2 = d_xs; c[1].H2 = H; c[1].W2 = W; c[1].Cin2 = CS; c[1].stride2 = 2;
+    c[2].x = d_y; c[2].w = d_w3; c[2].bias = d_b3; c[2].out = d_z; c[2].H = OH; c[2].W = OW; c[2].Cin = C2; c[2].N = C3; c[2].KH = c[2].KW = 1;
+    c[2].stride = 1; c[2].K = C2;
+    BtailParams p{}; p.dtype = g_test_dtype;
+    p.x1 = d_x1; p.w1 = d_w1; p.b1 = d_b1; p.w2p = d_w2; p.b2 = d_b2; p.xs = d_xs; p.wsc = d_wsc; p.xs_H = H; p.xs_W = W; p.xs_stride = 2;
+    p.y = d_y; p.w3p = d_w3; p.b3 = d_b3; p.z = d_z;
+    p.B = B; p.H = H; p.W = W; p.OH = OH; p.OW = OW; p.stride = 2; p.M = (int)M; p.C1 = C1; p.C3 = C3;
+    auto run = [&](int route) -> hipError_t {
+        if (route) return opd_launch_btail(p, nullptr);
+        for (auto& q : c) {
+            const hipError_t e = opd_launch_conv_gemm(q, nullptr);
+            if (e != hipSuccess) return e;
+        }
+        return hipSuccess;
+    };
+    for (int route = 0; route < 2; ++route) {
+        TCHK(hipMemset(d_y, 0xff, M * C2 * 2));
+        TCHK(hipMemset(d_z, 0xff, M * C3 * 2));
+        TCHK(run(route));
+        TCHK(hipDeviceSynchronize());
+        TCHK(hipMemcpy(y[route], d_y, M * C2 * 2, hipMemcpyDeviceToHost));
+        TCHK(hipMemcpy(z[route], d_z, M * C3 * 2, hipMemcpyDeviceToHost));
+    }
+    if (iters > 0 && us_out) {
+        hipEvent_t ev[2];
+        TCHK(hipEventCreate(&ev[0])); TCHK(hipEventCreate(&ev[1]));
+        for (int route = 0; route < 2; ++route) {
+            for (int i = -2; i < iters; ++i) {
+                if (i == 0) TCHK(hipEventRecord(ev[0], nullptr));
+                TCHK(run(route));
+            }
+            TCHK(hipEventRecord(ev[1], nullptr));
+            TCHK(hipEventSynchronize(ev[1]));
+            float ms = 0.f;
+            TCHK(hipEventElapsedTime(&ms, ev[0], ev[1]));
+            us_out[route] = ms * 1000.f / iters;
+        }
+        (void)hipEventDestroy(ev[0]); (void)hipEventDestroy(ev[1]);
     }
     return OPD_OK;
 }
@@ -935,7 +1010,19 @@
     return ksize;
 }
 int opd_test_valid_prefix(int valid, int in, int out) { return valid_prefix(valid, in, out); }
+static int trunk_plan_sw(const Switches& sw, const int* depths, int max_batch, int flags, int B, int H, int W, int num_cus, int* steps_out, int max_steps,
+                         int* split_out);
 int opd_test_trunk_plan(const int* depths, int max_batch, int flags, int B, int H, int W, int num_cus, int* steps_out, int max_steps, int* split_out) {
+    return trunk_plan_sw(Switches{}, depths, max_batch, flags, B, H, W, num_cus, steps_out, max_steps, split_out);
+}
+int opd_test_trunk_plan_trans(int tail_trans, const int* depths, int max_batch, int flags, int B, int H, int W, int num_cus, int* steps_out, int max_steps,
+                              int* split_out) {
+    Switches sw;
+    sw.tail_trans = tail_trans ? 1 : 0;
+    return trunk_plan_sw(sw, depths, max_batch, flags, B, H, W, num_cus, steps_out, max_steps, split_out);
+}
+static int trunk_plan_sw(const Switches& sw, const int* depths, int max_batch, int flags, int B, int H, int W, int num_cus, int* steps_out, int max_steps,
+                         int* split_out) {
     if (!depths || !steps_out || !split_out || B < 1 || H < 1 || W < 1 || num_cus < 1) return tfail(OPD_EINVAL, "bad trunk_plan arguments");
     Arch a;
     std::vector<Block> blocks;
@@ -961,7 +1048,7 @@
     if ((int)blocks.size() > max_steps) return tfail(OPD_EINVAL, "steps_out too small");
     opd_config cfg{};
     cfg.struct_size = sizeof(opd_config); cfg.max_batch = max_batch; cfg.max_height = H; cfg.max_width = W; cfg.flags = flags;
-    const TrunkPlan plan = plan_trunk(a, blocks, cfg, Switches{}, B, down2(down2(H)), down2(down2(W)), num_cus, false, 0, true);
+    const TrunkPlan plan = plan_trunk(a, blocks, cfg, sw, B, down2(down2(H)), down2(down2(W)), num_cus, false, 0, true);
     for (size_t i = 0; i < plan.steps.size(); ++i) {
         const TrunkStep& t = plan.steps[i];
         const int row[7] = {t.path, t.sc, t.res, t.store, t.C3, t.rev, t.rev_b};
```

Result: no change. 2967 (-0.0%).
